# phaistos-networks/Trinity

Hardware: AMD Instinct MI355X
Metric: queries/sec (higher is better)
Workload: dtype u32

## Files before the change

### trinity_amd/csrc/dev_structs.hpp

```cpp
#pragma once
#include <cstdint>
#ifdef __HIPCC__
#define TRI_HD __host__ __device__
#else
#define TRI_HD
#endif

struct DevTerm {
        uint32_t documents;
        uint32_t first_block;
        uint32_t nblocks;
        uint32_t last_n;
        uint32_t win_off;
        uint32_t flags;
        uint32_t npfor;
        uint32_t pad;
};
constexpr uint32_t TERM_FULL_BLOCKS = 1u;
constexpr uint32_t TERM_SPARSE = 2u;

#define TRI_BLOCK_N(t, b, index, off) (((t).flags & TERM_FULL_BLOCKS) ? ((b) + 1 == (t).nblocks ? (t).last_n : 32u) : (uint32_t)(index)[(off)-1])
constexpr uint32_t WIN_MIN_BLOCKS = 128;

constexpr uint32_t QT_GROUP = 0x80000000u;
constexpr uint32_t QT_NOT = 0x40000000u;
constexpr uint32_t QT_TERM = 0x3fffffffu;
constexpr uint32_t MAX_QTERMS = 16;
struct DevQuery {
        uint32_t nterms;
        uint32_t term_base;
        uint64_t out_off;
        uint32_t out_cap;
        uint32_t qid;
        uint32_t first_task, ntasks;
        uint32_t score_base, nscore;
        uint32_t phrase_base, nphrases;
        uint32_t fused_idx, form;
};

constexpr uint32_t RESULT_DOCIDS = 0, RESULT_BITMAP = 1;
constexpr uint32_t MAX_PHRASE_TERMS = 16;
struct DevPhrase {
        uint32_t term_base;
        uint32_t nterms;
        double weight;
};

struct DevTask {
        uint32_t slot;
        uint32_t tile_begin;
        uint32_t tile_end;
        uint32_t kind;
        uint64_t out_off;
};
constexpr uint32_t CAND_QUEUES = 8;
constexpr uint32_t CAND_TICKET_STRIDE = 16;
constexpr uint32_t CAND_HEAVY_TILES = 3;
constexpr uint32_t TASK_CAND = 0;
constexpr uint32_t TASK_DENSE = 1;
constexpr uint32_t TASK_FUSED = 2;
constexpr uint32_t TASK_FUSED16 = 3;

constexpr uint32_t TASK_FUSED_GEN = 4;
constexpr uint32_t TASK_PLANES = 5;
constexpr uint32_t TASK_PLANES8 = 6;
constexpr uint32_t TASK_PSET = 7;
constexpr uint32_t TASK_PROBE = 8;
constexpr uint32_t TASK_TREE = 9;
constexpr uint32_t TASK_KINDS = 10;
constexpr uint32_t PSET_INLINE_TERMS = 4;
#ifndef TRI_PSET_TASK_WINDOWS
#define TRI_PSET_TASK_WINDOWS 4
#endif
constexpr uint32_t PSET_TASK_WINDOWS = TRI_PSET_TASK_WINDOWS;
struct DevPsetUnit {
        uint64_t out_off;
        uint32_t w_begin, w_end;
        uint32_t tix;
        uint32_t nterms;
        uint32_t term_base;
        uint32_t first;
        uint32_t tt[PSET_INLINE_TERMS];
        uint32_t row[PSET_INLINE_TERMS];
};
static_assert(sizeof(DevPsetUnit) == 64, "one cache-line half per unit");
constexpr uint32_t PSET_UNIT_FIRST = 1u, PSET_UNIT_BITMAP = 2u;
constexpr uint32_t PSET_UNIT_ROUND_SHIFT = 4, PSET_UNIT_ROUND_MASK = 15u;
constexpr uint32_t PSET_ROUND_DOCS = 16384, PSET_STAGE_DOCS = 1024;
constexpr uint32_t PSET_UNIT_SCATTER = 4u;
constexpr uint32_t TREE_MAX_NODES = 64;
constexpr uint32_t TREE_HDR_WORDS = 8;
constexpr uint32_t TREE_CHUNK_WORDS = 2048;
constexpr uint32_t TREE_ROW_PHRASE = 0x80000000u;
struct DevTreeNode {
        uint8_t op;
        uint8_t parent;
        uint8_t ord;
        uint8_t thr;
        uint32_t arg;
        uint32_t row;
        uint32_t score;
        uint32_t rmask;
        uint8_t kid0, kid1, pad0, pad1;
        uint64_t kids;
};
static_assert(sizeof(DevTreeNode) == 32, "eight words per node");
constexpr uint32_t TREE_WIDE_MAX_NODES = 1024;
constexpr uint32_t TREE_WIDE_STACK = 64;
constexpr uint32_t TREE_KIND_WIDE = 1;
constexpr uint32_t TREE_NO_PARENT = 0xffffu;
struct DevTreeNodeW {
        uint8_t op;
        uint8_t cbits;
        uint16_t parent;
        uint32_t arg, row, score, rmask;
        uint16_t ord;
        uint16_t nkids;
        uint16_t thr;
        uint8_t pop;
        uint8_t pcbits;
        uint32_t pad;
};
static_assert(sizeof(DevTreeNodeW) == sizeof(DevTreeNode), "a wide record's nodes are eight words each too");
constexpr uint32_t RICH_NARROW_TERMS = 16, RICH_WIDE_TERMS = 64;
struct DevRichWide {
        uint64_t cells;
        uint64_t slots;
        uint32_t stride, pad;
};
static_assert(sizeof(DevRichWide) == 24, "three 8-byte words per plan slot");
TRI_HD constexpr uint32_t tree_counter_planes(const uint32_t nkids) {
        uint32_t b = 0;
        while ((1u << b) <= nkids)
                ++b;
        return b;
}
TRI_HD constexpr bool task_onepass(const uint32_t kind) { return kind >= TASK_FUSED && kind <= TASK_PLANES8; }

constexpr uint32_t PL_W = 32768;
constexpr uint32_t PL_WORDS = PL_W / 32;
constexpr uint32_t PL_NONE = 0xffffffffu;
constexpr uint32_t PL_NESTED = 6;
constexpr uint32_t PL_LEVEL_WORDS = 3;
constexpr uint32_t PL_STORED = 4;
constexpr uint32_t PL_PLANES = PL_STORED + PL_LEVEL_WORDS;
constexpr uint32_t PL_HI = PL_PLANES - 1;
constexpr uint32_t PL_HI_LEVELS = PL_STORED - 1;
constexpr uint32_t PL_RANK_WORDS = 16;
constexpr uint32_t PL_RANK_DOCS = 256;
constexpr uint32_t BLK_HITS_PLAIN = 0x80000000u;
constexpr int TILE_BLOCKS = 256;
constexpr int TILE_CANDS = TILE_BLOCKS * 32;
constexpr uint32_t SPAN_BITS = 1u << 17;
constexpr uint32_t SPAN_WORDS = SPAN_BITS / 32;
constexpr uint32_t CELL_LOG2 = 10;
constexpr uint32_t CELL_DOCS = 1u << CELL_LOG2;
constexpr uint32_t CELLS_PER_SPAN = SPAN_BITS / CELL_DOCS;
#ifndef TRI_FUS_CELLS
#define TRI_FUS_CELLS 14
#endif
constexpr uint32_t FUS_CELLS = TRI_FUS_CELLS;
constexpr uint32_t FUS_W = FUS_CELLS * CELL_DOCS;
constexpr uint32_t PLK_MAX_SPARSE = 6;
constexpr uint32_t PLK_NS_SMALL = 5;
constexpr uint32_t TOPK_MAX = 256;
constexpr uint32_t FUS_MAX_SLOTS = 8;
constexpr uint32_t FUS_MAX_LEAVES = 16;
struct DevFused {
        uint32_t nslots;
        uint32_t fbits;
        uint32_t cap;
        uint32_t nreq;
        uint32_t term[FUS_MAX_SLOTS];
        uint32_t gmask[FUS_MAX_SLOTS];
        uint32_t gslots[FUS_MAX_SLOTS];
        uint32_t nmask;
        uint32_t hw;
        uint32_t mode;
        uint32_t nleaf;
        uint32_t tt[8];
        uint8_t leaf_slot[FUS_MAX_LEAVES];
        uint32_t ctt[FUS_MAX_LEAVES][8];
        uint32_t plane[FUS_MAX_SLOTS];
        uint32_t negslots;
};
constexpr uint32_t FUS_MODE_TT = 1;
constexpr uint32_t FUS_MODE_EMIT = 2;
```

### trinity_amd/csrc/host/plan_host.cpp

```cpp
#include "../planner.hpp"
#include "../lucene_enc_units.hpp"
#include "lucene_encoder.hpp"
#include "perc_lower.hpp"

#include <cstdlib>
#include <memory>
#include <mutex>

namespace {
        struct HostPlan {
                BatchPlan P;
                uint8_t *block = nullptr;
                ~HostPlan() { free(block); }
        };
        void put_err(char *err, size_t cap, const std::string &s) {
                if (err && cap) {
                        const size_t n = std::min(cap - 1, s.size());
                        memcpy(err, s.data(), n);
                        err[n] = 0;
                }
        }
}

extern "C" {
void *tri_host_index_build(const uint8_t *index, uint64_t len, const uint8_t *hits, uint64_t hits_len, int codec, const uint32_t *terms3, uint64_t nterms,
                           uint32_t docs_cnt, char *err, uint64_t errcap) {
        auto H = std::make_unique<HostIndex>();
        std::string e;
        static_assert(sizeof(tri_term) == 12, "tri_term is three u32");
        if (build_host_index(index, len, hits, hits_len, codec, reinterpret_cast<const tri_term *>(terms3), nterms, docs_cnt, *H, e) != TRI_OK) {
                put_err(err, errcap, e);
                return nullptr;
        }
        return H.release();
}
void tri_host_index_free(void *h) { delete static_cast<HostIndex *>(h); }

void *tri_host_plan(void *hindex, const uint32_t *prog, uint64_t prog_len, const uint32_t *queries2, uint64_t nq, uint32_t flags, uint32_t topk, int similarity,
                    unsigned threads, const char *const *opt_names, const uint64_t *opt_values, unsigned nopt, uint32_t cus, char *err, uint64_t errcap) {
        const HostIndex &H = *static_cast<HostIndex *>(hindex);
        PlanEnv env;
        env.cus = cus ? cus : 256;
        bool use_frag_cache = false;
        for (unsigned i = 0; i < nopt; ++i) {
                const std::string n = opt_names[i];
                if (n == "frag_cache") {
                        use_frag_cache = opt_values[i] != 0;
                        continue;
                }
                tri_options &o = env.opt;
                uint64_t *slot = n == "dense_min_postings" ? &o.dense_min_postings : n == "dense_task_cost" ? &o.dense_task_cost : n == "fused" ? &o.fused
                                 : n == "fused_task_cost" ? &o.fused_task_cost : n == "fused_freq_cap" ? &o.fused_freq_cap : n == "fused_halfwords" ? &o.fused_halfwords
                                 : n == "account_needed_bytes" ? &o.account_needed_bytes : n == "planes" ? &o.planes : n == "planes_split" ? &o.planes_split
                                 : n == "plane_div" ? &o.plane_div : n == "plane_max_bytes" ? &o.plane_max_bytes : n == "probe_max_blocks" ? &o.probe_max_blocks : n == "tree_max_bytes" ? &o.tree_max_bytes : n == "tree_max_nodes" ? &o.tree_max_nodes : n == "tree_wide_min_nodes" ? &o.tree_wide_min_nodes : n == "result_bitmaps" ? &o.result_bitmaps : n == "cand_task_cost" ? &o.cand_task_cost : n == "dense_window_cost" ? &o.dense_window_cost
                                 : n == "cand_xcd" ? &o.cand_xcd : n == "planes_order" ? &o.planes_order : n == "pset_order" ? &o.pset_order : n == "scatter_bitmap_slack" ? &o.scatter_bitmap_slack : n == "phrase_task_div" ? &o.phrase_task_div : n == "plane_amortize" ? &o.plane_amortize : n == "rich_max_terms" ? &o.rich_max_terms : nullptr;
                if (!slot) {
                        put_err(err, errcap, "unknown option " + n);
                        return nullptr;
                }
                *slot = opt_values[i];
        }
        PlanInput in;
        in.prog = prog;
        in.prog_len = prog_len;
        static_assert(sizeof(tri_query) == 8, "tri_query is two u32");
        in.queries = reinterpret_cast<const tri_query *>(queries2);
        in.nq = nq;
        in.flags = flags;
        in.topk = topk;
        in.similarity = similarity;
        auto hp = std::make_unique<HostPlan>();
        std::unique_ptr<HostPool> pool;
        if (threads > 1)
                pool = std::make_unique<HostPool>(threads);
        std::string e;
        static trip::FragCache g_frag_cache;
        static std::mutex g_frag_mu;
        std::unique_lock<std::mutex> frag_lock(g_frag_mu, std::defer_lock);
        if (use_frag_cache)
                frag_lock.lock();
        const int rc = plan_batch(
                H, env, in, pool.get(),
                [&](size_t bytes) {
                        hp->block = static_cast<uint8_t *>(aligned_alloc(64, (bytes + 63) & ~(size_t)63));
                        if (hp->block)
                                memset(hp->block, 0, bytes);
                        return hp->block;
                },
                hp->P, e, use_frag_cache ? &g_frag_cache : nullptr);
        if (rc != TRI_OK) {
                put_err(err, errcap, e);
                return nullptr;
        }
        return hp.release();
}
void tri_host_plan_free(void *p) { delete static_cast<HostPlan *>(p); }

void tri_host_plan_summary(void *p, uint64_t *out , double *ms ) {
        const BatchPlan &P = static_cast<HostPlan *>(p)->P;
        const uint64_t v[] = {P.block_bytes,       P.plan.size(),    P.qterms.size(),      P.tasks.size(),  P.fused.size(),       P.qplane.size(),    P.plane_terms.size(), P.sterms.size(),
                              P.sweights.size(),   P.phrases.size(), P.pterms.size(),      P.ptasks.size(), P.plan.off,           P.qterms.off,       P.tasks.off,          P.sched.off,
                              P.fused.off,         P.qplane.off,     P.plane_terms.off,    P.sterms.off,    P.sweights.off,       P.phrases.off,      P.pterms.off,         P.ptasks.off,
                              P.n_dense,           P.n_cand,         P.n_fused,            P.n_fused16,     P.n_fusedgen,         P.n_planes,         P.n_planes8,          P.plw,
                              P.sparse_cap,        P.out_capacity,   P.term_bytes,         P.term_bytes_dense, P.dense_queries,   P.cand_queries,     P.fused_queries,      P.planes_queries,
                              P.unsupported_queries, P.rich_R,       sizeof(DevQuery),     sizeof(DevTask), sizeof(DevFused),     sizeof(DevPhrase),  P.cand_needed_term_bytes, P.plane_decoded_bytes,
                              P.n_pset,            P.pset_queries,   P.n_probe,            P.probe_queries, P.units.size(),       P.units.off,        P.pset_sched.off,     sizeof(DevPsetUnit),
                              P.n_tree,            P.tree_queries,   P.tree.size(),        P.tree.off,      P.tree_terms.size(),  P.tree_terms.off,   P.tree_hidden.size(), P.tree_hidden.off,
                              P.cand_q.off};
        static_assert(sizeof v / sizeof v[0] == 65, "summary layout");
        memcpy(out, v, sizeof v);
        if (ms)
                memcpy(ms, P.plan_ms, sizeof P.plan_ms);
}
void tri_host_plan_rich_wide(void *p, uint64_t *out ) {
        const BatchPlan &P = static_cast<HostPlan *>(p)->P;
        const uint64_t v[] = {P.rich_wide.size(), P.rich_wide.off, P.rich_sched.off, P.n_rich_wide, P.rich_wide_cells, P.rich_wide_slots, sizeof(DevRichWide)};
        memcpy(out, v, sizeof v);
}
void tri_host_plan_last_unsupported(void *p, char *out, uint64_t cap) { put_err(out, cap, static_cast<HostPlan *>(p)->P.last_unsupported); }
const uint8_t *tri_host_plan_block(void *p) { return static_cast<HostPlan *>(p)->P.block; }
void tri_host_plan_query_maps(void *p, uint32_t *slot_of_query, int32_t *qstatus) {
        const BatchPlan &P = static_cast<HostPlan *>(p)->P;
        memcpy(slot_of_query, P.slot_of_query.data(), P.slot_of_query.size() * 4);
        memcpy(qstatus, P.qstatus.data(), P.qstatus.size() * 4);
}
}

extern "C" {
int tri_host_lucene_encode(const uint32_t *docs, const uint32_t *freqs, const uint16_t *pos, const uint64_t *term_first, uint64_t nterms, uint8_t *index_out, uint64_t icap,
                           uint64_t *ilen, uint8_t *hits_out, uint64_t hcap, uint64_t *hlen, uint32_t *terms3) {
        using namespace trinity_amd::Codecs;
        Lucene::IndexSession sess;
        Lucene::Encoder enc(&sess);
        uint64_t h = 0;
        for (uint64_t t = 0; t < nterms; ++t) {
                enc.begin_term();
                for (uint64_t p = term_first[t]; p < term_first[t + 1]; ++p) {
                        enc.begin_document(docs[p]);
                        for (uint32_t i = 0; i < freqs[p]; ++i)
                                enc.new_hit(pos[h++]);
                        enc.end_document();
                }
                trinity_amd::term_index_ctx tctx;
                enc.end_term(&tctx);
                terms3[3 * t] = tctx.documents, terms3[3 * t + 1] = tctx.offset, terms3[3 * t + 2] = tctx.size;
        }
        *ilen = sess.indexOut.size(), *hlen = sess.positionsOut.size();
        if (*ilen > icap || *hlen > hcap)
                return -1;
        if (*ilen)
                memcpy(index_out, sess.indexOut.data(), *ilen);
        if (*hlen)
                memcpy(hits_out, sess.positionsOut.data(), *hlen);
        return 0;
}
int tri_host_lucene_encode_units(const uint32_t *docs, const uint32_t *freqs, const uint16_t *pos, const uint64_t *term_first, uint64_t nterms, uint8_t *index_out, uint64_t icap,
                                 uint64_t *ilen, uint8_t *hits_out, uint64_t hcap, uint64_t *hlen, uint32_t *terms3) {
        const uint64_t np = term_first[nterms];
        std::vector<uint64_t> hit_off(np + 1, 0), dblk_first(nterms + 1, 0), hblk_first(nterms + 1, 0);
        for (uint64_t p = 0; p < np; ++p)
                hit_off[p + 1] = hit_off[p] + freqs[p];
        for (uint64_t t = 0; t < nterms; ++t) {
                dblk_first[t + 1] = dblk_first[t] + (term_first[t + 1] - term_first[t]) / LENC_BLOCK;
                hblk_first[t + 1] = hblk_first[t] + (hit_off[term_first[t + 1]] - hit_off[term_first[t]]) / LENC_BLOCK;
        }
        std::vector<uint32_t> hdelta(hit_off[np] + 1);
        LencArgs a{docs, freqs, pos, hit_off.data(), term_first, hdelta.data(), dblk_first.data(), hblk_first.data(), nterms};
        for (uint64_t p = 0; p < np; ++p)
                lenc_unit_hdelta(a, p, hdelta.data());
        const uint64_t nd = dblk_first[nterms], nh = hblk_first[nterms];
        std::vector<uint64_t> doff(nd + 1, 0), hoff(nh + 1, 0), term_off(nterms + 1, 0), hterm_off(nterms + 1, 0);
        std::vector<uint32_t> tail_d(nterms + 1), tail_h(nterms + 1);
        for (uint64_t g = 0; g < nd; ++g)
                doff[g + 1] = doff[g] + lenc_unit_dblk_size(a, g);
        for (uint64_t h = 0; h < nh; ++h)
                hoff[h + 1] = hoff[h] + lenc_unit_hblk_size(a, h);
        for (uint64_t t = 0; t < nterms; ++t)
                lenc_unit_tail_size(a, t, &tail_d[t], &tail_h[t]);
        LencPlace pl{doff.data(), hoff.data(), term_off.data(), hterm_off.data(), tail_d.data(), tail_h.data()};
        for (uint64_t t = 0; t < nterms; ++t) {
                term_off[t + 1] = term_off[t] + lenc_term_index_size(a, pl, t);
                hterm_off[t + 1] = hterm_off[t] + lenc_term_hits_size(a, pl, t);
        }
        *ilen = term_off[nterms], *hlen = hterm_off[nterms];
        if (*ilen > icap || *hlen > hcap)
                return -1;
        for (uint64_t g = 0; g < nd; ++g)
                lenc_unit_dblk_write(a, pl, g, index_out);
        for (uint64_t h = 0; h < nh; ++h)
                lenc_unit_hblk_write(a, pl, h, hits_out);
        for (uint64_t t = 0; t < nterms; ++t) {
                lenc_unit_term_write(a, pl, t, index_out, hits_out);
                terms3[3 * t] = (uint32_t)(term_first[t + 1] - term_first[t]), terms3[3 * t + 1] = (uint32_t)term_off[t], terms3[3 * t + 2] = lenc_term_index_size(a, pl, t);
        }
        return 0;
}
}

extern "C" {
void tri_host_pfor128_group(const uint32_t *v, uint8_t *a, uint32_t *alen, uint8_t *b, uint32_t *blen) {
        auto get = [&](uint32_t i) { return v[i]; };
        const Pfor128Plan p = pfor128_plan(get);
        uint8_t *e = pfor128_emit(get, p, a);
        *alen = (uint32_t)(e - a);
        if ((uint32_t)(e - a) != p.bytes)
                *alen = 0xffffffffu;
        std::vector<uint8_t> o;
        trinity_amd::Codecs::Lucene::ints_encode(v, o);
        memcpy(b, o.data(), o.size());
        *blen = (uint32_t)o.size();
}
uint32_t tri_host_fastpfor_encode(const uint32_t *v, uint32_t *out) {
        std::vector<uint32_t> w;
        trif::fastpfor_encode(v, w);
        memcpy(out, w.data(), w.size() * 4);
        return (uint32_t)w.size();
}
int tri_host_fastpfor_decode(const uint32_t *w, uint32_t L, uint32_t *v) { return trif::fastpfor_decode(w, L, v) ? 1 : 0; }
uint32_t tri_host_pool_cpus(uint32_t threads, int32_t *out, uint32_t cap) {
        HostPool pool(threads);
        const std::vector<int> &c = pool.pinned_cpus();
        for (size_t i = 0; i < c.size() && i < cap; ++i)
                out[i] = c[i];
        return (uint32_t)c.size();
}

uint32_t tri_host_cpu_budget() { return host_cpu_budget(); }

uint32_t tri_host_index_hits_dir(void *h, uint32_t term, uint32_t *out, uint32_t *nfull) {
        const HostIndex &H = *static_cast<HostIndex *>(h);
        const DevTerm &t = H.terms[term];
        const bool have = H.codec == TRI_CODEC_GOOGLE || H.has_hdir;
        for (uint32_t b = 0; out && have && b < t.nblocks; ++b)
                out[b] = H.blk_hits[t.first_block + b];
        *nfull = H.has_hdir && t.nblocks ? H.hdir[t.pad] : 0;
        return t.nblocks;
}

void tri_host_index_facts(void *h, uint64_t *info6, uint32_t *per_term3) {
        const HostIndex &H = *static_cast<HostIndex *>(h);
        info6[0] = H.info.postings, info6[1] = H.info.blocks, info6[2] = H.info.doc_bytes, info6[3] = H.info.hit_bytes, info6[4] = H.transcoded_groups, info6[5] = H.dev_index.size();
        for (size_t t = 0; t < H.terms.size(); ++t) {
                per_term3[3 * t] = H.terms[t].documents;
                per_term3[3 * t + 1] = H.terms[t].nblocks;
                per_term3[3 * t + 2] = H.terms[t].nblocks ? H.blk_last[H.terms[t].first_block + H.terms[t].nblocks - 1] : 0;
        }
}

int tri_host_perc_lower(const uint32_t *prog, uint64_t prog_len, const uint32_t *queries2, uint64_t nq, uint32_t nterms, int32_t *status, uint64_t *info6, char *err, uint64_t errcap) {
        perc::Lowered L;
        std::string e;
        const int rc = perc::lower(prog, prog_len, reinterpret_cast<const tri_query *>(queries2), nq, nterms, L, e);
        put_err(err, errcap, e);
        if (rc != TRI_OK)
                return rc;
        for (uint64_t q = 0; q < nq; ++q)
                status[q] = L.status[q];
        uint64_t absent = 0;
        for (const uint32_t f : L.qflags)
                absent += (f & perc::Q_ABSENT) != 0;
        info6[0] = L.unsupported, info6[1] = L.leaf_term.size(), info6[2] = L.phrase_first.size() - 1, info6[3] = L.recs.size(), info6[4] = L.stack_max, info6[5] = absent;
        return TRI_OK;
}
int tri_host_perc_check_docs(const tri_perc_docs *docs, uint32_t nterms, char *err, uint64_t errcap) {
        std::string e;
        const int rc = perc::check_docs(docs, nterms, e);
        put_err(err, errcap, e);
        return rc;
}
}
```

### trinity_amd/csrc/k_psets.hpp

```cpp
#pragma once

#ifndef TRI_PSET_WG
#define TRI_PSET_WG 512
#endif
constexpr int PSET_WG = TRI_PSET_WG;
constexpr uint32_t PSET_WAVES = PSET_WG / 64;
constexpr uint32_t PSET_WORDS = 512;
constexpr uint32_t PSET_PER = PSET_WORDS / 64;
constexpr uint32_t PSET_STEP_WORDS = PSET_WAVES * PSET_WORDS;
static_assert(SPAN_WORDS % PSET_STEP_WORDS == 0, "a docID window is a whole number of steps");
constexpr uint32_t PSET_STAGE = 1024;
static_assert(PSET_PER == 8, "two 16-byte loads per lane and term");
static_assert(PSET_WAVES == 8, "the waves' counts are prefix-summed over lanes 0 .. 7 (psets_task)");
static_assert(PSET_WORDS * 32 == PSET_ROUND_DOCS && PSET_STAGE == PSET_STAGE_DOCS, "the planner sizes a task's rounds by them (dev_structs.hpp)");
static_assert(SPAN_WORDS == PSET_WAVES * PSET_WORDS, "a wave's share of a task: one sub-window of PSET_WORDS words per docID window");
static_assert(PSET_STAGE >= PSET_WORDS, "the dense walk parks the wave's words in its staging buffer");

struct PsetShared {
        uint32_t stage[PSET_WAVES][PSET_STAGE];
        alignas(16) uint32_t cnt[2][PSET_WAVES];
        DevPsetUnit unit[2];
        uint32_t tick[2];
};

#ifndef TRI_PSET_PREFETCH
#define TRI_PSET_PREFETCH 0
#endif
struct PsetNoBuf {};
struct PsetPairBuf {
        uint4 a0, a1, b0, b1;
};
template <class BUF, class R, class F>
__device__ __forceinline__ uint32_t psets_round(PsetShared &sh, R &&request, F &&words, const uint32_t w_origin, const uint32_t w_begin, const uint32_t w_end, uint32_t *__restrict__ qout,
                                                const bool as_bitmap, const uint32_t lane, const uint32_t wave, const uint32_t par) {
        const uint32_t nsub = w_end - w_begin;
        const uint32_t wave0 = w_begin * SPAN_WORDS + wave * nsub * PSET_WORDS + lane * PSET_PER;
        uint32_t *const st = sh.stage[wave];
        if (as_bitmap) {
                uint32_t lane_cnt = 0;
                BUF nxt;
                if (TRI_PSET_PREFETCH)
                        request(wave0, nxt);
                for (uint32_t sb = 0; sb < nsub; ++sb) {
                        const uint32_t word0 = wave0 + sb * PSET_WORDS;
                        BUF cur;
                        if (TRI_PSET_PREFETCH) {
                                cur = nxt;
                                if (sb + 1 < nsub)
                                        request(word0 + PSET_WORDS, nxt);
                        } else
                                request(word0, cur);
                        uint32_t acc[PSET_PER];
                        words(cur, word0, acc);
                        uint4 *o = (uint4 *)(qout + (word0 - w_origin * SPAN_WORDS));
                        o[0] = make_uint4(acc[0], acc[1], acc[2], acc[3]);
                        o[1] = make_uint4(acc[4], acc[5], acc[6], acc[7]);
#pragma unroll
                        for (uint32_t j = 0; j < PSET_PER; ++j)
                                lane_cnt += (uint32_t)__popc(acc[j]);
                }
                return lane_cnt;
        }
        uint32_t fill = 0;
        BUF nxt;
        if (TRI_PSET_PREFETCH)
                request(wave0, nxt);
        for (uint32_t sb = 0; sb < nsub; ++sb) {
                const uint32_t word0 = wave0 + sb * PSET_WORDS;
                BUF cur;
                if (TRI_PSET_PREFETCH) {
                        cur = nxt;
                        if (sb + 1 < nsub)
                                request(word0 + PSET_WORDS, nxt);
                } else
                        request(word0, cur);
                uint32_t acc[PSET_PER];
                words(cur, word0, acc);
                uint32_t c = 0;
#pragma unroll
                for (uint32_t j = 0; j < PSET_PER; ++j)
                        c += (uint32_t)__popc(acc[j]);
                uint32_t T;
                const uint32_t ex = wave_excl_scan(c, T);
#if !defined(TRI_PSET_VARIANT) || TRI_PSET_VARIANT != 1
                if (T && fill + T <= PSET_STAGE) {
                        uint32_t o = fill + ex;
#pragma unroll
                        for (uint32_t j = 0; j < PSET_PER; ++j) {
                                uint32_t m = acc[j];
                                const uint32_t d0 = (word0 + j) << 5;
                                while (m) {
                                        st[o++] = d0 + (uint32_t)__builtin_ctz(m);
                                        m &= m - 1u;
                                }
                        }
                }
#endif
                fill += T;
        }
        if (lane == 0)
                sh.cnt[par][wave] = fill;
        __syncthreads();
        const uint32_t own = sh.cnt[par][lane & (PSET_WAVES - 1u)], pre = row8_incl_scan(own);
        const uint32_t base = (uint32_t)__builtin_amdgcn_readlane((int)(pre - own), (int)wave);
        const uint32_t total = (uint32_t)__builtin_amdgcn_readlane((int)pre, (int)PSET_WAVES - 1);
#if defined(TRI_PSET_VARIANT) && (TRI_PSET_VARIANT == 1 || TRI_PSET_VARIANT == 2)
        return total;
#endif
        if (fill <= PSET_STAGE) {
                __builtin_amdgcn_wave_barrier();
                for (uint32_t i = lane; i < fill; i += 64u)
                        qout[base + i] = st[i];
                __builtin_amdgcn_wave_barrier();
        } else {
                uint32_t o = base;
                for (uint32_t sb = 0; sb < nsub; ++sb) {
                        const uint32_t word0 = wave0 + sb * PSET_WORDS;
                        uint32_t acc[PSET_PER];
                        BUF cur;
                        request(word0, cur);
                        words(cur, word0, acc);
                        uint32_t c = 0;
#pragma unroll
                        for (uint32_t j = 0; j < PSET_PER; ++j)
                                c += (uint32_t)__popc(acc[j]);
                        uint32_t T;
                        const uint32_t ex = wave_excl_scan(c, T);
                        if (!T)
                                continue;
                        if (T <= PSET_STAGE) {
                                uint32_t at = ex;
#pragma unroll
                                for (uint32_t j = 0; j < PSET_PER; ++j) {
                                        uint32_t m = acc[j];
                                        const uint32_t d0 = (word0 + j) << 5;
                                        while (m) {
                                                st[at++] = d0 + (uint32_t)__builtin_ctz(m);
                                                m &= m - 1u;
                                        }
                                }
                                __builtin_amdgcn_wave_barrier();
                                for (uint32_t i = lane; i < T; i += 64u)
                                        qout[o + i] = st[i];
                                __builtin_amdgcn_wave_barrier();
                                o += T;
                                continue;
                        }
#pragma unroll
                        for (uint32_t j = 0; j < PSET_PER; ++j)
                                st[lane * PSET_PER + j] = acc[j];
                        __builtin_amdgcn_wave_barrier();
                        const uint32_t wbase = word0 - lane * PSET_PER;
                        for (uint32_t cidx = 0; cidx < PSET_WORDS / 2; ++cidx) {
                                const uint32_t wi = 2u * cidx + (lane >> 5);
                                const bool bit = (st[wi] >> (lane & 31u)) & 1u;
                                const uint64_t bm = __builtin_amdgcn_ballot_w64(bit);
                                if (bit)
                                        qout[o + __builtin_amdgcn_mbcnt_hi((uint32_t)(bm >> 32), __builtin_amdgcn_mbcnt_lo((uint32_t)bm, 0u))] = ((wbase + wi) << 5) + (lane & 31u);
                                o += (uint32_t)__popcll(bm);
                        }
                        __builtin_amdgcn_wave_barrier();
                }
        }
        return total;
}

#ifndef TRI_PSET_WAVES
#define TRI_PSET_WAVES 8
#endif
template <int CODEC>
__global__ __launch_bounds__(PSET_WG, TRI_PSET_WAVES) void k_psets(const DevPsetUnit *__restrict__ units, const uint32_t *__restrict__ order, const uint32_t ntasks,
                                                                   uint32_t *__restrict__ ticket, const uint32_t *__restrict__ qterms, const uint32_t *__restrict__ qplane,
                                                                   uint32_t *__restrict__ out, uint32_t *__restrict__ counts, const uint32_t *__restrict__ masked,
                                                                   const uint32_t *__restrict__ planes, const uint32_t plw, const uint32_t *__restrict__ scat_off,
                                                                   const uint32_t *__restrict__ scat_cnt, const uint32_t *__restrict__ scat_docs TRI_FILTER_ARG) {
        __shared__ PsetShared sh;
        const uint32_t tid = threadIdx.x, lane = tid & 63u;
        const uint32_t wave = uni(tid >> 6);
        uint32_t nt = 0xffffffffu;
        if (wave == 0) {
                const uint32_t t0 = uni(atomicAdd(ticket, 1u)) >> 6;
                uint32_t wd = 0;
                if (t0 < ntasks)
                        wd = ((const uint32_t *)(units + order[t0]))[lane & 15u];
                ((uint32_t *)&sh.unit[0])[lane & 15u] = wd;
                sh.tick[0] = t0;
                nt = uni(atomicAdd(ticket, 1u)) >> 6;
        }
        __syncthreads();
        uint32_t par = 0;
        for (uint32_t p = 0;; p ^= 1u) {
                if (uni(sh.tick[p]) >= ntasks)
                        break;
                const DevPsetUnit &U = sh.unit[p];
                const uint32_t nterms = uni(U.nterms), w_begin = uni(U.w_begin), w_end = uni(U.w_end), tix = uni(U.tix), term_base = uni(U.term_base);
                const bool as_bitmap = uni(U.first) & PSET_UNIT_BITMAP;
                TRI_FILTER_TASK_OF(tix);
                uint32_t *const qout = out + (((uint64_t)uni((uint32_t)(U.out_off >> 32)) << 32) | uni((uint32_t)U.out_off));
                uint32_t nwd = 0, nnt = 0xffffffffu;
                if (wave == 0) {
                        if (nt < ntasks)
                                nwd = ((const uint32_t *)(units + order[nt]))[lane & 15u];
                        nnt = atomicAdd(ticket, 1u);
                }
                uint32_t produced = 0;
                uint32_t scat_at = 0, scat_n = 0;
                if (uni(U.first) & PSET_UNIT_SCATTER)
                        scat_at = uni(scat_off[tix]), scat_n = uni(scat_cnt[tix]);
                const uint32_t round_win = std::max(1u, (uni(U.first) >> PSET_UNIT_ROUND_SHIFT) & PSET_UNIT_ROUND_MASK);
                const uint32_t pair_row0 = uni(U.row[0]), pair_row1 = uni(U.row[1]), pair_tt1 = uni(U.tt[1]);
                if (nterms == 2 && pair_row0 != PL_NONE && pair_row1 != PL_NONE) {
                        const uint32_t *const row_a = planes + (size_t)pair_row0 * plw, *const row_b = planes + (size_t)pair_row1 * plw;
                        const bool pair_or = !(pair_tt1 & QT_GROUP);
                        const uint32_t flip = (pair_tt1 & QT_NOT) ? ~0u : 0u;
                        for (uint32_t wb = w_begin; wb < w_end; wb += round_win, par ^= 1u)
                        produced += psets_round<PsetPairBuf>(
                            sh,
                            [&](const uint32_t word0, PsetPairBuf &buf) {
                                    const uint4 *pa = (const uint4 *)(row_a + word0);
                                    const uint4 *pb = (const uint4 *)(row_b + word0);
                                    buf.a0 = pa[0], buf.a1 = pa[1], buf.b0 = pb[0], buf.b1 = pb[1];
                            },
                            [&](const PsetPairBuf &buf, const uint32_t word0, uint32_t(&acc)[PSET_PER]) {
                                    const uint4 a0 = buf.a0, a1 = buf.a1, b0 = buf.b0, b1 = buf.b1;
                                    if (pair_or) {
                                            acc[0] = a0.x | b0.x, acc[1] = a0.y | b0.y, acc[2] = a0.z | b0.z, acc[3] = a0.w | b0.w;
                                            acc[4] = a1.x | b1.x, acc[5] = a1.y | b1.y, acc[6] = a1.z | b1.z, acc[7] = a1.w | b1.w;
                                    } else {
                                            acc[0] = a0.x & (b0.x ^ flip), acc[1] = a0.y & (b0.y ^ flip), acc[2] = a0.z & (b0.z ^ flip), acc[3] = a0.w & (b0.w ^ flip);
                                            acc[4] = a1.x & (b1.x ^ flip), acc[5] = a1.y & (b1.y ^ flip), acc[6] = a1.z & (b1.z ^ flip), acc[7] = a1.w & (b1.w ^ flip);
                                    }
                                    if (masked) {
                                            const uint4 *pm = (const uint4 *)(masked + word0);
                                            const uint4 m0 = pm[0], m1 = pm[1];
                                            acc[0] &= ~m0.x, acc[1] &= ~m0.y, acc[2] &= ~m0.z, acc[3] &= ~m0.w;
                                            acc[4] &= ~m1.x, acc[5] &= ~m1.y, acc[6] &= ~m1.z, acc[7] &= ~m1.w;
                                    }
                            },
                            w_begin, wb, min(w_end, wb + round_win), as_bitmap ? qout : qout + produced, as_bitmap, lane, wave, par);
                } else
                        for (uint32_t wb = w_begin; wb < w_end; wb += round_win, par ^= 1u)
                        produced += psets_round<PsetNoBuf>(
                            sh, [](const uint32_t, PsetNoBuf &) {},
                            [&](const PsetNoBuf &, const uint32_t word0, uint32_t(&acc)[PSET_PER]) {
                                    uint32_t grp[PSET_PER];
                                    bool have_acc = false, cur_neg = false;
#pragma unroll
                                    for (uint32_t j = 0; j < PSET_PER; ++j)
                                            acc[j] = grp[j] = 0;
                                    for (uint32_t k = 0; k <= nterms; ++k) {
                                            uint32_t tt = QT_GROUP, row = 0;
                                            if (k < nterms) {
                                                    if (nterms <= PSET_INLINE_TERMS) {
                                                            tt = uni(U.tt[k]);
                                                            row = uni(U.row[k]);
                                                    } else {
                                                            tt = uni(qterms[term_base + k]);
                                                            row = uni(qplane[term_base + k]);
                                                    }
                                            }
                                            if (k && (tt & QT_GROUP)) {
#pragma unroll
                                                    for (uint32_t j = 0; j < PSET_PER; ++j) {
                                                            acc[j] = !have_acc ? grp[j] : cur_neg ? acc[j] & ~grp[j] : acc[j] & grp[j];
                                                            grp[j] = 0;
                                                    }
                                                    have_acc = true;
                                            }
                                            if (k == nterms)
                                                    break;
                                            if (tt & QT_GROUP)
                                                    cur_neg = tt & QT_NOT;
                                            if (row == PL_NONE)
                                                    continue;
                                            const uint4 *pa = (const uint4 *)(planes + (size_t)row * plw + word0);
#if defined(TRI_PSET_VARIANT) && TRI_PSET_VARIANT == 3
                                            const uint32_t hsh = (word0 * 2654435761u) ^ (k * 40503u);
                                            const uint4 v0 = make_uint4(hsh & (hsh >> 3) & (hsh >> 7), 0, (hsh >> 5) & (hsh << 2) & (hsh >> 11), 0), v1 = make_uint4(0, hsh & 0x10001u, 0, hsh & 0x200u);
#else
                                            const uint4 v0 = pa[0], v1 = pa[1];
#endif
                                            grp[0] |= v0.x, grp[1] |= v0.y, grp[2] |= v0.z, grp[3] |= v0.w;
                                            grp[4] |= v1.x, grp[5] |= v1.y, grp[6] |= v1.z, grp[7] |= v1.w;
                                    }
                                    if (masked) {
                                            const uint4 *pm = (const uint4 *)(masked + word0);
                                            const uint4 m0 = pm[0], m1 = pm[1];
                                            acc[0] &= ~m0.x, acc[1] &= ~m0.y, acc[2] &= ~m0.z, acc[3] &= ~m0.w;
                                            acc[4] &= ~m1.x, acc[5] &= ~m1.y, acc[6] &= ~m1.z, acc[7] &= ~m1.w;
                                    }
                            },
                            w_begin, wb, min(w_end, wb + round_win), as_bitmap ? qout : qout + produced, as_bitmap, lane, wave, par);
                if (uni(U.first) & PSET_UNIT_SCATTER) {
                        __syncthreads();
                        const uint32_t off = scat_at, n = scat_n, doc0 = w_begin * SPAN_BITS;
                        for (uint32_t i = tid; i < n; i += PSET_WG) {
                                const uint32_t rel = scat_docs[off + i] - doc0, bit = 1u << (rel & 31u);
                                produced += (atomicOr(&qout[rel >> 5], bit) & bit) ? 0u : 1u;
                        }
                }
                if (as_bitmap) {
#pragma unroll
                        for (int d = 32; d >= 1; d >>= 1)
                                produced += __shfl_xor(produced, d, 64);
                        sh.cnt[par][wave] = produced;
                        __syncthreads();
                        produced = 0;
#pragma unroll
                        for (uint32_t wv = 0; wv < PSET_WAVES; ++wv)
                                produced += uni(sh.cnt[par][wv]);
                        par ^= 1u;
                }
                if (wave == 0) {
                        counts[tix] = produced;
                        ((uint32_t *)&sh.unit[p ^ 1u])[lane & 15u] = nwd;
                        sh.tick[p ^ 1u] = nt;
                        __builtin_amdgcn_s_waitcnt(0xc07f);
                        nt = uni(nnt) >> 6;
                }
                __syncthreads();
        }
}

constexpr int PSCAT_WG = 256;
constexpr uint32_t PSCAT_MAX_TASKS = 4096;
static_assert((1ull << 31) / ((uint64_t)PSET_TASK_WINDOWS * SPAN_BITS) <= PSCAT_MAX_TASKS, "a query's tasks fit the workgroup's LDS counters");
struct PscatShared {
        DevTerm term[MAX_QTERMS];
        uint32_t nrows[MAX_QTERMS];
        uint32_t cnt[PSCAT_MAX_TASKS];
        uint32_t red[PSCAT_WG / 64 + 1];
};
struct PscatPost {
        uint32_t *cnt;
        const uint32_t *masked;
        uint32_t *place;
        uint32_t nbits, task_docs, cap;
        __device__ __forceinline__ void doc(const uint32_t d) {
                if (d >= nbits || (masked && ((masked[d >> 5] >> (d & 31u)) & 1u)))
                        return;
                const uint32_t at = atomicAdd(&cnt[d / task_docs], 1u);
                if (place && at < cap)
                        place[at] = d;
        }
        __device__ __forceinline__ void operator()(const uint32_t d, const uint32_t) { doc(d); }
};
__global__ __launch_bounds__(256) void k_psets_prep_list(const DevPsetUnit *__restrict__ units, const uint32_t nunits, uint32_t *__restrict__ cursor, uint32_t *__restrict__ list,
                                                         const uint32_t cap) {
        const uint32_t u = blockIdx.x * 256u + threadIdx.x;
        if (u >= nunits || !(units[u].first & PSET_UNIT_SCATTER) || units[u].w_begin != 0)
                return;
        const uint32_t at = atomicAdd(cursor, 1u);
        if (at < cap)
                list[at] = u;
}
template <int CODEC>
__global__ __launch_bounds__(PSCAT_WG) void k_psets_prep(const DevPsetUnit *__restrict__ units, const uint32_t *__restrict__ list, const uint32_t *__restrict__ listed, const DevQuery *__restrict__ plan, const DevTask *__restrict__ tasks,
                                                         const uint32_t *__restrict__ qterms, const uint32_t *__restrict__ qplane, const uint32_t *__restrict__ masked_,
                                                         const uint8_t *__restrict__ index, const uint32_t *__restrict__ blk_last, const uint32_t *__restrict__ blk_off,
                                                         const uint4 *__restrict__ blk_rec, const uint32_t *__restrict__ blk_doff, const DevTerm *__restrict__ terms,
                                                         uint32_t *__restrict__ cursor, uint32_t *__restrict__ scat_off, uint32_t *__restrict__ scat_cnt,
                                                         uint32_t *__restrict__ scat_docs, const uint32_t scat_cap, const FilterSel fsel) {
        __shared__ PscatShared sh;
        const uint32_t tid = threadIdx.x;
        if (blockIdx.x >= uni(*listed))
                return;
        const DevPsetUnit &U = units[uni(list[blockIdx.x])];
        const uint32_t nterms = uni(U.nterms), term_base = uni(U.term_base), tix = uni(U.tix);
        if (tid < MAX_QTERMS) {
                uint32_t n = 0;
                if (tid < nterms && qplane[term_base + tid] == PL_NONE) {
                        const DevTerm t = terms[qterms[term_base + tid] & QT_TERM];
                        sh.term[tid] = t;
                        n = t.nblocks;
                }
                sh.nrows[tid] = n;
        }
        const uint32_t slot = uni(tasks[tix].slot);
        const DevQuery &q = plan[slot];
        const uint32_t *const masked = filter_pick_if(masked_, fsel, slot);
        const uint32_t ntasks = min(uni(q.ntasks), PSCAT_MAX_TASKS), nbits = uni(q.out_cap) * 32u, task_docs = (uni(U.w_end) - uni(U.w_begin)) * SPAN_BITS;
        for (uint32_t t = tid; t < ntasks; t += PSCAT_WG)
                sh.cnt[t] = 0;
        __syncthreads();
        uint32_t total = 0;
        for (uint32_t k = 0; k < nterms; ++k)
                total += uni(sh.nrows[k]);
        for (uint32_t pass = 0; pass < 2; ++pass) {
                PscatPost post{sh.cnt, masked, pass ? scat_docs : nullptr, nbits, task_docs, scat_cap};
                for (uint32_t v = tid; v < total; v += PSCAT_WG) {
                        uint32_t k = 0, b = v;
                        for (; b >= sh.nrows[k]; ++k)
                                b -= sh.nrows[k];
                        const DevTerm t = sh.term[k];
                        const uint32_t *bl = blk_last + t.first_block;
                        const uint32_t prev = b ? bl[b - 1] : 0, last = bl[b];
#ifdef TRI_PROF
                        ProfClock prof_;
#endif
                        decode_row<CODEC, false, PscatPost>(index, blk_off, blk_rec, blk_doff, t, b, prev, last, 0u, post PROF_PASS);
                }
                __syncthreads();
                if (pass)
                        break;
                const uint32_t per = (ntasks + PSCAT_WG - 1) / PSCAT_WG, t0 = tid * per, t1 = min(ntasks, t0 + per);
                uint32_t mine = 0;
                for (uint32_t t = t0; t < t1; ++t)
                        mine += sh.cnt[t];
                uint32_t wtot;
                uint32_t ex = wave_excl_scan(mine, wtot);
                if ((tid & 63u) == 0)
                        sh.red[tid >> 6] = wtot;
                __syncthreads();
                uint32_t before = 0, all = 0;
                for (uint32_t w = 0; w < PSCAT_WG / 64; ++w) {
                        before += w < (tid >> 6) ? sh.red[w] : 0u;
                        all += sh.red[w];
                }
                if (tid == 0)
                        sh.red[PSCAT_WG / 64] = atomicAdd(cursor, all);
                __syncthreads();
                const uint32_t base = uni(sh.red[PSCAT_WG / 64]);
                uint32_t at = base + before + ex;
                for (uint32_t t = t0; t < t1; ++t) {
                        const uint32_t c = sh.cnt[t];
                        const bool fits = at + c <= scat_cap;
                        scat_off[tix + t] = fits ? at : 0u;
                        scat_cnt[tix + t] = fits ? c : 0u;
                        sh.cnt[t] = fits ? at : scat_cap;
                        at += c;
                }
                __syncthreads();
        }
}
```

### trinity_amd/csrc/planner.hpp

```cpp
#pragma once
#include "planner_lower.hpp"
#include "planner_tasks.hpp"

namespace trip {
        struct RowQ {
                uint8_t n = 0, q[CAND_QUEUES] = {}, sub[CAND_QUEUES] = {};
        };
        struct LapTimer {
                const bool on;
                std::chrono::steady_clock::time_point t0 = std::chrono::steady_clock::now();
                std::string line;
                void lap(const char *what) {
                        if (!on)
                                return;
                        char buf[64];
                        snprintf(buf, sizeof buf, " %s %.3f", what, ms_since(t0));
                        line += buf;
                }
        };

        struct PlanState {
                const HostIndex &ix;
                const PlanEnv &env;
                const tri_options &opt;
                HostPool *pool;
                BatchPlan &P;
                std::string &err;
                Ctx C;
                LapTimer dbg;
                FragCache *cache = nullptr;
                std::vector<Frag> frags;
                SectionCounts n;
                uint64_t cand_queries_all = 0;
                std::vector<uint64_t> benefit, cand_row;
                std::vector<uint32_t> tree_terms;
                std::vector<uint32_t> chosen;
                std::vector<uint32_t> row_of_rank;
                bool cand_rows = false;
                std::vector<RowQ> rowq;
                uint32_t pset_ranges = 0;
                uint32_t cand_first = 0, cand_qat[CAND_QUEUES] = {};
                std::vector<uint32_t> unit_of_task;
                ~PlanState() {
                        if (!cache)
                                return;
                        if (cache->frags.size() < frags.size())
                                cache->frags.resize(frags.size());
                        for (size_t k = 0; k < frags.size(); ++k)
                                cache->frags[k] = std::move(frags[k]);
                }
                template <class Fn>
                void run(Fn &&fn) {
                        if (pool && frags.size() > 1)
                                pool->run((unsigned)frags.size(), fn);
                        else
                                for (unsigned k = 0; k < frags.size(); ++k)
                                        fn(k);
                }
                int first_error() {
                        for (Frag &f : frags)
                                if (f.rc != TRI_OK) {
                                        err = f.err;
                                        return f.rc;
                                }
                        return TRI_OK;
                }
                template <class Fn>
                int run_pass(const char *name, const char *doing, Fn &&fn) {
                        run([&](unsigned k) {
                                Frag &f = frags[k];
                                try {
                                        f.rc = fn(f);
                                } catch (const std::bad_alloc &) {
                                        f.rc = herr(f.err, TRI_ERR_NOMEM, "tri_batch_create: out of host memory while %s", doing);
                                } catch (...) {
                                        f.rc = herr(f.err, TRI_ERR_INVALID, "tri_batch_create: unexpected exception while %s", doing);
                                }
                        });
                        dbg.lap(name);
                        return first_error();
                }
        };

        inline void eligible_planes(PlanState &S) {
                const HostIndex &ix = S.ix;
                const tri_options &opt = S.opt;
                S.P.plw = ((ix.max_doc >> 17) + 2u) * (SPAN_BITS / 32u);
                S.C.plw = S.P.plw;
                if (opt.planes && opt.plane_div && !ix.df_sorted.empty()) {
                        const uint64_t min_df = std::max<uint64_t>(1, ix.info.docs_cnt / opt.plane_div);
                        const size_t n = (size_t)(std::partition_point(ix.df_sorted.begin(), ix.df_sorted.end(), [&](uint32_t d) { return d && d >= min_df; }) - ix.df_sorted.begin());
                        const uint64_t row_bytes = (uint64_t)PL_PLANES * S.P.plw * 4;
                        S.C.n_ok = (uint32_t)std::min<uint64_t>(n, std::max<uint64_t>(1, opt.plane_max_bytes / std::max<uint64_t>(1, row_bytes)));
                }
        }

        inline void take_fragments(PlanState &S, FragCache *cache) {
                const size_t nq = S.C.in.nq;
                const unsigned nthreads = S.pool ? std::min<unsigned>(S.pool->size(), (unsigned)std::max<size_t>(1, nq / 512)) : 1u;
                const size_t nfrag = nthreads <= 1 ? 1 : std::min<size_t>(2 * nthreads, std::max<size_t>(1, nq / 256));
                S.frags.resize(nfrag);
                S.cache = cache;
                for (size_t k = 0; k < nfrag; ++k) {
                        if (cache && k < cache->frags.size()) {
                                S.frags[k] = std::move(cache->frags[k]);
                                S.frags[k].recycle();
                        }
                        S.frags[k].q_lo = nq * k / nfrag;
                        S.frags[k].q_hi = nq * (k + 1) / nfrag;
                }
        }

        inline void settle_batch_knobs(PlanState &S) {
                const tri_options &opt = S.opt;
                const PlanEnv &env = S.env;
                Ctx &C = S.C;
                uint64_t onepass_queries = 0, fused_postings = 0, phrase_queries = 0;
                for (const Frag &f : S.frags) {
                        onepass_queries += f.onepass_queries;
                        fused_postings += f.fused_postings;
                        phrase_queries += f.phrase_queries;
                }
                C.phrase_task_div = opt.phrase_task_div ? opt.phrase_task_div : !phrase_queries ? 1 : phrase_queries <= 8ull * env.cus ? 4 : phrase_queries <= 16ull * env.cus ? 2 : 1;
                C.planes_split = opt.planes_split ? opt.planes_split : (2 * onepass_queries >= 4ull * (uint64_t)env.cus * env.plk_wgs_per_cu ? 2 : 3) ;
                C.fused_task_cost = opt.fused_task_cost;
                if (!C.fused_task_cost) {
                        const uint64_t want_tasks = 2ull * (uint64_t)env.cus * env.fus_wgs_per_cu;
                        C.fused_task_cost = std::min<uint64_t>(8u << 20, std::max<uint64_t>(256u << 10, fused_postings / std::max<uint64_t>(1, want_tasks)));
                }
        }

        inline int place_fragments(PlanState &S) {
                BatchPlan &P = S.P;
                SectionCounts &n = S.n;
                const uint32_t n_ok = S.C.n_ok;
                uint64_t off = 0;
                S.benefit.assign(n_ok, 0), S.cand_row.assign(n_ok, 0);
                for (Frag &f : S.frags) {
                        f.b_plan = n.plan, f.b_qterms = n.qterms, f.b_sterms = n.sterms, f.b_phrases = n.phrases, f.b_pterms = n.pterms, f.b_tasks = n.tasks, f.b_fused = n.fused,
                        f.b_ptasks = n.ptasks, f.b_off = off, f.b_units = n.units, f.b_tree = n.tree, f.b_hidden = n.tree_hidden;
                        n.plan += f.tmp.size(), n.qterms += f.qterms.size(), n.sterms += f.sterms.size(), n.phrases += f.phrases.size(), n.pterms += f.pterms.size(),
                                n.tasks += f.tasks.size(), n.fused += f.fused.size(), n.ptasks += f.ptasks.size(), n.units += f.units.size(), n.tree += f.treepool.size(),
                                n.tree_hidden += f.n_hidden, off += f.off;
                        S.tree_terms.insert(S.tree_terms.end(), f.tree_terms.begin(), f.tree_terms.end());
                        P.merge(f);
                        for (uint32_t r = 0; r < n_ok; ++r)
                                S.benefit[r] += f.benefit[r], S.cand_row[r] += f.cand_row[r];
                        for (const size_t qi : f.left_out) {
                                P.qstatus[qi] = TRI_ERR_UNSUPPORTED;
                                ++P.unsupported_queries;
                        }
                        if (!f.left_out.empty())
                                P.last_unsupported = f.err;
                }
                S.cand_queries_all = P.cand_queries + P.probe_queries;
                if (n.qterms > 0xfffffff0ull || n.sterms > 0xfffffff0ull || n.tasks > 0xfffffff0ull || n.pterms > 0xfffffff0ull)
                        return herr(S.err, TRI_ERR_UNSUPPORTED, "tri_batch_create: the batch exceeds 2^32 terms or tasks: split it");
                P.out_capacity = off;
                if (P.rich_wide_queries)
                        n.rich_wide = n.plan, n.rich_sched = n.tasks;
                std::sort(S.tree_terms.begin(), S.tree_terms.end());
                S.tree_terms.erase(std::unique(S.tree_terms.begin(), S.tree_terms.end()), S.tree_terms.end());
                n.tree_terms = S.tree_terms.size();
                P.tree_scratch_bytes = ((uint64_t)n.tree_terms * PL_PLANES + n.tree_hidden + P.tree_queries) * P.plw * 4;
                if (P.tree_scratch_bytes > S.opt.tree_max_bytes)
                        return herr(S.err, TRI_ERR_NOMEM, "tri_batch_create: the batch's %llu tree queries need %llu bytes of bitmap scratch (%zu distinct term leaves, %zu phrase leaves; option tree_max_bytes = %llu): split the batch",
                                    (unsigned long long)P.tree_queries, (unsigned long long)P.tree_scratch_bytes, n.tree_terms, n.tree_hidden, (unsigned long long)S.opt.tree_max_bytes);
                return TRI_OK;
        }

        inline void choose_planes(PlanState &S) {
                const HostIndex &ix = S.ix;
                const uint32_t n_ok = S.C.n_ok;
                std::vector<uint32_t> rank_term(n_ok, UINT32_MAX);
                std::vector<uint8_t> forced(n_ok, 0);
                for (const Frag &f : S.frags) {
                        for (const QUse &u : f.quses)
                                rank_term[ix.df_rank[u.term]] = u.term;
                        for (const QUse &u : f.suses)
                                rank_term[ix.df_rank[u.term]] = u.term;
                        for (const FUse &u : f.fuses)
                                rank_term[ix.df_rank[u.term]] = u.term, forced[ix.df_rank[u.term]] = 1;
                }
                for (uint32_t r = 0; r < n_ok; ++r)
                        if (rank_term[r] != UINT32_MAX && (forced[r] || S.benefit[r] * std::max<uint64_t>(1, S.opt.plane_amortize) >= ix.terms[rank_term[r]].documents))
                                S.chosen.push_back(rank_term[r]);
                std::sort(S.chosen.begin(), S.chosen.end());
                S.row_of_rank.assign(n_ok, PL_NONE);
                for (const uint32_t term : S.chosen) {
                        S.row_of_rank[ix.df_rank[term]] = ix.df_rank[term];
                        S.P.plane_decoded_bytes += ix.docbytes[term];
                }
                S.P.plane_rows = n_ok;
                S.n.plane_terms = S.chosen.size();
                S.n.qplane = S.chosen.empty() ? 0 : S.n.qterms;
                S.n.splane = (S.chosen.empty() || !S.C.scored) ? 0 : S.n.sterms;
                S.n.sweights = S.C.scored ? S.n.sterms : 0;
        }

        inline void assign_cand_rows(PlanState &S) {
                const BatchPlan &P = S.P;
                const uint32_t n_ok = S.C.n_ok;
                const std::vector<uint64_t> &cand_row = S.cand_row;
                S.pset_ranges = ((S.ix.max_doc >> 17) + 1u + PSET_TASK_WINDOWS - 1) / PSET_TASK_WINDOWS;
                S.cand_rows = S.opt.cand_xcd && !S.chosen.empty() && S.cand_queries_all && P.cand_lead_docs >= CAND_ROWS_MIN_LEAD * S.cand_queries_all && P.cand_terms <= 3 * S.cand_queries_all;
                S.rowq.assign(S.cand_rows ? n_ok : 0, RowQ{});
                if (S.cand_rows) {
                        uint64_t total = 0, load[CAND_QUEUES] = {};
                        uint32_t placed[CAND_QUEUES] = {};
                        std::vector<uint32_t> rows;
                        for (uint32_t r = 0; r < n_ok; ++r)
                                if (cand_row[r] && S.row_of_rank[r] != PL_NONE)
                                        rows.push_back(r), total += cand_row[r];
                        std::sort(rows.begin(), rows.end(), [&](uint32_t a, uint32_t b) { return cand_row[a] != cand_row[b] ? cand_row[a] > cand_row[b] : a < b; });
                        const uint64_t cap = std::max<uint64_t>(1, total / (2 * CAND_QUEUES));
                        for (const uint32_t r : rows) {
                                RowQ &z = S.rowq[r];
                                z.n = (uint8_t)std::min<uint64_t>(CAND_QUEUES, (cand_row[r] + cap - 1) / cap);
                                for (uint32_t k = 0; k < z.n; ++k) {
                                        const uint32_t x = (uint32_t)(std::min_element(load, load + CAND_QUEUES) - load);
                                        load[x] += cand_row[r] / z.n;
                                        z.q[k] = (uint8_t)x;
                                        z.sub[k] = (uint8_t)(CAND_COST_SUBS + placed[x]++ % (CAND_SUBS - CAND_COST_SUBS - 1));
                                }
                        }
                }
                if (S.dbg.on) {
                        char buf[96];
                        snprintf(buf, sizeof buf, " [cand queries %llu lead docs %llu terms %llu rows %d]", (unsigned long long)S.cand_queries_all, (unsigned long long)P.cand_lead_docs, (unsigned long long)P.cand_terms, (int)S.cand_rows);
                        S.dbg.line += buf;
                }
        }

        inline int layout_block(PlanState &S, const std::function<uint8_t *(size_t)> &alloc_block) {
                BatchPlan &P = S.P;
                P.block_bytes = layout_sections(P, S.n);
                S.dbg.lap("sums+planes+layout");
                P.block = alloc_block(P.block_bytes);
                S.dbg.lap("alloc_block");
                if (!P.block)
                        return herr(S.err, TRI_ERR_NOMEM, "tri_batch_create: no host memory for the plan (%zu bytes)", P.block_bytes);
                point_sections(P, S.n);
                std::copy(S.tree_terms.begin(), S.tree_terms.end(), P.tree_terms.p);
                S.unit_of_task.assign(S.n.units ? S.n.tasks : 0, 0u);
                std::copy(S.chosen.begin(), S.chosen.end(), P.plane_terms.p);
                S.dbg.lap("spans");
                return TRI_OK;
        }

        inline int fill_fragment(PlanState &S, Frag &f) {
                const HostIndex &ix = S.ix;
                BatchPlan &P = S.P;
                const std::vector<uint32_t> &row_of_rank = S.row_of_rank;
                for (size_t i = 0; i < f.tmp.size(); ++i) {
                        DevQuery q = f.tmp[i].q;
                        q.term_base += (uint32_t)f.b_qterms;
                        q.score_base += (uint32_t)f.b_sterms;
                        q.phrase_base += (uint32_t)f.b_phrases;
                        q.first_task += (uint32_t)f.b_tasks;
                        q.out_off += f.b_off;
                        if (f.tmp[i].fuse)
                                q.fused_idx += (uint32_t)f.b_fused;
                        if (f.tmp[i].tree)
                                q.fused_idx += (uint32_t)f.b_tree;
                        if (f.tmp[i].hidden) {
                                q.qid = 0xffffffffu;
                                P.tree_hidden[f.b_hidden + f.tmp[i].hidden_ord] = (uint32_t)(f.b_plan + i);
                        } else
                                P.slot_of_query[q.qid] = (uint32_t)(f.b_plan + i);
                        P.plan[f.b_plan + i] = q;
                }
                if (!f.treepool.empty()) {
                        memcpy(&P.tree[f.b_tree], f.treepool.data(), f.treepool.size() * 4);
                        for (size_t i = 0; i < f.tmp.size(); ++i) {
                                if (!f.tmp[i].tree)
                                        continue;
                                uint32_t *rec = &P.tree[f.b_tree + f.tmp[i].q.fused_idx];
                                DevTreeNode *tn = reinterpret_cast<DevTreeNode *>(rec + TREE_HDR_WORDS);
                                for (uint32_t k = 0; k < rec[0]; ++k)
                                        if (tn[k].op == TRI_OP_TERM)
                                                tn[k].row = (uint32_t)(std::lower_bound(P.tree_terms.begin(), P.tree_terms.end(), tn[k].arg) - P.tree_terms.begin());
                                        else if (tn[k].op == TRI_OP_PHRASE) {
                                                tn[k].arg += (uint32_t)f.b_plan;
                                                tn[k].row += (uint32_t)f.b_hidden;
                                        }
                        }
                }
                for (size_t i = 0; i < f.tasks.size(); ++i) {
                        DevTask t = f.tasks[i];
                        t.slot += (uint32_t)f.b_plan;
                        t.out_off += f.b_off;
                        P.tasks[f.b_tasks + i] = t;
                }
                if (!f.qterms.empty())
                        memcpy(&P.qterms[f.b_qterms], f.qterms.data(), f.qterms.size() * 4);
                if (!f.sterms.empty())
                        memcpy(&P.sterms[f.b_sterms], f.sterms.data(), f.sterms.size() * 4);
                if (S.C.scored && !f.sweights.empty())
                        memcpy(&P.sweights[f.b_sterms], f.sweights.data(), f.sweights.size() * 8);
                for (size_t i = 0; i < f.phrases.size(); ++i) {
                        DevPhrase ph = f.phrases[i];
                        ph.term_base += (uint32_t)f.b_pterms;
                        P.phrases[f.b_phrases + i] = ph;
                }
                if (!f.pterms.empty())
                        memcpy(&P.pterms[f.b_pterms], f.pterms.data(), f.pterms.size() * 4);
                for (size_t i = 0; i < f.ptasks.size(); ++i)
                        P.ptasks[f.b_ptasks + i] = f.ptasks[i] + (uint32_t)f.b_tasks;
                for (size_t i = 0; i < f.fused.size(); ++i)
                        P.fused[f.b_fused + i] = f.fused[i];
                for (const FUse &u : f.fuses)
                        P.fused[f.b_fused + u.fidx].plane[u.slot] = row_of_rank[ix.df_rank[u.term]];
                for (size_t i = 0; i < f.units.size(); ++i) {
                        DevPsetUnit u = f.units[i];
                        u.out_off += f.b_off;
                        u.tix += (uint32_t)f.b_tasks;
                        u.term_base += (uint32_t)f.b_qterms;
                        const bool is_probe = f.tasks[f.units[i].tix].kind == TASK_PROBE;
                        bool rows = true;
                        for (uint32_t k = is_probe ? 1u : 0u; k < u.nterms; ++k) {
                                const uint32_t term = (k < PSET_INLINE_TERMS ? u.tt[k] : f.qterms[f.units[i].term_base + k]) & QT_TERM;
                                const uint32_t rank = ix.df_rank[term];
                                const uint32_t row = rank < row_of_rank.size() ? row_of_rank[rank] : PL_NONE;
                                rows &= row != PL_NONE;
                                if (k < PSET_INLINE_TERMS)
                                        u.row[k] = row;
                                if (row == PL_NONE && (u.first & PSET_UNIT_SCATTER) && u.w_begin == 0)
                                        f.pscatter_docs += ix.terms[term].documents;
                        }
                        if (is_probe && !rows) {
                                P.tasks[u.tix].kind = TASK_CAND;
                                if (u.first & PSET_UNIT_FIRST) {
                                        ++f.probe_demoted;
                                        f.probe_demoted_bytes += distinct_docbytes(ix, &f.qterms[f.units[i].term_base], u.nterms, f.S.seen);
                                }
                        }
                        P.units[f.b_units + i] = u;
                        S.unit_of_task[u.tix] = (uint32_t)(f.b_units + i);
                }
                if (S.n.splane) {
                        std::fill(&P.splane.p[f.b_sterms], &P.splane.p[f.b_sterms] + f.sterms.size(), PL_NONE);
                        for (const QUse &u : f.suses)
                                P.splane[f.b_sterms + u.qpos] = row_of_rank[ix.df_rank[u.term]];
                }
                if (S.n.qplane) {
                        std::fill(&P.qplane.p[f.b_qterms], &P.qplane.p[f.b_qterms] + f.qterms.size(), PL_NONE);
                        for (const QUse &u : f.quses)
                                P.qplane[f.b_qterms + u.qpos] = row_of_rank[ix.df_rank[u.term]];
                }
                return TRI_OK;
        }

        inline uint32_t key_planes_order(const PlanState &S, const Frag &f, const size_t i, const DevTask &tk) {
                const DevQuery &q = S.P.plan[tk.slot];
                const DevFused &z = S.P.fused[q.fused_idx];
                uint32_t minrow = PL_NONE;
                for (uint32_t sidx = 0; sidx < z.nslots; ++sidx)
                        minrow = std::min(minrow, z.plane[sidx]);
                const uint32_t ord = (uint32_t)(f.b_tasks + i) - q.first_task, per = SCHED_NB / 4;
                return SCHED_RANK[tk.kind] * SCHED_NB + (S.opt.planes_order == 2 ? std::min(minrow, per - 1) * 4 + std::min(ord, 3u) : std::min(ord, 3u) * per + std::min(minrow, per - 1));
        }
        inline uint32_t key_pset_order(const PlanState &S, const Frag &f, const size_t i) {
                const uint32_t range = (uint32_t)(f.tcost[i] & 0xffffffffull) / PSET_TASK_WINDOWS;
                const uint32_t rb = S.pset_ranges <= PSET_RANGE_BKS ? std::min(range, PSET_RANGE_BKS - 1) : (uint32_t)std::min<uint64_t>((uint64_t)range * PSET_RANGE_BKS / S.pset_ranges, PSET_RANGE_BKS - 1);
                return PSET_KEY0 + rb * PSET_SUBS + pset_sub((uint32_t)(f.tcost[i] >> 32));
        }
        inline uint32_t key_cand_rows(const PlanState &S, const Frag &f, const size_t i, const DevTask &tk) {
                const DevQuery &q = S.P.plan[tk.slot];
                uint32_t row = PL_NONE;
                for (uint32_t k = 1; k < q.nterms && row == PL_NONE; ++k)
                        row = S.P.qplane[q.term_base + k];
                uint32_t queue, sub;
                if (tk.tile_end - tk.tile_begin > CAND_HEAVY_TILES || row == PL_NONE)
                        queue = (uint32_t)(f.b_tasks + i) % CAND_QUEUES, sub = (sched_key(TASK_CAND, f.tcost[i]) % SCHED_NB) / (SCHED_NB / CAND_COST_SUBS);
                else if (row < S.rowq.size() && S.rowq[row].n) {
                        const RowQ &z = S.rowq[row];
                        const uint32_t piece = (uint32_t)(f.b_tasks + i) % z.n;
                        queue = z.q[piece], sub = z.sub[piece];
                } else
                        queue = row % CAND_QUEUES, sub = CAND_SUBS - 1;
                return CAND_KEY0 + queue * CAND_SUBS + sub;
        }
        inline uint32_t schedule_key(const PlanState &S, const Frag &f, const size_t i) {
                const DevTask &tk = S.P.tasks[f.b_tasks + i];
                switch (tk.kind) {
                        case TASK_PLANES:
                        case TASK_PLANES8:
                                if (S.opt.planes_order)
                                        return key_planes_order(S, f, i, tk);
                                break;
                        case TASK_PSET:
                                if (S.opt.pset_order)
                                        return key_pset_order(S, f, i);
                                break;
                        case TASK_CAND:
                                if (S.cand_rows)
                                        return key_cand_rows(S, f, i, tk);
                                break;
                }
                return sched_key(tk.kind, f.tcost[i]);
        }
        inline int key_fragment(const PlanState &S, Frag &f) {
                f.keys.resize(f.tasks.size());
                f.hist.assign(SCHED_KEYS, 0u);
                for (size_t i = 0; i < f.tasks.size(); ++i)
                        ++f.hist[f.keys[i] = schedule_key(S, f, i)];
                return TRI_OK;
        }

        inline void place_schedule(PlanState &S) {
                BatchPlan &P = S.P;
                uint32_t at = 0;
                for (uint32_t r = 0; r < TASK_KINDS; ++r) {
                        const uint32_t before = at;
                        if (r == SCHED_RANK[TASK_CAND])
                                S.cand_first = at;
                        auto place = [&](const uint32_t bk) {
                                for (Frag &f : S.frags) {
                                        const uint32_t c = f.hist[bk];
                                        f.hist[bk] = at;
                                        at += c;
                                }
                        };
                        for (uint32_t bk = r * SCHED_NB; bk < (r + 1) * SCHED_NB; ++bk)
                                place(bk);
                        if (r == SCHED_RANK[TASK_PSET] && S.opt.pset_order)
                                for (uint32_t bk = PSET_KEY0; bk < PSET_KEY0 + std::min(S.pset_ranges, PSET_RANGE_BKS) * PSET_SUBS; ++bk)
                                        place(bk);
                        if (r == SCHED_RANK[TASK_CAND])
                                for (uint32_t bk = CAND_KEY0; bk < PSET_KEY0; ++bk) {
                                        if ((bk - CAND_KEY0) % CAND_SUBS == 0)
                                                S.cand_qat[(bk - CAND_KEY0) / CAND_SUBS] = at;
                                        place(bk);
                                }
                        for (uint32_t k = 0; k < TASK_KINDS; ++k)
                                if (SCHED_RANK[k] == r)
                                        P.*SCHED_COUNT[k] = at - before;
                }
                const uint32_t units_first = sched_first(P, TASK_PSET), n_units_run = P.n_pset + P.n_probe;
                S.run([&](unsigned k) {
                        Frag &f = S.frags[k];
                        for (size_t i = 0; i < f.tasks.size(); ++i) {
                                const uint32_t pos = f.hist[f.keys[i]]++, ti = (uint32_t)(f.b_tasks + i);
                                P.sched[pos] = ti;
                                if (pos >= units_first && pos - units_first < n_units_run)
                                        P.pset_sched[pos - units_first] = S.unit_of_task[ti];
                        }
                });
        }

        inline void split_tree_section(BatchPlan &P) {
                if (!P.n_tree)
                        return;
                uint32_t *const ts = P.sched.p + sched_first(P, TASK_TREE);
                auto narrow = [&](const uint32_t ti) { return P.tree[P.plan[P.tasks[ti].slot].fused_idx + 1] != TREE_KIND_WIDE; };
                P.n_tree_wide = P.n_tree - (uint32_t)std::count_if(ts, ts + P.n_tree, narrow);
                if (P.n_tree_wide && P.n_tree_wide < P.n_tree)
                        std::stable_partition(ts, ts + P.n_tree, narrow);
        }

        inline void place_rich_wide(BatchPlan &P) {
                if (P.rich_wide.empty())
                        return;
                uint64_t cells = 0, slots = 0;
                for (size_t i = 0; i < P.plan.size(); ++i) {
                        const DevQuery &q = P.plan[i];
                        DevRichWide w{};
                        if (q.nscore > RICH_NARROW_TERMS) {
                                w.cells = cells, w.slots = slots, w.stride = (q.nscore + 7u) & ~7u;
                                cells += (uint64_t)q.out_cap * w.stride, slots += q.out_cap;
                                P.n_rich_wide += q.ntasks;
                        }
                        P.rich_wide[i] = w;
                }
                P.rich_wide_cells = cells, P.rich_wide_slots = slots;
                std::copy(P.sched.begin(), P.sched.end(), P.rich_sched.begin());
                std::stable_partition(P.rich_sched.begin(), P.rich_sched.end(), [&](const uint32_t ti) { return P.rich_wide[P.tasks[ti].slot].stride == 0; });
        }

        inline void deal_cand_queues(PlanState &S) {
                BatchPlan &P = S.P;
                const uint32_t nc = P.n_cand;
                uint32_t *const sc = P.sched.p + S.cand_first;
                if (S.cand_rows) {
                        for (uint32_t x = 0; x <= CAND_QUEUES; ++x)
                                P.cand_q[x] = x < CAND_QUEUES ? S.cand_qat[x] - S.cand_first : nc;
                } else {
                        const std::vector<uint32_t> was(sc, sc + nc);
                        uint32_t pos = 0;
                        for (uint32_t x = 0; x < CAND_QUEUES; ++x) {
                                P.cand_q[x] = pos;
                                for (uint32_t i = x; i < nc; i += CAND_QUEUES)
                                        sc[pos++] = was[i];
                        }
                        P.cand_q[CAND_QUEUES] = pos;
                }
        }

        inline void order_phrase_tasks(BatchPlan &P) {
                if (P.ptasks.size() <= 1)
                        return;
                const size_t np = P.ptasks.size();
                std::vector<uint32_t> key(np), sorted(np);
                uint32_t hist[SCHED_NB + 1] = {};
                for (size_t i = 0; i < np; ++i) {
                        const uint32_t ti = P.ptasks[i];
                        const DevTask &tk = P.tasks[ti];
                        const DevQuery &q = P.plan[tk.slot];
                        const uint64_t end = ti + 1 < q.first_task + q.ntasks ? P.tasks[ti + 1].out_off : q.out_off + q.out_cap;
                        key[i] = SCHED_NB - 1 - cost_bucket(end - tk.out_off);
                        ++hist[key[i] + 1];
                }
                for (uint32_t bk = 0; bk < SCHED_NB; ++bk)
                        hist[bk + 1] += hist[bk];
                for (size_t i = 0; i < np; ++i)
                        sorted[hist[key[i]]++] = P.ptasks[i];
                std::copy(sorted.begin(), sorted.end(), P.ptasks.p);
        }

        inline void account_distinct_bytes(const HostIndex &ix, const Ctx &C, BatchPlan &P) {
                std::vector<uint8_t> seen(ix.terms.size(), 0);
                std::vector<uint8_t> seen_hits(ix.terms.size(), 0);
                for (size_t sidx = 0; sidx < P.plan.size(); ++sidx) {
                        const DevQuery &q = P.plan[sidx];
                        const uint32_t kind = P.tasks[q.first_task].kind;
                        auto touch = [&](uint32_t term) {
                                if (!(seen[term] & 0x80u))
                                        P.distinct_bytes += ix.docbytes[term];
                                if (!(seen[term] & (1u << kind)))
                                        P.distinct_bytes_kind[kind] += ix.docbytes[term];
                                seen[term] |= (uint8_t)(0x80u | (1u << kind));
                        };
                        if (kind == TASK_TREE) {
                                const uint32_t *rec = &P.tree[q.fused_idx];
                                const DevTreeNode *tn = reinterpret_cast<const DevTreeNode *>(rec + TREE_HDR_WORDS);
                                for (uint32_t k = 0; k < rec[0]; ++k)
                                        if (tn[k].op == TRI_OP_TERM)
                                                touch(tn[k].arg);
                        } else if (task_onepass(kind)) {
                                const DevFused &z = P.fused[q.fused_idx];
                                for (uint32_t k = 0; k < z.nslots; ++k)
                                        touch(z.term[k]);
                        } else {
                                for (uint32_t k = 0; k < q.nterms; ++k)
                                        touch(P.qterms[q.term_base + k] & QT_TERM);
                                if (C.mode != TRI_FLAG_DOCUMENTS_ONLY)
                                        for (uint32_t k = 0; k < q.nscore; ++k)
                                                touch(P.sterms[q.score_base + k]);
                        }
                        auto touch_hits = [&](uint32_t term, bool phrase) {
                                if (!(seen_hits[term] & 1u))
                                        P.distinct_bytes += ix.hitbytes[term];
                                if (phrase && !(seen_hits[term] & 2u))
                                        P.distinct_bytes_kind[TASK_KINDS] += ix.hitbytes[term];
                                seen_hits[term] |= (uint8_t)(1u | (phrase ? 2u : 0u));
                        };
                        for (uint32_t ph = 0; ph < q.nphrases; ++ph)
                                for (uint32_t k = 0; k < P.phrases[q.phrase_base + ph].nterms; ++k)
                                        touch_hits(P.pterms[P.phrases[q.phrase_base + ph].term_base + k], true);
                        if (C.rich)
                                for (uint32_t k = 0; k < q.nscore; ++k)
                                        touch_hits(P.sterms[q.score_base + k], false);
                }
        }
}

inline int plan_batch(const HostIndex &ix, const PlanEnv &env, const PlanInput &in, HostPool *pool, const std::function<uint8_t *(size_t)> &alloc_block,
                      BatchPlan &P, std::string &err, trip::FragCache *frag_cache = nullptr) {
        using namespace trip;
        auto t0 = std::chrono::steady_clock::now();
        static const bool dbg_plan = getenv("TRINITY_DEBUG_PLAN") != nullptr;
        const uint32_t mode = in.flags & (TRI_FLAG_DOCUMENTS_ONLY | TRI_FLAG_ACCUMULATED_SCORE | TRI_FLAG_MATCHED_TERMS);
        PlanState S{ix, env, env.opt, pool, P, err, Ctx{ix, env, in, mode == TRI_FLAG_ACCUMULATED_SCORE, mode == TRI_FLAG_MATCHED_TERMS, mode}, LapTimer{dbg_plan}};
        if (env.opt.tree_max_nodes < TREE_MAX_NODES || env.opt.tree_max_nodes > TREE_WIDE_MAX_NODES)
                return herr(err, TRI_ERR_INVALID, "tri_batch_create: option tree_max_nodes = %llu (%u .. %u)", (unsigned long long)env.opt.tree_max_nodes, TREE_MAX_NODES, TREE_WIDE_MAX_NODES);
        if (env.opt.rich_max_terms < RICH_NARROW_TERMS || env.opt.rich_max_terms > RICH_WIDE_TERMS)
                return herr(err, TRI_ERR_INVALID, "tri_batch_create: option rich_max_terms = %llu (%u .. %u)", (unsigned long long)env.opt.rich_max_terms, RICH_NARROW_TERMS, RICH_WIDE_TERMS);
        P.slot_of_query.assign(in.nq, UINT32_MAX);
        P.qstatus.assign(in.nq, TRI_OK);
        eligible_planes(S);
        take_fragments(S, frag_cache);
        S.dbg.lap("setup");
        if (const int rc = S.run_pass("LOWER", "lowering the batch", [&](Frag &f) { return lower_range(S.C, f); }))
                return rc;
        settle_batch_knobs(S);
        S.dbg.lap("glue0");
        P.plan_ms[0] = ms_since(t0);
        if (const int rc = S.run_pass("TASKS", "cutting the batch into tasks", [&](Frag &f) { return task_range(S.C, f); }))
                return rc;
        P.plan_ms[1] = ms_since(t0);
        if (const int rc = place_fragments(S))
                return rc;
        choose_planes(S);
        assign_cand_rows(S);
        if (const int rc = layout_block(S, alloc_block))
                return rc;
        if (const int rc = S.run_pass("FILL", "filling the plan", [&](Frag &f) {
                    fill_fragment(S, f);
                    return key_fragment(S, f);
            }))
                return rc;
        for (const Frag &f : S.frags) {
                P.pscatter_docs += f.pscatter_docs;
                P.probe_queries -= f.probe_demoted, P.cand_queries += f.probe_demoted;
                P.term_bytes_probe -= f.probe_demoted_bytes;
        }
        P.plan_ms[2] = ms_since(t0);
        place_schedule(S);
        deal_cand_queues(S);
        split_tree_section(P);
        place_rich_wide(P);
        order_phrase_tasks(P);
        P.sparse_cap = (P.sparse_cap + 63u) & ~63u;
        S.dbg.lap("sched+rest");
        if (dbg_plan)
                fprintf(stderr, "[tri plan] nq %zu frags %zu:%s\n", in.nq, S.frags.size(), S.dbg.line.c_str());
        P.plan_ms[3] = ms_since(t0);
        if (env.opt.account_needed_bytes && !ix.terms.empty())
                account_distinct_bytes(ix, S.C, P);
        return TRI_OK;
}
```

### trinity_amd/csrc/planner_tasks.hpp

```cpp
#pragma once
#include "planner_types.hpp"

namespace trip {
        inline void tasks_tree(const Ctx &C, Frag &f, Tmp &t, const uint32_t slot, uint64_t &off) {
                t.q.out_off = off;
                t.q.out_cap = (uint32_t)t.tree_ub;
                t.q.first_task = (uint32_t)f.tasks.size();
                t.q.ntasks = 1;
                f.tcost.push_back(std::max<uint64_t>(1, t.tree_ub));
                f.tasks.push_back({slot, 0, (C.plw + TREE_CHUNK_WORDS - 1) / TREE_CHUNK_WORDS, TASK_TREE, off});
                off += t.q.out_cap;
                ++f.tree_queries;
        }

        inline int tasks_onepass(const Ctx &C, Frag &f, Tmp &t, const uint32_t slot, uint64_t &off) {
                const HostIndex &ix = C.ix;
                DevFused z = f.fz[t.fz];
                uint32_t nsparse = 0;
                for (uint32_t sidx = 0; sidx < z.nslots; ++sidx) {
                        z.plane[sidx] = PL_NONE;
                        nsparse += C.plane_ok(z.term[sidx]) ? 0u : 1u;
                }
                const bool pk = !t.truth && (C.env.opt.planes & 4u) && nsparse <= PLK_MAX_SPARSE && ix.max_doc < 0x7fff0000u;
                {
// ... 30 lines not shown
                        if (emit)
                                for (uint32_t sidx = 0; sidx < z.nslots; ++sidx)
                                        b1 += C.first_block_ge(ix.terms[z.term[sidx]], (uint64_t)wb * fw);
                        uint64_t entries = 0;
                        if (pk) {
                                for (uint32_t sidx = 0; sidx < z.nslots; ++sidx) {
                                        if (C.plane_ok(z.term[sidx]))
                                                continue;
                                        const DevTerm &tk = ix.terms[z.term[sidx]];
                                        const uint32_t r0 = C.first_block_ge(tk, (uint64_t)wb * fw);
                                        const uint32_t r1 = C.first_block_ge(tk, (uint64_t)we * fw);
                                        if (r0 < tk.nblocks)
                                                entries += 32ull * (std::min(r1, tk.nblocks - 1) - r0 + 1);
                                }
                                if (entries > 0x7fffffffull)
                                        return herr(f.err, TRI_ERR_UNSUPPORTED, "query %u: a task's decoded lists exceed 2^31 entries", t.q.qid);
                                f.sparse_cap = std::max(f.sparse_cap, (uint32_t)entries);
                        }
                        f.tcost.push_back(per_win * (we - wb));
                        f.tasks.push_back({slot, wb, we, pk ? (z.nslots <= PLK_NS_SMALL ? TASK_PLANES : TASK_PLANES8) : z.mode ? TASK_FUSED_GEN : z.hw ? TASK_FUSED16 : TASK_FUSED,
                                           off + (emit ? b1 * 32 + 32ull * ord * z.nslots : 0)});
                }
                if (emit) {
                        uint64_t blocks = 0;
                        for (uint32_t sidx = 0; sidx < z.nslots; ++sidx)
                                blocks += ix.terms[z.term[sidx]].nblocks;
                        t.q.out_cap = (uint32_t)std::min<uint64_t>(0xffffffffull, blocks * 32 + 32ull * (ord + 1) * z.nslots);
                        off += t.q.out_cap;
                }
                t.q.ntasks = (uint32_t)f.tasks.size() - t.q.first_task;
                f.fused.push_back(z);
                return TRI_OK;
        }

        struct Route {
                bool pset = false;
                bool pscatter = false;
                bool probe = false;
        };
        inline Route route_cnf(const Ctx &C, Frag &f, Tmp &t, const uint32_t *qt) {
                const HostIndex &ix = C.ix;
                const tri_options &opt = C.env.opt;
                const uint64_t planes_opt = opt.planes;
                const DevTerm &lead = ix.terms[qt[0] & QT_TERM];
                Route r;
                r.pset = t.dense && (planes_opt & 2u);
                for (uint32_t k = 0; r.pset && k < t.q.nterms; ++k)
                        r.pset = C.plane_ok(qt[k] & QT_TERM);
                if (t.dense && !r.pset && (planes_opt & 2u) && C.mode == TRI_FLAG_DOCUMENTS_ONLY && opt.result_bitmaps && !t.q.nphrases && t.q.nterms >= 2) {
                        uint64_t plane_df = 0;
                        bool one_group = true;
                        for (uint32_t k = 0; k < t.q.nterms; ++k) {
                                one_group = one_group && !(qt[k] & QT_NOT) && (k == 0) == ((qt[k] & QT_GROUP) != 0);
                                if (C.plane_ok(qt[k] & QT_TERM))
                                        plane_df += ix.terms[qt[k] & QT_TERM].documents;
                        }
                        const uint32_t nwin = t.last_doc / SPAN_BITS + 1;
                        const double N = std::max<double>(1.0, (double)ix.info.docs_cnt);
                        r.pscatter = one_group && plane_df && std::min<double>(N, (double)plane_df) * (double)std::max<uint64_t>(1, opt.scatter_bitmap_slack) >= (double)nwin * SPAN_WORDS;
                        r.pset = r.pscatter;
                }
                if (t.dense && !r.pset && t.nlead == 1 && (planes_opt & 1u) && !C.plane_ok(qt[0] & QT_TERM) && t.q.nterms >= 2) {
                        bool probes = true;
                        for (uint32_t k = 1; probes && k < t.q.nterms; ++k)
                                probes = C.plane_ok(qt[k] & QT_TERM);
                        if (probes)
                                t.dense = false;
                }
                if (t.dense) {
                        (r.pset ? f.term_bytes_pset : f.term_bytes_dense) += distinct_docbytes(ix, qt, t.q.nterms, f.S.seen);
                        for (uint32_t k = 0; k < t.q.nterms; ++k) {
                                const uint32_t term = qt[k] & QT_TERM;
                                if ((planes_opt & 2u) && C.plane_ok(term)) {
                                        f.benefit[ix.df_rank[term]] += ix.terms[term].documents;
                                        f.quses.push_back({t.q.term_base + k, term});
                                }
                        }
                        ++(r.pset ? f.pset_queries : f.dense_queries);
                } else {
                        r.probe = t.nlead == 1 && t.q.nterms >= 2 && t.q.nphrases == 0 && (planes_opt & 1u) && lead.nblocks <= opt.probe_max_blocks;
                        for (uint32_t k = 1; r.probe && k < t.q.nterms; ++k)
                                r.probe = C.plane_ok(qt[k] & QT_TERM);
                        ++(r.probe ? f.probe_queries : f.cand_queries);
                        f.cand_lead_docs += lead.documents, f.cand_terms += t.q.nterms;
                        if (r.probe)
                                f.term_bytes_probe += distinct_docbytes(ix, qt, t.q.nterms, f.S.seen);
                        bool first_row = !r.probe;
                        for (uint32_t k = 1; k < t.q.nterms; ++k) {
                                const uint32_t term = qt[k] & QT_TERM;
                                if ((planes_opt & 1u) && C.plane_ok(term)) {
                                        f.benefit[ix.df_rank[term]] += std::min<uint64_t>(ix.terms[term].documents, 32ull * lead.documents);
                                        f.quses.push_back({t.q.term_base + k, term});
                                        if (first_row) {
                                                const uint32_t ntiles = (lead.nblocks + TILE_BLOCKS - 1) / TILE_BLOCKS;
                                                f.cand_row[ix.df_rank[term]] += ntiles + (ntiles + CAND_HEAVY_TILES - 1) / CAND_HEAVY_TILES;
                                                first_row = false;
                                        }
                                }
                        }
                }
                if (C.scored && (planes_opt & 1u))
                        for (uint32_t k = 0; k < t.q.nscore; ++k) {
                                const uint32_t term = f.sterms[t.q.score_base + k];
                                if (C.plane_ok(term)) {
                                        f.benefit[ix.df_rank[term]] += std::min<uint64_t>(ix.terms[term].documents, 32ull * t.lead_docs);
                                        f.suses.push_back({t.q.score_base + k, term});
                                }
                        }
                return r;
        }

        inline int tasks_windows(const Ctx &C, Frag &f, Tmp &t, const uint32_t slot, const uint32_t *qt, const Route r, const uint64_t off) {
                const HostIndex &ix = C.ix;
                const tri_options &opt = C.env.opt;
                const uint32_t nlead = t.nlead;
                const bool pset = r.pset, pscatter = r.pscatter;
                const uint32_t nwin = t.last_doc / SPAN_BITS + 1;
                bool bitmap = false;
                double est = 1.0;
                if (pset || (C.mode == TRI_FLAG_DOCUMENTS_ONLY && opt.result_bitmaps && !t.q.nphrases)) {
                        const double N = std::max<double>(1.0, (double)ix.info.docs_cnt);
                        double g = 0.0;
                        bool negg = false;
                        for (uint32_t k = 0; k <= t.q.nterms; ++k) {
                                if (k == t.q.nterms || (k && (qt[k] & QT_GROUP))) {
                                        if (!negg)
                                                est *= std::min(1.0, g / N);
                                        g = 0.0;
                                }
                                if (k == t.q.nterms)
                                        break;
                                if (qt[k] & QT_GROUP)
                                        negg = qt[k] & QT_NOT;
                                g += ix.terms[qt[k] & QT_TERM].documents;
                        }
                        bitmap = C.mode == TRI_FLAG_DOCUMENTS_ONLY && opt.result_bitmaps && !t.q.nphrases && (pscatter || est * N >= (double)nwin * SPAN_WORDS);
                }
                uint32_t round_win = 1;
                while (round_win < PSET_TASK_WINDOWS && est * (double)PSET_ROUND_DOCS * (double)(round_win * 2u) <= 0.75 * (double)PSET_STAGE_DOCS)
                        round_win *= 2u;
                if (pscatter && !bitmap)
                        return herr(f.err, TRI_ERR_INTERNAL, "query %u: a scatter union whose result is not a bitmap", t.q.qid);
                t.q.form = bitmap ? RESULT_BITMAP : RESULT_DOCIDS;
                const uint64_t per_win = std::max<uint64_t>(1, t.sumdf / (ix.info.docs_cnt / SPAN_BITS + 1)) + (pset ? 0 : opt.dense_window_cost);
                const uint32_t pdiv = t.q.nphrases ? (uint32_t)std::max<uint64_t>(1, C.phrase_task_div) : 1u;
                const uint32_t win_per_task = pset ? std::max(1u, PSET_TASK_WINDOWS / pdiv) : (uint32_t)std::max<uint64_t>(1, std::max<uint64_t>(1, opt.dense_task_cost) / pdiv / per_win);
                uint32_t ord = 0;
                uint64_t lead_blocks = 0;
                for (uint32_t k = 0; k < nlead; ++k)
                        lead_blocks += ix.terms[qt[k] & QT_TERM].nblocks;
                uint64_t heaviest = 0xffffffffull;
                for (uint32_t k = 0; pset && k < t.q.nterms; ++k)
                        heaviest = std::min<uint64_t>(heaviest, ix.df_rank[qt[k] & QT_TERM]);
                for (uint32_t wb = 0; wb < nwin; wb += win_per_task, ++ord) {
                        const uint32_t we = std::min(nwin, wb + win_per_task);
                        uint64_t b1 = 0;
                        for (uint32_t k = 0; k < nlead; ++k)
                                b1 += C.first_block_ge(ix.terms[qt[k] & QT_TERM], (uint64_t)wb * SPAN_BITS);
                        f.tcost.push_back(pset ? wb | heaviest << 32 : per_win * (we - wb));
                        const uint64_t task_off = bitmap ? off + (uint64_t)wb * SPAN_WORDS : off + b1 * 32 + 32ull * ord * nlead;
                        if (pset)
                                f.units.push_back(make_unit(t.q, qt, (uint32_t)f.tasks.size(), wb, we, task_off,
                                                            (bitmap ? PSET_UNIT_BITMAP : 0u) | (pscatter ? PSET_UNIT_SCATTER : 0u) | round_win << PSET_UNIT_ROUND_SHIFT));
                        f.tasks.push_back({slot, wb, we, pset ? TASK_PSET : TASK_DENSE, task_off});
                }
                t.q.out_cap = bitmap ? nwin * SPAN_WORDS : (uint32_t)std::min<uint64_t>(0xffffffffull, lead_blocks * 32 + 32ull * (ord + 1) * nlead);
                f.bitmap_queries += bitmap;
                f.pscatter_queries += pscatter;
                return TRI_OK;
        }

        inline uint64_t cand_needed_bytes(const HostIndex &ix, const uint32_t *qt, const uint32_t nterms) {
                const DevTerm &lead = ix.terms[qt[0] & QT_TERM];
                uint64_t need = ix.docbytes[qt[0] & QT_TERM];
                const uint32_t *ll = &ix.blk_last[lead.first_block];
                for (uint32_t k = 1; k < nterms; ++k) {
                        const DevTerm &tk = ix.terms[qt[k] & QT_TERM];
                        const uint32_t *ol = &ix.blk_last[tk.first_block];
                        uint64_t blocks = 0;
                        uint32_t at = 0;
                        for (uint32_t lb = 0; lb < lead.nblocks && at < tk.nblocks; ++lb) {
                                const uint32_t lo_doc = lb ? ll[lb - 1] + 1 : 1u, hi_doc = ll[lb];
                                at = (uint32_t)(std::lower_bound(ol + at, ol + tk.nblocks, lo_doc) - ol);
                                if (at >= tk.nblocks)
                                        break;
                                const uint32_t last = (uint32_t)(std::lower_bound(ol + at, ol + tk.nblocks, hi_doc) - ol);
                                const uint32_t span = std::min(last, tk.nblocks - 1) - at + 1;
                                const uint32_t ndocs = lb + 1 == lead.nblocks ? lead.last_n : 32u;
                                blocks += std::min(span, ndocs);
                        }
                        need += (uint64_t)((double)ix.docbytes[qt[k] & QT_TERM] * std::min(1.0, (double)blocks / std::max(1u, tk.nblocks)));
                }
                return need;
        }

        inline void tasks_tiles(const Ctx &C, Frag &f, Tmp &t, const uint32_t slot, const uint32_t *qt, const Route r, const uint64_t off) {
                const tri_options &opt = C.env.opt;
                const DevTerm &lead = C.ix.terms[qt[0] & QT_TERM];
                const uint32_t ntiles = (lead.nblocks + TILE_BLOCKS - 1) / TILE_BLOCKS;
                const uint64_t per_tile = std::max<uint64_t>(1, t.cost / ntiles);
                const uint32_t tiles_per_task = (uint32_t)std::max<uint64_t>(1, std::max<uint64_t>(1, opt.cand_task_cost / (t.q.nphrases ? std::max<uint64_t>(1, C.phrase_task_div) : 1)) / per_tile);
                for (uint32_t tb = 0; tb < ntiles; tb += tiles_per_task) {
                        const uint32_t te = std::min(ntiles, tb + tiles_per_task);
                        f.tcost.push_back(per_tile * (te - tb));
                        if (r.probe)
                                f.units.push_back(make_unit(t.q, qt, (uint32_t)f.tasks.size(), tb, te, off + (uint64_t)tb * TILE_CANDS, tb == 0 ? PSET_UNIT_FIRST : 0u));
                        f.tasks.push_back({slot, tb, te, r.probe ? TASK_PROBE : TASK_CAND, off + (uint64_t)tb * TILE_CANDS});
                }
                t.q.out_cap = lead.documents;
                if (opt.account_needed_bytes)
                        f.cand_needed_term_bytes += cand_needed_bytes(C.ix, qt, t.q.nterms);
        }

        inline int task_range(const Ctx &C, Frag &f) {
                const HostIndex &ix = C.ix;
                f.benefit.assign(C.n_ok, 0);
                f.cand_row.assign(C.n_ok, 0);
                uint64_t off = 0;
                for (size_t ti = 0; ti < f.tmp.size(); ++ti) {
                        if (ti + 6 < f.tmp.size()) {
                                const Tmp &a = f.tmp[ti + 6];
                                for (uint32_t k = 0; k < a.q.nterms && k < 8 && !a.tree; ++k)
                                        prefetch_term(ix, f.qterms[a.q.term_base + k] & QT_TERM);
                        }
                        Tmp &t = f.tmp[ti];
                        const uint32_t slot = (uint32_t)ti;
                        if (t.tree) {
                                tasks_tree(C, f, t, slot, off);
                                continue;
                        }
                        if (t.fuse) {
                                if (const int rc = tasks_onepass(C, f, t, slot, off))
                                        return rc;
                                continue;
                        }
                        const uint32_t *qt = &f.qterms[t.q.term_base];
                        const Route r = route_cnf(C, f, t, qt);
                        t.q.out_off = off;
                        t.q.first_task = (uint32_t)f.tasks.size();
                        if (t.dense) {
                                if (const int rc = tasks_windows(C, f, t, slot, qt, r, off))
                                        return rc;
                        } else
                                tasks_tiles(C, f, t, slot, qt, r, off);
                        off += t.q.out_cap;
                        t.q.ntasks = (uint32_t)f.tasks.size() - t.q.first_task;
                        if (t.q.nphrases)
                                for (uint32_t k = t.q.first_task; k < t.q.first_task + t.q.ntasks; ++k)
                                        f.ptasks.push_back(k);
                }
                f.off = off;
                return TRI_OK;
        }
}
```

### trinity_amd/csrc/planner_types.hpp

```cpp
#pragma once
#include "host_pool.hpp"
#include "index_host.hpp"

#include <array>
#include <chrono>
#include <cmath>
#include <memory>
#include <numeric>

struct tri_options {
        uint64_t dense_min_postings = 512 * 1024;
        uint64_t dense_task_cost = 192 * 1024;
        uint64_t dense_window_cost = 16 * 1024;
        uint64_t cand_task_cost = 32 * 1024;
        uint64_t fused = 1;
        uint64_t fused_task_cost = 0;
        uint64_t fused_freq_cap = 0;
        uint64_t account_needed_bytes = 0;
        uint64_t fused_halfwords = 1;
        uint64_t overlap_dense_wgs = 0, overlap_cand_wgs = 0;
        uint64_t overlap = 0;
        uint64_t planes = 7;
        uint64_t planes_split = 0;
        uint64_t plane_div = 1024;
        uint64_t plane_amortize = 1;
        uint64_t plane_max_bytes = 8ull << 30;
        uint64_t planes_rebuild = 0;
        uint64_t phrase_task_div = 0;
        uint64_t planes_order = 1;
        uint64_t scatter_bitmap_slack = 4;
        uint64_t pset_order = 1;
        uint64_t cand_xcd = 1;
        uint64_t plan_threads = 0;
        uint64_t plan_hot_us = 300;
        uint64_t plan_pin = 2;
        uint64_t result_bitmaps = 1;
        uint64_t tree_max_bytes = 16ull << 30;
        uint64_t tree_max_nodes = 64;
        uint64_t tree_wide_min_nodes = 65;
        uint64_t rich_max_terms = 16;
        uint64_t isect_max_bytes = 2ull << 30;
        uint64_t isect_max_masks = 262144;
        uint64_t isect_max_runs = 524288;
        uint64_t perc_max_bytes = 4ull << 30;
        uint64_t perc_prune = 1;
        uint64_t probe_max_blocks = 0;
};

struct PlanEnv {
        tri_options opt;
        uint32_t cus = 256;
        uint32_t fus_wgs_per_cu = 2;
        uint32_t plk_wgs_per_cu = 2;
};

template <class T>
struct Span {
        T *p = nullptr;
        size_t n = 0;
        size_t off = 0;
        size_t size() const { return n; }
        bool empty() const { return !n; }
        T *data() { return p; }
        const T *data() const { return p; }
        T &operator[](size_t i) { return p[i]; }
        const T &operator[](size_t i) const { return p[i]; }
        T *begin() { return p; }
        T *end() { return p + n; }
        const T *begin() const { return p; }
        const T *end() const { return p + n; }
};

struct PlanInput {
        const uint32_t *prog = nullptr;
        size_t prog_len = 0;
        const tri_query *queries = nullptr;
        size_t nq = 0;
        const double *weights = nullptr;
        uint32_t flags = 0, topk = 0;
        int similarity = TRI_SIM_BM25;
};

namespace trip {
        struct PlanCounters {
                uint64_t term_bytes = 0, term_bytes_dense = 0, term_bytes_fused = 0, term_bytes_planes = 0, term_bytes_phrase_hits = 0, term_bytes_pset = 0, term_bytes_probe = 0,
                         cand_needed_term_bytes = 0;
                uint64_t dense_queries = 0, pset_queries = 0, probe_queries = 0, cand_queries = 0, fused_queries = 0, planes_queries = 0, tree_queries = 0;
                uint64_t bitmap_queries = 0;
                uint64_t pscatter_queries = 0, pscatter_docs = 0;
                uint64_t cand_lead_docs = 0, cand_terms = 0;
                uint64_t probe_demoted = 0, probe_demoted_bytes = 0;
                uint32_t sparse_cap = 0;
                uint32_t rich_R = 0;
                uint64_t rich_wide_queries = 0;
                bool rich_allow = false;
                void merge(const PlanCounters &o) {
                        term_bytes += o.term_bytes, term_bytes_dense += o.term_bytes_dense, term_bytes_fused += o.term_bytes_fused, term_bytes_planes += o.term_bytes_planes;
                        term_bytes_phrase_hits += o.term_bytes_phrase_hits, term_bytes_pset += o.term_bytes_pset, term_bytes_probe += o.term_bytes_probe;
                        cand_needed_term_bytes += o.cand_needed_term_bytes;
                        dense_queries += o.dense_queries, pset_queries += o.pset_queries, probe_queries += o.probe_queries, cand_queries += o.cand_queries;
                        fused_queries += o.fused_queries, planes_queries += o.planes_queries, tree_queries += o.tree_queries;
                        bitmap_queries += o.bitmap_queries, pscatter_queries += o.pscatter_queries, pscatter_docs += o.pscatter_docs;
                        cand_lead_docs += o.cand_lead_docs, cand_terms += o.cand_terms;
                        probe_demoted += o.probe_demoted, probe_demoted_bytes += o.probe_demoted_bytes;
                        sparse_cap = std::max(sparse_cap, o.sparse_cap);
                        rich_R = std::max(rich_R, o.rich_R);
                        rich_wide_queries += o.rich_wide_queries;
                        rich_allow |= o.rich_allow;
                }
        };
}

struct BatchPlan : trip::PlanCounters {
        uint8_t *block = nullptr;
        size_t block_bytes = 0;
        Span<DevQuery> plan;
        Span<uint32_t> qterms;
        Span<DevTask> tasks;
        Span<uint32_t> sched;
        Span<DevFused> fused;
        Span<uint32_t> qplane;
        Span<uint32_t> plane_terms;
        Span<uint32_t> splane;
        Span<uint32_t> sterms;
        Span<double> sweights;
        Span<DevPhrase> phrases;
        Span<uint32_t> pterms, ptasks;
        Span<DevPsetUnit> units;
        Span<uint32_t> pset_sched;
        Span<uint32_t> cand_q;
        Span<uint32_t> tree;
        Span<uint32_t> tree_terms;
        Span<uint32_t> tree_hidden;
        Span<DevRichWide> rich_wide;
        Span<uint32_t> rich_sched;
        uint32_t n_rich_wide = 0;
        uint64_t rich_wide_cells = 0, rich_wide_slots = 0;
        uint32_t n_tree = 0;
        uint32_t n_tree_wide = 0;
        uint64_t tree_scratch_bytes = 0;
        std::vector<uint32_t> slot_of_query;
        std::vector<int32_t> qstatus;
        uint32_t n_dense = 0, n_pset = 0, n_probe = 0, n_cand = 0, n_fused = 0, n_fused16 = 0, n_fusedgen = 0, n_planes = 0, n_planes8 = 0;
        uint32_t plw = 0;
        uint32_t plane_rows = 0;
        uint64_t out_capacity = 0;
        uint64_t plane_decoded_bytes = 0, unsupported_queries = 0;
        uint64_t distinct_bytes = 0, distinct_bytes_kind[TASK_KINDS + 1] = {};
        std::string last_unsupported;
        double plan_ms[4] = {0, 0, 0, 0};
};

namespace trip {
        constexpr size_t SECTION_ALIGN = 64;
        struct SectionCounts {
                size_t plan = 0, qterms = 0, tasks = 0, fused = 0, qplane = 0, plane_terms = 0, splane = 0, sterms = 0, sweights = 0, phrases = 0, pterms = 0, ptasks = 0, units = 0,
                       tree = 0, tree_terms = 0, tree_hidden = 0, rich_wide = 0, rich_sched = 0;
        };
        template <class Plan, class Fn>
        inline void for_each_section(Plan &P, const SectionCounts &n, Fn &&fn) {
                fn(P.plan, n.plan);
                fn(P.qterms, n.qterms);
                fn(P.tasks, n.tasks);
                fn(P.sched, n.tasks);
                fn(P.fused, n.fused);
                fn(P.qplane, n.qplane);
                fn(P.plane_terms, n.plane_terms);
                fn(P.splane, n.splane);
                fn(P.sterms, n.sterms);
                fn(P.sweights, n.sweights);
                fn(P.phrases, n.phrases);
                fn(P.pterms, n.pterms);
                fn(P.ptasks, n.ptasks);
                fn(P.units, n.units);
                fn(P.pset_sched, n.units);
                fn(P.cand_q, (size_t)CAND_QUEUES + 1);
                fn(P.tree, n.tree);
                fn(P.tree_terms, n.tree_terms);
                fn(P.tree_hidden, n.tree_hidden);
                if (n.rich_wide) {
                        fn(P.rich_wide, n.rich_wide);
                        fn(P.rich_sched, n.rich_sched);
                }
        }
        inline size_t layout_sections(BatchPlan &P, const SectionCounts &n) {
                size_t bytes = 0;
                for_each_section(P, n, [&](auto &s, const size_t count) {
                        s.off = bytes;
                        s.n = count;
                        bytes += (count * sizeof(*s.p) + SECTION_ALIGN + SECTION_ALIGN - 1) & ~(SECTION_ALIGN - 1);
                });
                return bytes;
        }
        inline void point_sections(BatchPlan &P, const SectionCounts &n) {
                for_each_section(P, n, [&](auto &s, size_t) { s.p = reinterpret_cast<std::remove_reference_t<decltype(*s.p)> *>(P.block + s.off); });
        }

        constexpr uint32_t SCHED_NB = 64 * 4;
        constexpr uint32_t CAND_SUBS = 128, CAND_COST_SUBS = 16;
        constexpr uint32_t PSET_RANGE_BKS = 64, PSET_SUBS = 64;
        constexpr uint32_t CAND_KEY0 = TASK_KINDS * SCHED_NB, PSET_KEY0 = CAND_KEY0 + CAND_QUEUES * CAND_SUBS, SCHED_KEYS = PSET_KEY0 + PSET_RANGE_BKS * PSET_SUBS;
        inline uint32_t pset_sub(const uint32_t rank) { return rank < PSET_SUBS / 2 ? rank : std::min(PSET_SUBS / 2 + (rank - PSET_SUBS / 2) / 8, PSET_SUBS - 1); }
        constexpr uint64_t CAND_ROWS_MIN_LEAD = 1024;
        constexpr uint32_t SCHED_RANK[TASK_KINDS] = {3, 0, 4, 5, 6, 7, 8, 1, 2, 9};
        constexpr uint32_t BatchPlan::*const SCHED_COUNT[TASK_KINDS] = {&BatchPlan::n_cand, &BatchPlan::n_dense, &BatchPlan::n_fused, &BatchPlan::n_fused16, &BatchPlan::n_fusedgen,
                                                                        &BatchPlan::n_planes, &BatchPlan::n_planes8, &BatchPlan::n_pset, &BatchPlan::n_probe, &BatchPlan::n_tree};
        inline uint32_t sched_first(const BatchPlan &P, const uint32_t kind) {
                uint32_t at = 0;
                for (uint32_t k = 0; k < TASK_KINDS; ++k)
                        if (SCHED_RANK[k] < SCHED_RANK[kind])
                                at += P.*SCHED_COUNT[k];
                return at;
        }
        inline uint32_t cost_bucket(const uint64_t cost) {
                const uint64_t c = std::max<uint64_t>(1, cost);
                const uint32_t lg = 63u - (uint32_t)__builtin_clzll(c);
                const uint32_t frac = lg >= 2 ? (uint32_t)((c >> (lg - 2)) & 3u) : (uint32_t)((c << (2 - lg)) & 3u);
                return lg * 4 + frac;
        }
        inline uint32_t sched_key(const uint32_t kind, const uint64_t cost) {
                if (kind == TASK_PSET)
                        return SCHED_RANK[TASK_PSET] * SCHED_NB + (uint32_t)std::min<uint64_t>((cost & 0xffffffffull) / PSET_TASK_WINDOWS, SCHED_NB - 1);
                return SCHED_RANK[kind] * SCHED_NB + (SCHED_NB - 1 - cost_bucket(cost));
        }

        struct PNode {
                uint32_t op = 0, term = 0;
                uint32_t tok = 0;
                uint32_t kid_off = 0, kid_n = 0;
                uint64_t cost = 0;
                bool empty = false;
        };

        struct Scratch {
                std::vector<PNode> nodes;
                std::vector<int> kidpool, st, tmpk;
                std::vector<uint64_t> cs;
                std::vector<uint32_t> gt, gs;
                std::vector<uint32_t> gorder, leaves, leaf_tok, negs, opts, opt_tok, ts, ts_tok, u, uniq, rt, seen, phterms, slots;
                struct PhraseTmp {
                        uint32_t t0, n;
                        double weight;
                };
                std::vector<PhraseTmp> qphrases;
                std::vector<std::pair<uint32_t, double>> sc;
                const int *kids(const PNode &x) const { return kidpool.data() + x.kid_off; }
        };

        struct Tmp {
                DevQuery q;
                uint64_t cost;
                uint32_t nlead;
                int32_t fz;
                bool truth;
                bool tree;
                bool hidden;
                uint64_t tree_ub;
                bool tree_wide;
                uint32_t hidden_ord;
                uint64_t sumdf, lead_docs;
                uint32_t last_doc;
                bool dense, fuse;
        };

        struct QUse {
                uint32_t qpos, term;
        };
        struct FUse {
                uint32_t fidx, slot, term;
        };

        struct Frag : PlanCounters {
                size_t q_lo = 0, q_hi = 0;
                Scratch S;
                std::vector<Tmp> tmp;
                std::vector<uint32_t> qterms, pterms, sterms;
                std::vector<double> sweights;
                std::vector<DevPhrase> phrases;
                std::vector<DevFused> fz;
                std::vector<size_t> left_out;
                uint64_t onepass_queries = 0, fused_postings = 0, phrase_queries = 0;
                std::vector<DevTask> tasks;
                std::vector<uint64_t> tcost;
                std::vector<DevFused> fused;
                std::vector<uint32_t> ptasks;
                std::vector<DevPsetUnit> units;
                std::vector<QUse> quses, suses;
                std::vector<FUse> fuses;
                std::vector<uint64_t> benefit;
                std::vector<uint64_t> cand_row;
                std::vector<uint32_t> keys, hist;
                std::vector<uint32_t> treepool;
                std::vector<uint32_t> tree_terms;
                uint32_t n_hidden = 0;
                uint64_t off = 0;
                size_t b_plan = 0, b_qterms = 0, b_sterms = 0, b_phrases = 0, b_pterms = 0, b_tasks = 0, b_fused = 0, b_ptasks = 0, b_units = 0, b_tree = 0, b_hidden = 0;
                uint64_t b_off = 0;
                int rc = TRI_OK;
                std::string err;
                void recycle() {
                        Frag fresh;
                        auto keep = [](auto &dst, auto &src) {
                                src.clear();
                                dst = std::move(src);
                        };
                        keep(fresh.S.nodes, S.nodes), keep(fresh.S.kidpool, S.kidpool), keep(fresh.S.st, S.st), keep(fresh.S.tmpk, S.tmpk), keep(fresh.S.cs, S.cs);
                        keep(fresh.S.gt, S.gt), keep(fresh.S.gs, S.gs), keep(fresh.S.gorder, S.gorder), keep(fresh.S.leaves, S.leaves), keep(fresh.S.leaf_tok, S.leaf_tok);
                        keep(fresh.S.negs, S.negs), keep(fresh.S.opts, S.opts), keep(fresh.S.opt_tok, S.opt_tok), keep(fresh.S.ts, S.ts), keep(fresh.S.ts_tok, S.ts_tok);
                        keep(fresh.S.u, S.u), keep(fresh.S.uniq, S.uniq), keep(fresh.S.rt, S.rt), keep(fresh.S.seen, S.seen), keep(fresh.S.phterms, S.phterms);
                        keep(fresh.S.slots, S.slots), keep(fresh.S.qphrases, S.qphrases), keep(fresh.S.sc, S.sc);
                        keep(fresh.tmp, tmp), keep(fresh.qterms, qterms), keep(fresh.pterms, pterms), keep(fresh.sterms, sterms), keep(fresh.sweights, sweights);
                        keep(fresh.phrases, phrases), keep(fresh.fz, fz), keep(fresh.left_out, left_out), keep(fresh.tasks, tasks), keep(fresh.tcost, tcost);
                        keep(fresh.fused, fused), keep(fresh.ptasks, ptasks), keep(fresh.units, units), keep(fresh.quses, quses), keep(fresh.suses, suses);
                        keep(fresh.fuses, fuses), keep(fresh.benefit, benefit), keep(fresh.cand_row, cand_row), keep(fresh.keys, keys), keep(fresh.hist, hist), keep(fresh.treepool, treepool);
                        keep(fresh.tree_terms, tree_terms);
                        *this = std::move(fresh);
                }
        };
        struct FragCache {
                std::vector<Frag> frags;
        };

        struct Ctx {
                const HostIndex &ix;
                const PlanEnv &env;
                const PlanInput &in;
                bool scored, rich;
                uint32_t mode;
                uint32_t n_ok = 0;
                bool plane_ok(uint32_t term) const { return ix.df_rank[term] < n_ok; }
                uint64_t planes_split = 2, fused_task_cost = 0, phrase_task_div = 1;
                uint32_t plw = 0;
                double term_weight(const uint32_t df) const {
                        if (in.similarity == TRI_SIM_TFIDF)
                                return std::log((double)((uint64_t)ix.info.docs_cnt + 1) / (double)(df + 1)) + 1.0;
                        if (in.similarity == TRI_SIM_TRIVIAL)
                                return 0.0;
                        const float num = (float)((uint64_t)ix.info.docs_cnt - (uint64_t)df) + 0.5f;
                        const float den = (float)df + 0.5f;
                        return (double)std::log(1 + num / den);
                }
                uint32_t first_block_ge(const DevTerm &t, const uint64_t key) const {
                        if (t.win_off != 0xffffffffu && !ix.win.empty() && !(key & (CELL_DOCS - 1)) && (key >> CELL_LOG2) < ix.nwin)
                                return ix.win[t.win_off + (key >> CELL_LOG2)];
                        const uint32_t *lb = &ix.blk_last[t.first_block];
                        return (uint32_t)(std::lower_bound(lb, lb + t.nblocks, (uint32_t)std::min<uint64_t>(key, 0xffffffffull)) - lb);
                }
        };

        inline uint64_t distinct_docbytes(const HostIndex &ix, const uint32_t *terms, const size_t n, std::vector<uint32_t> &seen) {
                uint64_t bytes = 0;
                seen.clear();
                for (size_t k = 0; k < n; ++k) {
                        const uint32_t term = terms[k] & QT_TERM;
                        if (std::find(seen.begin(), seen.end(), term) == seen.end()) {
                                seen.push_back(term);
                                bytes += ix.docbytes[term];
                        }
                }
                return bytes;
        }
        inline DevPsetUnit make_unit(const DevQuery &q, const uint32_t *qt, const uint32_t tix, const uint32_t begin, const uint32_t end, const uint64_t out_off, const uint32_t first) {
                DevPsetUnit u{};
                u.out_off = out_off;
                u.first = first;
                u.w_begin = begin, u.w_end = end;
                u.tix = tix;
                u.nterms = q.nterms;
                u.term_base = q.term_base;
                for (uint32_t k = 0; k < q.nterms && k < PSET_INLINE_TERMS; ++k)
                        u.tt[k] = qt[k];
                return u;
        }
        template <class Fn>
        inline void for_each_term_token(const HostIndex &ix, const PlanInput &in, const size_t q, Fn &&fn) {
                const tri_query &t = in.queries[q];
                if ((uint64_t)t.prog_off + t.prog_len > in.prog_len)
                        return;
                for (uint32_t i = 0; i < t.prog_len && i < 16; ++i) {
                        const uint32_t tok = in.prog[t.prog_off + i];
                        const uint32_t x = tok & 0x0fffffffu;
                        if ((tok >> 28) == TRI_OP_TERM && x < ix.terms.size())
                                fn(x);
                }
        }
        inline void prefetch_term(const HostIndex &ix, const uint32_t x) {
                __builtin_prefetch(&ix.terms[x]);
                __builtin_prefetch(&ix.docbytes[x]);
                __builtin_prefetch(&ix.df_rank[x]);
        }

        inline double ms_since(std::chrono::steady_clock::time_point &t0) {
                const auto now = std::chrono::steady_clock::now();
                const double ms = std::chrono::duration<double, std::milli>(now - t0).count();
                t0 = now;
                return ms;
        }
}
```

### trinity_amd/csrc/trinity_hip.hip

```cpp
#include "../../include/trinity_hip.h"
#include <chrono>
#include <hip/hip_runtime.h>

#include <algorithm>
#include <array>
#include <cmath>
#include <cstdarg>
#include <cstdio>
#include <cstring>
#include <ctime>
#include <unistd.h>
#include <dlfcn.h>
#include <memory>
#include <mutex>
#include <numeric>
#include <string>
#include <thread>
#include <unordered_map>
#include <functional>
#include <vector>

static thread_local char g_err[512] = "";
static int fail(int code, const char *fmt, ...) {
        va_list ap;
// ... 278 lines not shown
        DevMem<uint64_t> d_hashes;
        Pooled<uint32_t> d_part_docs;
        Pooled<double> d_part_scores, d_all_scores;
        Pooled<uint32_t> d_rich_present;
        Pooled<uint16_t> d_rich_freq;
        Pooled<uint16_t> d_rich_freq_wide;
        Pooled<uint32_t> d_rich_present_hi, d_rich_allow_hi;
        DevMem<uint16_t> d_rich_pool;
        DevMem<uint8_t> d_rich_plen;
        DevMem<uint64_t> d_rich_payload;
        Pooled<double> d_pscore;
        Pooled<uint32_t> d_tree_scratch;
        Pooled<double> d_tree_scores;
        Pooled<uint32_t> d_scat_docs;
        Pooled<uint8_t> d_filter_tab;
        Pooled<uint32_t> d_filter_rows;
        Pooled<uint8_t> d_rank_block;
        template <class T>
        T *dev_at(const Span<T> &s) const {
                return reinterpret_cast<T *>(d_arena + s.off);
        }
        template <class T>
        T *dev_opt(const Span<T> &s) const {
                return s.empty() ? nullptr : dev_at(s);
        }
        uint32_t *d_counts = nullptr;
        uint32_t *d_ticket = nullptr;
        uint32_t *d_build = nullptr;
        unsigned long long *d_qthr = nullptr;
        uint32_t *d_part_counts = nullptr;
        uint32_t *d_score_order = nullptr;
        uint32_t *d_task_hits = nullptr;
        uint64_t *d_task_pos_base = nullptr;
        uint32_t *d_scat_off = nullptr, *d_scat_cnt = nullptr;
        uint32_t *d_scat_list = nullptr;
        uint64_t *d_qcounts = nullptr;
        uint32_t *d_top_counts = nullptr, *d_top_docs = nullptr;
        float *d_top_scores = nullptr;
        uint32_t *d_tree_rows = nullptr, *d_tree_prows = nullptr, *d_tree_qbits = nullptr, *d_tree_cc = nullptr, *d_tree_build = nullptr;
        double *d_rank_w = nullptr, *d_rank_part_scores = nullptr, *d_rank_scores = nullptr;
        uint32_t *d_rank_part_docs = nullptr, *d_rank_part_counts = nullptr, *d_rank_docs = nullptr, *d_rank_counts = nullptr;
        uint32_t scat_cap = 0;
        bool ran = false;
        bool planes_hi = false;
        std::vector<uint64_t> h_task_pos_base;
        size_t rich_pool_cap = 0;
        std::vector<uint32_t> h_counts;
        std::vector<uint64_t> h_query_counts;
        bool synced = false;
        std::vector<const tri_filter *> filter_rows;
        size_t filter_rows_cap = 0;
        bool rank_on = false, rank_done = false;
        tri_ranker rank{};
        std::vector<uint32_t> h_prog;
        std::vector<tri_query> h_queries;
        tri_batch_info info{};
        ~tri_batch() {
                if (!dev)
                        return;
                hipSetDevice(dev->device);
                if (ran && !synced)
                        hipStreamSynchronize(dev->stream);
                if (ev[EV_UP])
                        hipEventSynchronize(ev[EV_UP]);
        }
};


#include "dev_stream.hpp"
#include "k_decode.hpp"
#include "k_match.hpp"
#include "k_score.hpp"
#include "k_fused.hpp"
#include "k_planes.hpp"
#include "k_psets.hpp"
#include "k_probe.hpp"
#include "k_encode.hpp"
#include "k_phrase.hpp"
#include "k_rich.hpp"
#include "k_rich_rank.hpp"
#include "k_decode_hits.hpp"
#include "k_isect.hpp"
#include "k_tree.hpp"
#include "k_tree_wide.hpp"
#include "k_perc.hpp"
#include "k_commit.hpp"
#include "k_lencode.hpp"
#include "filtered_kernels.hpp"

template <class Pick, class... Args>
static void tri_launch(const int codec, Pick pick, const dim3 grid, const dim3 block, const hipStream_t stream, Args &&...args) {
        if (codec == TRI_CODEC_LUCENE)
                hipLaunchKernelGGL(pick(std::integral_constant<int, CODEC_LUCENE>()), grid, block, 0, stream, std::forward<Args>(args)...);
        else
                hipLaunchKernelGGL(pick(std::integral_constant<int, CODEC_GOOGLE>()), grid, block, 0, stream, std::forward<Args>(args)...);
}
#define TRI_LAUNCH(K, codec, grid, block, stream, ...) tri_launch(codec, [](auto c_) { return K<c_.value>; }, grid, block, stream, __VA_ARGS__)

extern "C" int tri_dev_open(int device, tri_dev **out) {
        if (!out)
                return fail(TRI_ERR_INVALID, "tri_dev_open: null out");
        int n = 0;
        HIP_TRY(hipGetDeviceCount(&n));
        if (device < 0 || device >= n)
                return fail(TRI_ERR_INVALID, "tri_dev_open: device %d out of range (%d devices)", device, n);
        HIP_TRY(hipSetDevice(device));
        auto d = std::make_unique<tri_dev>();
        d->device = device;
        HIP_TRY(hipStreamCreateWithFlags(&d->stream, hipStreamNonBlocking));
        HIP_TRY(hipStreamCreateWithFlags(&d->stream2, hipStreamNonBlocking));
        HIP_TRY(hipStreamCreateWithFlags(&d->stream_up, hipStreamNonBlocking));
        HIP_TRY(hipStreamCreateWithFlags(&d->stream_rb, hipStreamNonBlocking));
        HIP_TRY(hipEventCreateWithFlags(&d->ev_fork, hipEventDisableTiming));
        HIP_TRY(hipEventCreateWithFlags(&d->ev_join, hipEventDisableTiming));
        hipDeviceProp_t prop;
        HIP_TRY(hipGetDeviceProperties(&prop, device));
        d->cus = prop.multiProcessorCount;
        *out = d.release();
        return TRI_OK;
}

extern "C" void tri_dev_close(tri_dev *d) {
        if (!d)
                return;
        if (d->refs > 0) {
                d->closing = true;
                return;
        }
        dev_destroy(d);
}

namespace {
        uint64_t *option_slot(tri_options &o, const char *name) {
                static const struct {
                        const char *name;
                        uint64_t tri_options::*field;
                } table[] = {{"dense_min_postings", &tri_options::dense_min_postings}, {"dense_task_cost", &tri_options::dense_task_cost},
                             {"fused", &tri_options::fused},
                             {"fused_task_cost", &tri_options::fused_task_cost},
                             {"fused_freq_cap", &tri_options::fused_freq_cap},
                             {"fused_halfwords", &tri_options::fused_halfwords},
                             {"account_needed_bytes", &tri_options::account_needed_bytes},
                             {"overlap_dense_wgs", &tri_options::overlap_dense_wgs},
                             {"overlap_cand_wgs", &tri_options::overlap_cand_wgs},
                             {"overlap", &tri_options::overlap},
                             {"planes", &tri_options::planes},
                             {"plane_div", &tri_options::plane_div},
                             {"planes_split", &tri_options::planes_split},
                             {"plane_max_bytes", &tri_options::plane_max_bytes},
                             {"plane_amortize", &tri_options::plane_amortize},
                             {"planes_rebuild", &tri_options::planes_rebuild},
                             {"cand_xcd", &tri_options::cand_xcd},
                             {"plan_threads", &tri_options::plan_threads},
                             {"probe_max_blocks", &tri_options::probe_max_blocks}, {"phrase_task_div", &tri_options::phrase_task_div}, {"plan_hot_us", &tri_options::plan_hot_us}, {"plan_pin", &tri_options::plan_pin}, {"planes_order", &tri_options::planes_order}, {"pset_order", &tri_options::pset_order}, {"scatter_bitmap_slack", &tri_options::scatter_bitmap_slack}, {"tree_max_bytes", &tri_options::tree_max_bytes}, {"tree_max_nodes", &tri_options::tree_max_nodes}, {"tree_wide_min_nodes", &tri_options::tree_wide_min_nodes}, {"rich_max_terms", &tri_options::rich_max_terms}, {"result_bitmaps", &tri_options::result_bitmaps}, {"cand_task_cost", &tri_options::cand_task_cost}, {"dense_window_cost", &tri_options::dense_window_cost},
                             {"isect_max_bytes", &tri_options::isect_max_bytes}, {"isect_max_masks", &tri_options::isect_max_masks}, {"isect_max_runs", &tri_options::isect_max_runs},
                             {"perc_max_bytes", &tri_options::perc_max_bytes}, {"perc_prune", &tri_options::perc_prune}};
                for (const auto &e : table)
                        if (!strcmp(e.name, name))
                                return &(o.*(e.field));
                return nullptr;
        }
}

extern "C" int tri_dev_set_option(tri_dev *d, const char *name, uint64_t value) {
        if (!d || !name)
                return fail(TRI_ERR_INVALID, "tri_dev_set_option: null argument");
        uint64_t *slot = option_slot(d->opt, name);
        if (!slot)
                return fail(TRI_ERR_INVALID, "tri_dev_set_option: unknown option '%s'", name);
        *slot = value;
        return TRI_OK;
}

extern "C" int tri_dev_get_option(tri_dev *d, const char *name, uint64_t *value) {
        if (!d || !name || !value)
                return fail(TRI_ERR_INVALID, "tri_dev_get_option: null argument");
        if (!strcmp(name, "rich_write_last_us") || !strcmp(name, "rank_last_us")) {
                *value = !strcmp(name, "rich_write_last_us") ? d->rich_write_last_us : d->rank_last_us;
                return TRI_OK;
        }
        if (!strcmp(name, "crank_merge_last_us")) {
                *value = d->crank_merge_last_us;
                return TRI_OK;
        }
        const uint64_t *slot = option_slot(d->opt, name);
        if (!slot)
                return fail(TRI_ERR_INVALID, "tri_dev_get_option: unknown option '%s'", name);
        *value = *slot;
        return TRI_OK;
}

extern "C" int tri_dev_memory(tri_dev *d, tri_dev_memory_info *out) {
        if (!d || !out)
                return fail(TRI_ERR_INVALID, "tri_dev_memory: null argument");
        HIP_TRY(hipSetDevice(d->device));
        size_t fr = 0, total = 0;
        HIP_TRY(hipMemGetInfo(&fr, &total));
        DevLock g(d->mu);
        uint64_t all = 0, pinned = 0;
        for (const auto &kv : d->pool.size_of)
                all += kv.second;
        for (const auto &pb : d->pinned_idle)
                pinned += pb.first;
        out->pool_idle_bytes = d->pool.idle_bytes;
        out->pool_in_use_bytes = all - d->pool.idle_bytes;
        out->pinned_idle_bytes = pinned;
        out->device_free_bytes = fr;
        out->device_total_bytes = total;
        return TRI_OK;
}

extern "C" int tri_dev_sync(tri_dev *d) {
        if (!d)
                return fail(TRI_ERR_INVALID, "null dev");
        HIP_TRY(hipStreamSynchronize(d->stream));
        return TRI_OK;
}

extern "C" void *tri_dev_stream(tri_dev *d) { return d ? (void *)d->stream : nullptr; }

namespace {
        template <class T>
        int dev_upload(DevMem<T> &dst, const std::vector<T> &src, size_t extra = 0) {
                HIP_TRY(dst.alloc((src.size() + extra) * sizeof(T) + 16));
                if (!src.empty())
                        HIP_TRY(hipMemcpy(dst, src.data(), src.size() * sizeof(T), hipMemcpyHostToDevice));
                return TRI_OK;
        }
}

extern "C" int tri_index_upload(tri_dev *dev, const uint8_t *index, size_t len, const uint8_t *hits, size_t hits_len, int codec,
                                const tri_term *terms, size_t nterms, uint32_t docs_cnt, tri_index **out) {
        if (!dev || !out || (!index && len) || (!terms && nterms) || (!hits && hits_len))
                return fail(TRI_ERR_INVALID, "tri_index_upload: null argument");
        HIP_TRY(hipSetDevice(dev->device));
        auto ix = std::make_unique<tri_index>();
        {
                std::string err;
                if (const int rc = build_host_index(index, len, hits, hits_len, codec, terms, nterms, docs_cnt, *ix, err))
                        return fail(rc, "%s", err.c_str());
        }
        ix->dev.retain(dev);
        if (!ix->dev_index.empty()) {
                index = ix->dev_index.data();
                len = ix->dev_index.size();
                hits = ix->dev_hits.empty() ? nullptr : ix->dev_hits.data();
                hits_len = ix->dev_hits.size();
        }
        int rc;
        if ((rc = dev_upload(ix->d_win, ix->win, 3 * CELLS_PER_SPAN + 8)))
                return rc;
        HIP_TRY(hipMemset(ix->d_win + ix->win.size(), 0, (3 * CELLS_PER_SPAN + 8) * sizeof(uint32_t)));
        HIP_TRY(ix->d_index.alloc(len + 256));
        HIP_TRY(hipMemset(ix->d_index, 0, len + 256));
        if (len)
                HIP_TRY(hipMemcpy(ix->d_index, index, len, hipMemcpyHostToDevice));
        if ((rc = dev_upload(ix->d_blk_last, ix->blk_last)) || (rc = dev_upload(ix->d_blk_off, ix->blk_off)) || (rc = dev_upload(ix->d_terms, ix->terms)))
                return rc;
        if (codec == TRI_CODEC_GOOGLE) {
                ix->blk_doff.push_back((uint32_t)ix->dstream.size() + 1);
                ix->dstream.resize(ix->dstream.size() + 256, 0);
                if ((rc = dev_upload(ix->d_dstream, ix->dstream)) || (rc = dev_upload(ix->d_blk_doff, ix->blk_doff)))
                        return rc;
        }
        if (hits_len) {
                HIP_TRY(ix->d_hits.alloc(hits_len + 256));
                HIP_TRY(hipMemset(ix->d_hits, 0, hits_len + 256));
                HIP_TRY(hipMemcpy(ix->d_hits, hits, hits_len, hipMemcpyHostToDevice));
                if (ix->has_hdir && ((rc = dev_upload(ix->d_blk_hits, ix->blk_hits)) || (rc = dev_upload(ix->d_hdir, ix->hdir))))
                        return rc;
        }
        if (codec == TRI_CODEC_GOOGLE && (rc = dev_upload(ix->d_blk_hits, ix->blk_hits)))
                return rc;
        if (codec == TRI_CODEC_LUCENE) {
                static_assert(sizeof(RowRec) == sizeof(uint4), "row records are read as uint4");
                HIP_TRY(ix->d_blk_rec.alloc(ix->blk_rec.size() * sizeof(uint4) + 16));
                if (!ix->blk_rec.empty())
                        HIP_TRY(hipMemcpy(ix->d_blk_rec, ix->blk_rec.data(), ix->blk_rec.size() * sizeof(uint4), hipMemcpyHostToDevice));
        }
        ix->release_device_columns();
        *out = ix.release();
        return TRI_OK;
}


extern "C" int tri_index_set_masked(tri_index *ix, const uint32_t *docids, size_t n) {
        if (!ix || (!docids && n))
                return fail(TRI_ERR_INVALID, "tri_index_set_masked: null argument");
        HIP_TRY(hipSetDevice(ix->dev->device));
        HIP_TRY(hipStreamSynchronize(ix->dev->stream));
        if (!n) {
                ix->d_masked.reset();
                return TRI_OK;
        }
        const size_t words = ((size_t)ix->max_doc / SPAN_BITS + 2) * (SPAN_BITS / 32);
        std::vector<uint32_t> bm(words, 0);
        for (size_t i = 0; i < n; ++i)
                if (docids[i] <= ix->max_doc)
                        bm[docids[i] >> 5] |= 1u << (docids[i] & 31);
        if (!ix->d_masked)
                HIP_TRY(ix->d_masked.alloc(words * 4));
        HIP_TRY(hipMemcpy(ix->d_masked, bm.data(), words * 4, hipMemcpyHostToDevice));
        return TRI_OK;
}

extern "C" void tri_index_destroy(tri_index *ix) {
        delete ix;
// ... 545 lines not shown
        b->dev.retain(dev);
        b->flags = flags;
        b->topk = topk;
        b->similarity = similarity;
        b->nq = nq;
        const PlanInput in{prog, prog_len, queries, nq, weights, flags, topk, similarity};
        if (const int rc = create_plan(b.get(), in))
                return rc;
        dbg_lap(0);
        DevLock dev_lock(dev->mu);
        if (const int rc = create_arena(b.get()))
                return rc;
        dbg_lap(1);
        if (const int rc = create_buffers(b.get(), in, dbg_lap))
                return rc;
        HIP_TRY(hipEventRecord(b->ev[EV_UP], dev->stream_up));
        create_info(b.get());
        b->info.create_ms = (float)std::chrono::duration<double, std::milli>(std::chrono::steady_clock::now() - t_create).count();
        if (dbg_create)
                fprintf(stderr, "[tri create] nq %zu: plan %.3f  arena+copy %.3f  planes/sparse %.3f  out(%.1f MB) %.3f  rest %.3f  total %.3f ms\n", nq, dbg_t[0], dbg_t[1] - dbg_t[0],
                        dbg_t[2] - dbg_t[1], (double)b->out_capacity * 4 / 1e6, dbg_t[3] - dbg_t[2], b->info.create_ms - dbg_t[3], b->info.create_ms);
        *out = b.release();
        return TRI_OK;
}

extern "C" void tri_batch_destroy(tri_batch *b) {
        delete b;
}


static FilterSel filter_sel(const tri_batch *b) {
        if (b->filter_rows.empty())
                return FilterSel{nullptr, nullptr, nullptr, 0u};
        return FilterSel{b->d_filter_rows, (const uint32_t *)b->d_filter_tab.get(), b->dev_at(b->tasks), (uint32_t)filter_words(b->ix)};
}
template <class F>
struct FilteredKernel;
template <class... A>
struct FilteredKernel<void (*)(A...)> {
        using type = void (*)(A..., FilterSel);
};
template <class Pick, class... Args>
static void tri_launch_matching(const tri_batch *b, const int kernel, const int variant, Pick pick, const dim3 grid, const dim3 block, const hipStream_t stream, Args &&...args) {
        const FilterSel fsel = filter_sel(b);
        if (!fsel.rows)
                return tri_launch(b->ix->codec, pick, grid, block, stream, std::forward<Args>(args)...);
        using Plain = decltype(+pick(std::integral_constant<int, CODEC_GOOGLE>()));
        const auto twin = reinterpret_cast<typename FilteredKernel<Plain>::type>(const_cast<void *>(filtered_kernel(kernel, b->ix->codec == TRI_CODEC_LUCENE ? CODEC_LUCENE : CODEC_GOOGLE, variant)));
        hipLaunchKernelGGL(twin, grid, block, 0, stream, std::forward<Args>(args)..., fsel);
}
static size_t filter_tab_ptrs_off(const tri_batch *b) { return (b->plan.size() * 4 + 15) & ~(size_t)15; }

static int run_filter_rows(tri_batch *b) {
        if (b->filter_rows.empty())
                return TRI_OK;
        tri_dev *dev = b->dev;
        const size_t n4 = filter_words(b->ix) / 4;
        const uint32_t nrows = (uint32_t)b->filter_rows.size();
        for (uint32_t y0 = 0; y0 < nrows; y0 += 65535u) {
                hipLaunchKernelGGL(k_filter_rows, dim3((unsigned)std::min<size_t>((n4 + FILTER_WG - 1) / FILTER_WG, 1024), std::min(65535u, nrows - y0)), dim3(FILTER_WG), 0, dev->stream,
                                   (const uint4 *const *)(b->d_filter_tab + filter_tab_ptrs_off(b)) + y0, (const uint4 *)b->ix->d_masked.get(), (uint4 *)b->d_filter_rows.get() + (size_t)y0 * n4, n4);
                HIP_TRY(hipGetLastError());
        }
        return TRI_OK;
}

static int run_plane_rows(tri_batch *b) {
        tri_dev *dev = b->dev;
        tri_index *ix = b->ix;
        b->info.term_planes_decoded_bytes = 0;
        if (!b->plane_terms.empty()) {
                std::vector<uint32_t> build;
                const uint8_t needs = b->planes_hi ? 3u : 1u;
                for (const uint32_t term : b->plane_terms) {
                        const uint32_t row = ix->df_rank[term];
                        if (row < ix->pc_cap && ((ix->pc_built[row] & needs) != needs || dev->opt.planes_rebuild)) {
                                build.push_back(term);
                                build.push_back(row);
                                b->info.term_planes_decoded_bytes += ix->docbytes[term];
                        }
                }
                if (!build.empty()) {
                        HIP_TRY(hipMemcpyAsync(b->d_build, build.data(), build.size() * 4, hipMemcpyHostToDevice, dev->stream));
                        const uint32_t nrows = (uint32_t)(build.size() / 2), nwin = b->plw / PL_WORDS;
                        for (uint32_t y0 = 0; y0 < nrows; y0 += 65535u) {
                                const uint32_t ny = std::min(65535u, nrows - y0);
                                if (b->planes_hi)
                                        TRI_LAUNCH(k_term_planes, ix->codec, dim3(nwin, ny), dim3(AND_WG), dev->stream, ix->d_index, ix->d_blk_last, ix->d_blk_off, ix->d_blk_rec,
                                                   ix->d_blk_doff, ix->d_win, ix->d_terms, (const uint32_t *)b->d_build + 2 * (size_t)y0, ix->d_pcache, (size_t)b->plw, ix->d_pcache_hi,
                                                   (size_t)PL_HI * b->plw, b->plw, (uint32_t *)nullptr);
                                else
                                        TRI_LAUNCH(k_term_plane0, ix->codec, dim3((nwin + P0_GROUP - 1) / P0_GROUP, ny), dim3(AND_WG), dev->stream, ix->d_index, ix->d_blk_last, ix->d_blk_off,
                                                   ix->d_blk_rec, ix->d_blk_doff, ix->d_win, ix->d_terms, (const uint32_t *)b->d_build + 2 * (size_t)y0, ix->d_pcache, b->plw, (uint32_t *)nullptr);
                                HIP_TRY(hipGetLastError());
                        }
                        for (size_t i = 1; i < build.size(); i += 2)
                                ix->pc_built[build[i]] |= needs;
                }
        }
        HIP_TRY(hipEventRecord(b->ev[EV_PLANE_ROWS], dev->stream));
        return TRI_OK;
}

static int run_matching(tri_batch *b) {
        tri_dev *dev = b->dev;
        tri_index *ix = b->ix;
        const uint8_t *match_bytes = ix->codec == TRI_CODEC_GOOGLE ? ix->d_dstream : ix->d_index;
        const uint32_t *match_off = ix->codec == TRI_CODEC_GOOGLE ? ix->d_blk_doff : ix->d_blk_off;
        uint32_t dense_wgs = TRI_DENSE_WAVES * 256 / DENSE_WG, cand_wgs = 4;
        bool overlap = false;
        if (dev->opt.overlap_dense_wgs && dev->opt.overlap_cand_wgs && (b->n_dense || b->n_pset) && b->n_cand) {
                overlap = true;
                dense_wgs = (uint32_t)dev->opt.overlap_dense_wgs;
                cand_wgs = (uint32_t)dev->opt.overlap_cand_wgs;
        } else if (dev->opt.overlap && b->n_cand && trip::sched_first(*b, TASK_CAND))
                overlap = true;
        hipStream_t cand_stream = dev->stream;
        if (overlap) {
                HIP_TRY(hipEventRecord(dev->ev_fork, dev->stream));
                HIP_TRY(hipStreamWaitEvent(dev->stream2, dev->ev_fork, 0));
                cand_stream = dev->stream2;
        }
        const DevPsetUnit *units = b->dev_at(b->units);
        const uint32_t *pset_sched = b->dev_at(b->pset_sched);
        const FilterSel fsel = filter_sel(b);
        const bool prep = b->n_pset && b->pscatter_queries, prep_forked = prep && !overlap && b->n_dense;
        if (prep) {
                if (prep_forked) {
                        HIP_TRY(hipEventRecord(dev->ev_fork, dev->stream));
                        HIP_TRY(hipStreamWaitEvent(dev->stream2, dev->ev_fork, 0));
                }
                hipStream_t prep_stream = prep_forked ? dev->stream2 : dev->stream;
                const uint32_t nunits = b->n_pset + b->n_probe, nscat = (uint32_t)b->pscatter_queries;
                hipLaunchKernelGGL(k_psets_prep_list, dim3((nunits + 255) / 256), dim3(256), 0, prep_stream, units, nunits, b->d_ticket + TICKET_SCAT_WORD + 1, b->d_scat_list, nscat);
                HIP_TRY(hipGetLastError());
                TRI_LAUNCH(k_psets_prep, ix->codec, dim3(nscat), dim3(PSCAT_WG), prep_stream, units, (const uint32_t *)b->d_scat_list, (const uint32_t *)(b->d_ticket + TICKET_SCAT_WORD + 1),
                           b->dev_at(b->plan), b->dev_at(b->tasks), (const uint32_t *)b->dev_at(b->qterms), (const uint32_t *)b->dev_opt(b->qplane), ix->d_masked, ix->d_index, ix->d_blk_last, ix->d_blk_off, ix->d_blk_rec,
                           ix->d_blk_doff, ix->d_terms, b->d_ticket + TICKET_SCAT_WORD, b->d_scat_off, b->d_scat_cnt, b->d_scat_docs, b->scat_cap, fsel);
                HIP_TRY(hipGetLastError());
                if (prep_forked)
                        HIP_TRY(hipEventRecord(dev->ev_join, dev->stream2));
        }
        if (b->n_dense) {
                tri_launch_matching(b, FK_AND_DENSE, 0, [](auto c) { return k_and_dense<c.value>; }, dim3(std::min<uint32_t>(b->n_dense, (uint32_t)dev->cus * dense_wgs)), dim3(DENSE_WG), dev->stream, match_bytes, ix->d_blk_last,
                           match_off, ix->d_win, ix->d_terms, b->dev_at(b->plan), b->dev_at(b->tasks), b->dev_at(b->sched) + trip::sched_first(*b, TASK_DENSE), b->dev_at(b->qterms), b->n_dense,
                           b->d_ticket + TICKET_DENSE_WORD, b->d_out, b->d_counts, ix->d_masked, (const uint32_t *)b->dev_opt(b->qplane), (const uint32_t *)ix->d_pcache, b->plw);
                HIP_TRY(hipGetLastError());
        }
        HIP_TRY(hipEventRecord(b->ev[EV_DENSE], dev->stream));
        if (prep_forked)
                HIP_TRY(hipStreamWaitEvent(dev->stream, dev->ev_join, 0));
        if (b->n_pset) {
                const uint32_t pset_wgs = TRI_PSET_WAVES * 256 / PSET_WG;
                tri_launch_matching(b, FK_PSETS, 0, [](auto c) { return k_psets<c.value>; }, dim3(std::min<uint32_t>(b->n_pset, (uint32_t)dev->cus * (overlap && dev->opt.overlap_dense_wgs ? std::min<uint32_t>(dense_wgs, pset_wgs) : pset_wgs))),
                           dim3(PSET_WG), dev->stream, units, pset_sched, b->n_pset, b->d_ticket + TICKET_PSET_WORD, (const uint32_t *)b->dev_at(b->qterms), (const uint32_t *)b->dev_opt(b->qplane), b->d_out,
                           b->d_counts, ix->d_masked, (const uint32_t *)ix->d_pcache, b->plw, (const uint32_t *)b->d_scat_off, (const uint32_t *)b->d_scat_cnt,
                           (const uint32_t *)b->d_scat_docs);
                HIP_TRY(hipGetLastError());
        }
        HIP_TRY(hipEventRecord(b->ev[EV_PSET], dev->stream));
        if (b->n_probe) {
                tri_launch_matching(b, FK_PROBE, 0, [](auto c) { return k_probe<c.value>; }, dim3(std::min<uint32_t>((b->n_probe + PROBE_WG / 64 - 1) / (PROBE_WG / 64), (uint32_t)dev->cus * (TRI_PROBE_WAVES * 256 / PROBE_WG))),
                           dim3(PROBE_WG), dev->stream, match_bytes, ix->d_blk_last, match_off, ix->d_terms, units, pset_sched + b->n_pset, b->n_probe, b->d_ticket + TICKET_PROBE_WORD,
                           (const uint32_t *)b->dev_at(b->qterms), (const uint32_t *)b->dev_opt(b->qplane), b->d_out, b->d_counts, ix->d_masked, (const uint32_t *)ix->d_pcache, b->plw);
                HIP_TRY(hipGetLastError());
        }
        HIP_TRY(hipEventRecord(b->ev[EV_PROBE], dev->stream));
        if (b->n_cand)
                tri_launch_matching(b, FK_AND, 0, [](auto c) { return k_and<c.value>; }, dim3(std::min<uint32_t>(b->n_cand, (uint32_t)dev->cus * cand_wgs)), dim3(AND_WG), cand_stream, match_bytes, ix->d_blk_last, match_off,
                           ix->d_win, ix->d_terms, b->dev_at(b->plan), b->dev_at(b->tasks), b->dev_at(b->sched) + trip::sched_first(*b, TASK_CAND), b->dev_at(b->qterms), b->dev_at(b->cand_q),
                           b->d_ticket + TICKET_CAND_WORD, b->d_out, b->d_counts, ix->d_masked, (const uint32_t *)b->dev_opt(b->qplane), (const uint32_t *)ix->d_pcache, b->plw);
        HIP_TRY(hipGetLastError());
        if (overlap) {
                HIP_TRY(hipEventRecord(dev->ev_join, dev->stream2));
                HIP_TRY(hipStreamWaitEvent(dev->stream, dev->ev_join, 0));
        }
        HIP_TRY(hipEventRecord(b->ev[EV_CAND], dev->stream));
        return TRI_OK;
}

static int run_fused(tri_batch *b) {
        tri_dev *dev = b->dev;
        tri_index *ix = b->ix;
        for (uint32_t kind = TASK_FUSED; kind <= TASK_FUSED_GEN; ++kind) {
                const uint32_t nf = b->*trip::SCHED_COUNT[kind], variant = kind - TASK_FUSED;
                if (!nf)
                        continue;
                tri_launch_matching(b, FK_FUSED, (int)variant, [&](auto c) { return std::array{k_fused<c.value, 0, 0>, k_fused<c.value, 1, 0>, k_fused<c.value, 0, 1>}[variant]; },
                           dim3(std::min<uint32_t>(nf, (uint32_t)dev->cus * FUS_WGS_PER_CU)), dim3(FUS_WG), dev->stream, ix->d_index, ix->d_blk_last, ix->d_blk_off, ix->d_blk_rec,
                           ix->d_blk_doff, ix->d_win, ix->d_terms, b->dev_at(b->plan), b->dev_at(b->fused), b->dev_at(b->tasks), (const uint32_t *)b->dev_at(b->sched) + trip::sched_first(*b, kind), b->dev_at(b->sterms),
                           b->dev_at(b->sweights), nf, b->d_ticket + TICKET_FUSED_WORD + 2 * variant, b->d_counts, b->topk, b->d_part_docs, b->d_part_scores, b->d_part_counts, ix->d_masked,
                           b->similarity, b->d_out, b->d_all_scores, b->d_rich_allow);
                HIP_TRY(hipGetLastError());
        }
        HIP_TRY(hipEventRecord(b->ev[EV_FUSED], dev->stream));
        return TRI_OK;
}

static int run_planes(tri_batch *b) {
        tri_dev *dev = b->dev;
        tri_index *ix = b->ix;
        if (b->d_qthr)
                HIP_TRY(hipMemsetAsync(b->d_qthr, 0, (b->plan.size() + 1) * 8, dev->stream));
        for (uint32_t kind = TASK_PLANES; kind <= TASK_PLANES8; ++kind) {
                const uint32_t np = b->*trip::SCHED_COUNT[kind], wide = kind - TASK_PLANES;
                if (!np)
                        continue;
                tri_launch_matching(b, FK_PLANES, (int)wide, [&](auto c) { return wide ? k_planes<c.value, FUS_MAX_SLOTS> : k_planes<c.value, PLK_NS_SMALL>; },
                           dim3(std::min<uint32_t>(np, (uint32_t)dev->cus * PLK_WGS_PER_CU)), dim3(PLK_WG), dev->stream, ix->d_index, ix->d_blk_last, ix->d_blk_off, ix->d_blk_rec,
                           ix->d_blk_doff, ix->d_win, ix->d_terms, b->dev_at(b->plan), b->dev_at(b->fused), b->dev_at(b->tasks), (const uint32_t *)b->dev_at(b->sched) + trip::sched_first(*b, kind), b->dev_at(b->sterms),
                           b->dev_at(b->sweights), np, b->d_ticket + TICKET_PLANES_WORD + 2 * wide, b->d_counts, b->topk, b->d_part_docs, b->d_part_scores, b->d_part_counts, ix->d_masked,
                           b->similarity, (const uint32_t *)ix->d_pcache, (const uint32_t *)ix->d_pcache_hi, b->plw, ix->pc_cap, b->d_sparse, b->sparse_cap, b->d_qthr);
                HIP_TRY(hipGetLastError());
        }
        HIP_TRY(hipEventRecord(b->ev[EV_PLANES], dev->stream));
        return TRI_OK;
}

static int run_phrases(tri_batch *b) {
        tri_dev *dev = b->dev;
        tri_index *ix = b->ix;
        if (!b->ptasks.empty() && ix->codec == TRI_CODEC_GOOGLE && ix->d_prank && ix->pc_cap) {
                std::vector<uint32_t> hits_build, hits_only;
                uint32_t max_blocks = 0;
                for (size_t i = 0; i < b->pterms.size(); ++i) {
                        const uint32_t term = b->pterms[i], r = ix->df_rank[term];
                        if (r >= ix->pc_cap || ix->ph_built[r])
                                continue;
                        const DevTerm &t = ix->terms[term];
                        if (!(t.flags & TERM_FULL_BLOCKS) || !t.documents)
                                continue;
                        ix->ph_built[r] = 1;
                        max_blocks = std::max(max_blocks, t.nblocks);
                        std::vector<uint32_t> &dst = (ix->pc_built[r] & 4u) ? hits_only : hits_build;
                        ix->pc_built[r] |= 5u;
                        dst.push_back(term);
                        dst.push_back(r);
                }
                const uint32_t nrows_build = (uint32_t)(hits_build.size() / 2);
                hits_build.insert(hits_build.end(), hits_only.begin(), hits_only.end());
                if (!hits_build.empty()) {
                        uint32_t *d_pairs = ix->d_ph_pairs + 2 * ix->ph_pairs_n;
                        HIP_TRY(hipMemcpyAsync(d_pairs, hits_build.data(), hits_build.size() * 4, hipMemcpyHostToDevice, dev->stream));
                        ix->ph_pairs_n += hits_build.size() / 2;
                        for (uint32_t y0 = 0; y0 < nrows_build; y0 += 65535u) {
                                const dim3 grid((b->plw / PL_WORDS + P0_GROUP - 1) / P0_GROUP, std::min(65535u, nrows_build - y0));
                                TRI_LAUNCH(k_term_plane0, ix->codec, grid, dim3(AND_WG), dev->stream, ix->d_index, ix->d_blk_last, ix->d_blk_off, ix->d_blk_rec, ix->d_blk_doff, ix->d_win,
                                           ix->d_terms, (const uint32_t *)d_pairs + 2 * (size_t)y0, ix->d_pcache, b->plw, ix->d_prank);
                                HIP_TRY(hipGetLastError());
                        }
                        const uint32_t npairs = (uint32_t)(hits_build.size() / 2);
                        for (uint32_t y0 = 0; y0 < npairs; y0 += 65535u) {
                                hipLaunchKernelGGL(k_term_hits, dim3((max_blocks + 255) / 256, std::min(65535u, npairs - y0)), dim3(256), 0, dev->stream, ix->d_index, ix->d_blk_off,
                                                   ix->d_blk_hits, ix->d_terms, (const uint32_t *)d_pairs + 2 * (size_t)y0, (const uint64_t *)ix->d_hs_off, ix->d_phs, ix->d_term_row);
                                HIP_TRY(hipGetLastError());
                        }
                }
        }
        if (!b->ptasks.empty()) {
                const uint32_t np = (uint32_t)b->ptasks.size();
                TRI_LAUNCH(k_phrase, ix->codec, dim3(std::min<uint32_t>(np, (uint32_t)dev->cus * PHRASE_WGS_PER_CU)), dim3(AND_WG), dev->stream, ix->d_index, ix->d_hits,
                           ix->d_blk_hits, ix->d_hdir, ix->d_blk_last, ix->d_blk_off, ix->d_win, ix->d_terms, b->dev_at(b->plan), b->dev_at(b->tasks), b->dev_at(b->ptasks), np, b->dev_at(b->phrases), b->dev_at(b->pterms),
                           b->d_ticket + TICKET_PHRASE_WORD, b->d_out, b->d_counts, b->d_pscore,
                           (b->flags & TRI_FLAG_ACCUMULATED_SCORE) ? 65535u : 1u,
                           b->similarity, (const uint32_t *)ix->d_pcache, ix->pc_plw, (const uint32_t *)ix->d_prank, (const unsigned long long *)ix->d_phs,
                           (const uint64_t *)ix->d_hs_off, ix->codec == TRI_CODEC_GOOGLE ? (const uint32_t *)ix->d_term_row : nullptr);
                HIP_TRY(hipGetLastError());
        }
        HIP_TRY(hipEventRecord(b->ev[EV_PHRASE], dev->stream));
        return TRI_OK;
}

static int run_trees(tri_batch *b) {
        tri_dev *dev = b->dev;
        tri_index *ix = b->ix;
        if (b->n_tree) {
                const uint32_t plw = b->plw, nterms = (uint32_t)b->tree_terms.size(), nhid = (uint32_t)b->tree_hidden.size();
                const uint32_t nchunks = (plw + TREE_CHUNK_WORDS - 1) / TREE_CHUNK_WORDS;
                const uint32_t *tsched = b->dev_at(b->sched) + trip::sched_first(*b, TASK_TREE);
                const uint32_t *d_tree = b->dev_at(b->tree);
                for (uint32_t y0 = 0; y0 < nterms; y0 += 65535u) {
                        const dim3 grid(plw / PL_WORDS, std::min(65535u, nterms - y0));
                        TRI_LAUNCH(k_term_planes, ix->codec, grid, dim3(AND_WG), dev->stream, ix->d_index, ix->d_blk_last, ix->d_blk_off, ix->d_blk_rec, ix->d_blk_doff, ix->d_win,
                                   ix->d_terms, (const uint32_t *)b->d_tree_build + 2 * (size_t)y0, b->d_tree_rows, (size_t)PL_PLANES * plw, b->d_tree_rows + plw,
                                   (size_t)PL_PLANES * plw, plw, (uint32_t *)nullptr);
                        HIP_TRY(hipGetLastError());
                }
                if (nhid) {
                        HIP_TRY(hipMemsetAsync(b->d_tree_prows, 0, (size_t)nhid * plw * 4, dev->stream));
                        hipLaunchKernelGGL(k_tree_gather, dim3(nhid), dim3(TREE_WG), 0, dev->stream, b->dev_at(b->plan), b->dev_at(b->tasks), b->dev_at(b->tree_hidden), b->d_out,
                                           b->d_counts, b->d_pscore, b->d_tree_prows, plw);
                        HIP_TRY(hipGetLastError());
                }
                const bool scored_run = b->flags & TRI_FLAG_ACCUMULATED_SCORE, rich_run = b->flags & TRI_FLAG_MATCHED_TERMS;
                double *tscores = !scored_run ? nullptr : b->topk ? (double *)b->d_tree_scores : (double *)b->d_all_scores;
                const uint32_t n_narrow = b->n_tree - b->n_tree_wide;
                for (uint32_t y0 = 0; y0 < b->n_tree;) {
                        const bool wide = y0 >= n_narrow;
                        const uint32_t ny = std::min(65535u, (wide ? b->n_tree : n_narrow) - y0);
                        const dim3 grid(nchunks, ny);
                        uint32_t *qbits = b->d_tree_qbits + (size_t)y0 * plw, *cc = b->d_tree_cc + (size_t)y0 * nchunks;
#define TREE_EVAL_ARGS b->dev_at(b->plan), b->dev_at(b->tasks), tsched + y0, d_tree, (const uint32_t *)b->d_tree_rows, (const uint32_t *)b->d_tree_prows, (const uint32_t *)ix->d_masked, qbits, cc, plw, filter_sel(b)
                        if (wide)
                                hipLaunchKernelGGL(k_tree_eval_wide, grid, dim3(TREE_WG), 0, dev->stream, TREE_EVAL_ARGS);
                        else
                                hipLaunchKernelGGL(k_tree_eval, grid, dim3(TREE_WG), 0, dev->stream, TREE_EVAL_ARGS);
#undef TREE_EVAL_ARGS
                        hipLaunchKernelGGL(k_tree_expand, grid, dim3(TREE_WG), 0, dev->stream, b->dev_at(b->plan), b->dev_at(b->tasks), tsched + y0, (const uint32_t *)qbits, (const uint32_t *)cc,
// ... 1109 lines not shown
```

### trinity_amd/hostplan.py

```python
import ctypes as C

import numpy as np

from .engine import TrinityError, flatten, host_lib

_SUMMARY = ["block_bytes", "n_plan", "n_qterms", "n_tasks", "n_fused_maps", "n_qplane", "n_plane_terms", "n_sterms", "n_sweights", "n_phrases", "n_pterms", "n_ptasks",
            "off_plan", "off_qterms", "off_tasks", "off_sched", "off_fused", "off_qplane", "off_plane_terms", "off_sterms", "off_sweights", "off_phrases", "off_pterms", "off_ptasks",
            "n_dense", "n_cand", "n_fused", "n_fused16", "n_fusedgen", "n_planes", "n_planes8", "plw", "sparse_cap", "out_capacity", "term_bytes", "term_bytes_dense",
            "dense_queries", "cand_queries", "fused_queries", "planes_queries", "unsupported_queries", "rich_R", "sizeof_query", "sizeof_task", "sizeof_fused", "sizeof_phrase",
            "cand_needed_term_bytes", "plane_decoded_bytes", "n_pset", "pset_queries", "n_probe", "probe_queries", "n_units", "off_units", "off_unit_sched", "sizeof_unit",
            "n_tree", "tree_queries", "n_tree_words", "off_tree", "n_tree_terms", "off_tree_terms", "n_tree_hidden", "off_tree_hidden", "off_cand_q"]

DEV_QUERY = np.dtype([("nterms", "<u4"), ("term_base", "<u4"), ("out_off", "<u8"), ("out_cap", "<u4"), ("qid", "<u4"), ("first_task", "<u4"), ("ntasks", "<u4"),
                      ("score_base", "<u4"), ("nscore", "<u4"), ("phrase_base", "<u4"), ("nphrases", "<u4"), ("fused_idx", "<u4"), ("form", "<u4")])
DEV_TASK = np.dtype([("slot", "<u4"), ("begin", "<u4"), ("end", "<u4"), ("kind", "<u4"), ("out_off", "<u8")])
TASK_CAND, TASK_DENSE, TASK_FUSED, TASK_FUSED16, TASK_FUSED_GEN, TASK_PLANES, TASK_PLANES8, TASK_PSET, TASK_PROBE, TASK_TREE = range(10)
DEV_TREE_NODE = np.dtype([("op", "u1"), ("parent", "u1"), ("ord", "u1"), ("thr", "u1"), ("arg", "<u4"), ("row", "<u4"), ("score", "<u4"), ("rmask", "<u4"),
                          ("kid0", "u1"), ("kid1", "u1"), ("pad", "u1", 2), ("kids", "<u8")])
TREE_HDR_WORDS = 8
DEV_TREE_NODE_WIDE = np.dtype([("op", "u1"), ("cbits", "u1"), ("parent", "<u2"), ("arg", "<u4"), ("row", "<u4"), ("score", "<u4"), ("rmask", "<u4"),
                               ("ord", "<u2"), ("nkids", "<u2"), ("thr", "<u2"), ("pop", "u1"), ("pcbits", "u1"), ("pad", "<u4")])
TREE_KIND_NARROW, TREE_KIND_WIDE = 0, 1
DEV_RICH_WIDE = np.dtype([("cells", "<u8"), ("slots", "<u8"), ("stride", "<u4"), ("pad", "<u4")])
_RICH_WIDE = ["n_rich_wide_tab", "off_rich_wide", "off_rich_sched", "n_rich_wide", "rich_wide_cells", "rich_wide_slots", "sizeof_rich_wide"]
TREE_NO_PARENT = 0xFFFF
DEV_UNIT = np.dtype([("out_off", "<u8"), ("begin", "<u4"), ("end", "<u4"), ("tix", "<u4"), ("nterms", "<u4"), ("term_base", "<u4"), ("first", "<u4"), ("tt", "<u4", 4), ("row", "<u4", 4)])
SCHED_ORDER = [TASK_DENSE, TASK_PSET, TASK_PROBE, TASK_CAND, TASK_FUSED, TASK_FUSED16, TASK_FUSED_GEN, TASK_PLANES, TASK_PLANES8, TASK_TREE]


def _lib():
    L = host_lib()
    if not hasattr(L, "_plan_ready"):
        vp = C.c_void_p
        L.tri_host_index_build.restype = vp
        L.tri_host_index_build.argtypes = [vp, C.c_uint64, vp, C.c_uint64, C.c_int, vp, C.c_uint64, C.c_uint32, C.c_char_p, C.c_uint64]
        L.tri_host_index_free.argtypes = [vp]
        L.tri_host_plan.restype = vp
        L.tri_host_plan.argtypes = [vp, vp, C.c_uint64, vp, C.c_uint64, C.c_uint32, C.c_uint32, C.c_int, C.c_uint, vp, vp, C.c_uint, C.c_uint32, C.c_char_p, C.c_uint64]
        L.tri_host_plan_free.argtypes = [vp]
        L.tri_host_plan_summary.argtypes = [vp, vp, vp]
        L.tri_host_plan_block.restype = C.POINTER(C.c_uint8)
        L.tri_host_plan_block.argtypes = [vp]
        L.tri_host_plan_query_maps.argtypes = [vp, vp, vp]
        L.tri_host_plan_last_unsupported.argtypes = [vp, C.c_char_p, C.c_uint64]
        L.tri_host_plan_last_unsupported.restype = None
        L.tri_host_plan_rich_wide.argtypes = [vp, vp]
        L.tri_host_plan_rich_wide.restype = None
        L.tri_host_pfor128_group.argtypes = [vp, vp, C.POINTER(C.c_uint32), vp, C.POINTER(C.c_uint32)]
        L.tri_host_pfor128_group.restype = None
        for f in (L.tri_host_lucene_encode, L.tri_host_lucene_encode_units):
            f.argtypes = [vp, vp, vp, vp, C.c_uint64, vp, C.c_uint64, C.POINTER(C.c_uint64), vp, C.c_uint64, C.POINTER(C.c_uint64), vp]
        L._plan_ready = True
    return L


class HostIndex:
    def __init__(self, index_bytes, terms, docs_cnt, codec=1, hits=None):
        b = np.ascontiguousarray(index_bytes, dtype=np.uint8)
        t = np.ascontiguousarray(terms, dtype=np.uint32).reshape(-1, 3)
        h = np.ascontiguousarray(hits, dtype=np.uint8) if hits is not None and len(hits) else None
        err = C.create_string_buffer(600)
        self.h = _lib().tri_host_index_build(b.ctypes.data, b.size, h.ctypes.data if h is not None else None, h.size if h is not None else 0, codec, t.ctypes.data, t.shape[0],
                                             docs_cnt, err, 600)
        if not self.h:
            raise TrinityError(err.value.decode())

    @classmethod
    def from_segment(cls, seg):
        return cls(seg.index, seg.terms, seg.docs_cnt, codec=seg.codec, hits=seg.hits)

    def hits_dir(self, term):
        L = _lib()
        L.tri_host_index_hits_dir.restype = C.c_uint32
        L.tri_host_index_hits_dir.argtypes = [C.c_void_p, C.c_uint32, C.c_void_p, C.POINTER(C.c_uint32)]
        nfull = C.c_uint32()
        n = L.tri_host_index_hits_dir(self.h, term, None, C.byref(nfull))
        out = np.zeros(max(1, n), dtype=np.uint32)
        L.tri_host_index_hits_dir(self.h, term, out.ctypes.data, C.byref(nfull))
        return out[:n], nfull.value

    def close(self):
        if self.h:
            _lib().tri_host_index_free(self.h)
            self.h = None

    def __del__(self):
        self.close()


class HostPlan:

    def __init__(self, hindex, programs, flags, topk=0, similarity=0, threads=1, options=None, cus=256, flat=None):
        self.nq = len(programs) if flat is None else flat[1].shape[0]
        prog, q = flatten(programs) if flat is None else flat
        options = options or {}
        names = (C.c_char_p * max(1, len(options)))(*[k.encode() for k in options])
        values = np.array(list(options.values()) or [0], dtype=np.uint64)
        err = C.create_string_buffer(600)
        self.h = _lib().tri_host_plan(hindex.h, prog.ctypes.data, prog.size, q.ctypes.data, self.nq, flags, topk, similarity, threads, names, values.ctypes.data, len(options), cus,
                                      err, 600)
        if not self.h:
            raise TrinityError(err.value.decode())
        out = np.zeros(len(_SUMMARY), dtype=np.uint64)
        ms = np.zeros(4, dtype=np.float64)
        _lib().tri_host_plan_summary(self.h, out.ctypes.data, ms.ctypes.data)
        self.s = {k: int(v) for k, v in zip(_SUMMARY, out)}
        self.ms = ms
        wide = np.zeros(len(_RICH_WIDE), dtype=np.uint64)
        _lib().tri_host_plan_rich_wide(self.h, wide.ctypes.data)
        self.s.update({k: int(v) for k, v in zip(_RICH_WIDE, wide)})
        assert self.s["sizeof_rich_wide"] == DEV_RICH_WIDE.itemsize
        assert self.s["sizeof_query"] == DEV_QUERY.itemsize and self.s["sizeof_task"] == DEV_TASK.itemsize
        p = _lib().tri_host_plan_block(self.h)
        self.block = np.ctypeslib.as_array(p, shape=(max(1, self.s["block_bytes"]),)).copy()
        self.slot_of_query = np.zeros(max(1, self.nq), dtype=np.uint32)
        self.qstatus = np.zeros(max(1, self.nq), dtype=np.int32)
        _lib().tri_host_plan_query_maps(self.h, self.slot_of_query.ctypes.data, self.qstatus.ctypes.data)
        why = C.create_string_buffer(600)
        _lib().tri_host_plan_last_unsupported(self.h, why, 600)
        self.last_unsupported = why.value.decode()

    def _view(self, off, n, dtype):
        dt = np.dtype(dtype)
        return self.block[self.s[off] : self.s[off] + n * dt.itemsize].view(dt)

    @property
    def plan(self):
        return self._view("off_plan", self.s["n_plan"], DEV_QUERY)

    @property
    def tasks(self):
        return self._view("off_tasks", self.s["n_tasks"], DEV_TASK)

    @property
    def sched(self):
        return self._view("off_sched", self.s["n_tasks"], "<u4")

    @property
    def units(self):
        return self._view("off_units", self.s["n_units"], DEV_UNIT)

    @property
    def unit_sched(self):
        return self._view("off_unit_sched", self.s["n_pset"] + self.s["n_probe"], "<u4")

    @property
    def cand_q(self):
        return self._view("off_cand_q", 9, "<u4")

    @property
    def qterms(self):
        return self._view("off_qterms", self.s["n_qterms"], "<u4")

    @property
    def qplane(self):
        return self._view("off_qplane", self.s["n_qplane"], "<u4")

    @property
    def plane_terms(self):
        return self._view("off_plane_terms", self.s["n_plane_terms"], "<u4")

    @property
    def tree_terms(self):
        return self._view("off_tree_terms", self.s["n_tree_terms"], "<u4")

    @property
    def tree_hidden(self):
        return self._view("off_tree_hidden", self.s["n_tree_hidden"], "<u4")

    @property
    def rich_wide(self):
        return self._view("off_rich_wide", self.s["n_rich_wide_tab"], DEV_RICH_WIDE)

    @property
    def rich_sched(self):
        return self._view("off_rich_sched", self.s["n_tasks"] if self.s["n_rich_wide_tab"] else 0, "<u4")

    def leaf_report_mask(self, slot, node):
        if self.tree_kind(slot)[0] == TREE_KIND_WIDE:
            nd = self.tree_nodes_wide(slot)[node]
            return int(nd["rmask"]) | (int(nd["pad"]) << 32)
        nd = self.tree_nodes(slot)[node]
        return int(nd["rmask"]) | ((int(nd["kids"]) & 0xFFFFFFFF) << 32)

    def tree_nodes(self, slot):
        words = self._view("off_tree", self.s["n_tree_words"], "<u4")
        at = int(self.plan[slot]["fused_idx"])
        n = int(words[at])
        return words[at + TREE_HDR_WORDS : at + TREE_HDR_WORDS + 8 * n].view(DEV_TREE_NODE)

    def tree_kind(self, slot):
        words = self._view("off_tree", self.s["n_tree_words"], "<u4")
        at = int(self.plan[slot]["fused_idx"])
        return int(words[at + 1]), int(words[at])

    def tree_header(self, slot):
        words = self._view("off_tree", self.s["n_tree_words"], "<u4")
        at = int(self.plan[slot]["fused_idx"])
        return words[at : at + TREE_HDR_WORDS]

    def tree_nodes_wide(self, slot):
        assert self.tree_kind(slot)[0] == TREE_KIND_WIDE
        return self.tree_nodes(slot).view(DEV_TREE_NODE_WIDE)

    def close(self):
        if self.h:
            self.block = None
            _lib().tri_host_plan_free(self.h)
            self.h = None

    def __del__(self):
        self.close()


def pfor128_group_pair(v):
    v = np.ascontiguousarray(v, dtype=np.uint32)
    assert v.size == 128
    a, b = np.zeros(700, dtype=np.uint8), np.zeros(700, dtype=np.uint8)
    al, bl = C.c_uint32(), C.c_uint32()
    _lib().tri_host_pfor128_group(v.ctypes.data, a.ctypes.data, C.byref(al), b.ctypes.data, C.byref(bl))
    return a[: al.value] if al.value != 0xFFFFFFFF else None, b[: bl.value]


def lucene_encode(docs, freqs, positions, term_first, units=False):
    d = np.ascontiguousarray(docs, dtype=np.uint32)
    f = np.ascontiguousarray(freqs, dtype=np.uint32)
    p = np.ascontiguousarray(positions, dtype=np.uint16)
    tf = np.ascontiguousarray(term_first, dtype=np.uint64)
    n = tf.size - 1
    icap, hcap = 128 + 16 * n + 12 * d.size, 128 + 6 * p.size + 8 * n
    io, ho, t3 = np.zeros(icap, dtype=np.uint8), np.zeros(hcap, dtype=np.uint8), np.zeros((max(n, 1), 3), dtype=np.uint32)
    il, hl = C.c_uint64(), C.c_uint64()
    fn = _lib().tri_host_lucene_encode_units if units else _lib().tri_host_lucene_encode
    if fn(d.ctypes.data, f.ctypes.data, p.ctypes.data, tf.ctypes.data, n, io.ctypes.data, icap, C.byref(il), ho.ctypes.data, hcap, C.byref(hl), t3.ctypes.data):
        raise TrinityError("lucene_encode: buffer too small")
    return io[: il.value], ho[: hl.value], t3[:n]


def cpu_budget():
    L = host_lib()
    L.tri_host_cpu_budget.restype = C.c_uint32
    return int(L.tri_host_cpu_budget())


def pool_cpus(threads=16):
    L = host_lib()
    L.tri_host_pool_cpus.restype = C.c_uint32
    L.tri_host_pool_cpus.argtypes = [C.c_uint32, C.c_void_p, C.c_uint32]
    out = np.zeros(256, dtype=np.int32)
    n = L.tri_host_pool_cpus(threads, out.ctypes.data, out.size)
    return out[:n].tolist()
```

Before: 14.64 million.

## Share identical pset tasks across queries, copying leader output to followers

The planner hashes pset query units and groups queries with identical term sets, windows and flags. Only leader tasks are launched. The kernel writes each result word, docid and count to the follower output slots as well, and follower tasks are scheduled past the lead range. This removes redundant intersection work for duplicate queries, at the cost of extra stores, planner hashing and more complex scheduling.

```diff
diff --git a/trinity_amd/csrc/dev_structs.hpp b/trinity_amd/csrc/dev_structs.hpp
--- a/trinity_amd/csrc/dev_structs.hpp
+++ b/trinity_amd/csrc/dev_structs.hpp
@@ -86,6 +86,9 @@
 static_assert(sizeof(DevPsetUnit) == 64, "one cache-line half per unit");
 constexpr uint32_t PSET_UNIT_FIRST = 1u, PSET_UNIT_BITMAP = 2u;
 constexpr uint32_t PSET_UNIT_ROUND_SHIFT = 4, PSET_UNIT_ROUND_MASK = 15u;
+constexpr uint32_t PSET_UNIT_FOL_SHIFT = 8, PSET_UNIT_FOL_MASK = 15u, PSET_UNIT_FOL_AT_SHIFT = 12;
+constexpr uint32_t PSET_GROUP_MAX = PSET_UNIT_FOL_MASK + 1u;
+constexpr uint32_t PSET_FOL_AT_END = 1u << (32 - PSET_UNIT_FOL_AT_SHIFT);
 constexpr uint32_t PSET_ROUND_DOCS = 16384, PSET_STAGE_DOCS = 1024;
 constexpr uint32_t PSET_UNIT_SCATTER = 4u;
 constexpr uint32_t TREE_MAX_NODES = 64;
diff --git a/trinity_amd/csrc/host/plan_host.cpp b/trinity_amd/csrc/host/plan_host.cpp
--- a/trinity_amd/csrc/host/plan_host.cpp
+++ b/trinity_amd/csrc/host/plan_host.cpp
@@ -53,7 +53,7 @@
                                  : n == "fused_task_cost" ? &o.fused_task_cost : n == "fused_freq_cap" ? &o.fused_freq_cap : n == "fused_halfwords" ? &o.fused_halfwords
                                  : n == "account_needed_bytes" ? &o.account_needed_bytes : n == "planes" ? &o.planes : n == "planes_split" ? &o.planes_split
                                  : n == "plane_div" ? &o.plane_div : n == "plane_max_bytes" ? &o.plane_max_bytes : n == "probe_max_blocks" ? &o.probe_max_blocks : n == "tree_max_bytes" ? &o.tree_max_bytes : n == "tree_max_nodes" ? &o.tree_max_nodes : n == "tree_wide_min_nodes" ? &o.tree_wide_min_nodes : n == "result_bitmaps" ? &o.result_bitmaps : n == "cand_task_cost" ? &o.cand_task_cost : n == "dense_window_cost" ? &o.dense_window_cost
-                                 : n == "cand_xcd" ? &o.cand_xcd : n == "planes_order" ? &o.planes_order : n == "pset_order" ? &o.pset_order : n == "scatter_bitmap_slack" ? &o.scatter_bitmap_slack : n == "phrase_task_div" ? &o.phrase_task_div : n == "plane_amortize" ? &o.plane_amortize : n == "rich_max_terms" ? &o.rich_max_terms : nullptr;
+                                 : n == "cand_xcd" ? &o.cand_xcd : n == "planes_order" ? &o.planes_order : n == "pset_order" ? &o.pset_order : n == "share_tasks" ? &o.share_tasks : n == "scatter_bitmap_slack" ? &o.scatter_bitmap_slack : n == "phrase_task_div" ? &o.phrase_task_div : n == "plane_amortize" ? &o.plane_amortize : n == "rich_max_terms" ? &o.rich_max_terms : nullptr;
                 if (!slot) {
                         put_err(err, errcap, "unknown option " + n);
                         return nullptr;
@@ -117,6 +117,11 @@
         const uint64_t v[] = {P.rich_wide.size(), P.rich_wide.off, P.rich_sched.off, P.n_rich_wide, P.rich_wide_cells, P.rich_wide_slots, sizeof(DevRichWide)};
         memcpy(out, v, sizeof v);
 }
+void tri_host_plan_share(void *p, uint64_t *out ) {
+        const BatchPlan &P = static_cast<HostPlan *>(p)->P;
+        const uint64_t v[] = {P.n_pset_lead, (uint64_t)P.n_pset - P.n_pset_lead, 0};
+        memcpy(out, v, sizeof v);
+}
 void tri_host_plan_last_unsupported(void *p, char *out, uint64_t cap) { put_err(out, cap, static_cast<HostPlan *>(p)->P.last_unsupported); }
 const uint8_t *tri_host_plan_block(void *p) { return static_cast<HostPlan *>(p)->P.block; }
 void tri_host_plan_query_maps(void *p, uint32_t *slot_of_query, int32_t *qstatus) {
diff --git a/trinity_amd/csrc/k_psets.hpp b/trinity_amd/csrc/k_psets.hpp
--- a/trinity_amd/csrc/k_psets.hpp
+++ b/trinity_amd/csrc/k_psets.hpp
@@ -21,7 +21,17 @@
         alignas(16) uint32_t cnt[2][PSET_WAVES];
         DevPsetUnit unit[2];
         uint32_t tick[2];
+        uint32_t fol_lo[PSET_GROUP_MAX - 1], fol_hi[PSET_GROUP_MAX - 1];
+        uint32_t fol_tix[PSET_GROUP_MAX - 1];
 };
+#ifdef TRI_FILTERED_KERNELS
+constexpr bool PSET_SHARE = false;
+#else
+constexpr bool PSET_SHARE = true;
+#endif
+__device__ __forceinline__ uint32_t *psets_follower(const PsetShared &sh, uint32_t *const p, const uint32_t m) {
+        return p + (ptrdiff_t)(((uint64_t)uni(sh.fol_hi[m]) << 32) | uni(sh.fol_lo[m]));
+}
 
 #ifndef TRI_PSET_PREFETCH
 #define TRI_PSET_PREFETCH 0
@@ -32,7 +42,8 @@
 };
 template <class BUF, class R, class F>
 __device__ __forceinline__ uint32_t psets_round(PsetShared &sh, R &&request, F &&words, const uint32_t w_origin, const uint32_t w_begin, const uint32_t w_end, uint32_t *__restrict__ qout,
-                                                const bool as_bitmap, const uint32_t lane, const uint32_t wave, const uint32_t par) {
+                                                const bool as_bitmap, const uint32_t lane, const uint32_t wave, const uint32_t par, const uint32_t nfol_) {
+        const uint32_t nfol = PSET_SHARE ? nfol_ : 0u;
         const uint32_t nsub = w_end - w_begin;
         const uint32_t wave0 = w_begin * SPAN_WORDS + wave * nsub * PSET_WORDS + lane * PSET_PER;
         uint32_t *const st = sh.stage[wave];
@@ -55,6 +66,11 @@
                         uint4 *o = (uint4 *)(qout + (word0 - w_origin * SPAN_WORDS));
                         o[0] = make_uint4(acc[0], acc[1], acc[2], acc[3]);
                         o[1] = make_uint4(acc[4], acc[5], acc[6], acc[7]);
+                        for (uint32_t m = 0; m < nfol; ++m) {
+                                uint4 *om = (uint4 *)psets_follower(sh, (uint32_t *)o, m);
+                                om[0] = make_uint4(acc[0], acc[1], acc[2], acc[3]);
+                                om[1] = make_uint4(acc[4], acc[5], acc[6], acc[7]);
+                        }
 #pragma unroll
                         for (uint32_t j = 0; j < PSET_PER; ++j)
                                 lane_cnt += (uint32_t)__popc(acc[j]);
@@ -111,6 +127,11 @@
                 __builtin_amdgcn_wave_barrier();
                 for (uint32_t i = lane; i < fill; i += 64u)
                         qout[base + i] = st[i];
+                for (uint32_t m = 0; m < nfol; ++m) {
+                        uint32_t *const qm = psets_follower(sh, qout, m);
+                        for (uint32_t i = lane; i < fill; i += 64u)
+                                qm[base + i] = st[i];
+                }
                 __builtin_amdgcn_wave_barrier();
         } else {
                 uint32_t o = base;
@@ -142,6 +163,11 @@
                                 __builtin_amdgcn_wave_barrier();
                                 for (uint32_t i = lane; i < T; i += 64u)
                                         qout[o + i] = st[i];
+                                for (uint32_t m = 0; m < nfol; ++m) {
+                                        uint32_t *const qm = psets_follower(sh, qout, m);
+                                        for (uint32_t i = lane; i < T; i += 64u)
+                                                qm[o + i] = st[i];
+                                }
                                 __builtin_amdgcn_wave_barrier();
                                 o += T;
                                 continue;
@@ -155,8 +181,14 @@
                                 const uint32_t wi = 2u * cidx + (lane >> 5);
                                 const bool bit = (st[wi] >> (lane & 31u)) & 1u;
                                 const uint64_t bm = __builtin_amdgcn_ballot_w64(bit);
+                                const uint32_t at = o + __builtin_amdgcn_mbcnt_hi((uint32_t)(bm >> 32), __builtin_amdgcn_mbcnt_lo((uint32_t)bm, 0u)), doc = ((wbase + wi) << 5) + (lane & 31u);
                                 if (bit)
-                                        qout[o + __builtin_amdgcn_mbcnt_hi((uint32_t)(bm >> 32), __builtin_amdgcn_mbcnt_lo((uint32_t)bm, 0u))] = ((wbase + wi) << 5) + (lane & 31u);
+                                        qout[at] = doc;
+                                for (uint32_t m = 0; m < nfol; ++m) {
+                                        uint32_t *const qm = psets_follower(sh, qout, m);
+                                        if (bit)
+                                                qm[at] = doc;
+                                }
                                 o += (uint32_t)__popcll(bm);
                         }
                         __builtin_amdgcn_wave_barrier();
@@ -170,7 +202,7 @@
 #endif
 template <int CODEC>
 __global__ __launch_bounds__(PSET_WG, TRI_PSET_WAVES) void k_psets(const DevPsetUnit *__restrict__ units, const uint32_t *__restrict__ order, const uint32_t ntasks,
-                                                                   uint32_t *__restrict__ ticket, const uint32_t *__restrict__ qterms, const uint32_t *__restrict__ qplane,
+                                                                   const uint32_t *__restrict__ fol, uint32_t *__restrict__ ticket, const uint32_t *__restrict__ qterms, const uint32_t *__restrict__ qplane,
                                                                    uint32_t *__restrict__ out, uint32_t *__restrict__ counts, const uint32_t *__restrict__ masked,
                                                                    const uint32_t *__restrict__ planes, const uint32_t plw, const uint32_t *__restrict__ scat_off,
                                                                    const uint32_t *__restrict__ scat_cnt, const uint32_t *__restrict__ scat_docs TRI_FILTER_ARG) {
@@ -197,6 +229,15 @@
                 const bool as_bitmap = uni(U.first) & PSET_UNIT_BITMAP;
                 TRI_FILTER_TASK_OF(tix);
                 uint32_t *const qout = out + (((uint64_t)uni((uint32_t)(U.out_off >> 32)) << 32) | uni((uint32_t)U.out_off));
+                const uint32_t nfol = PSET_SHARE ? (uni(U.first) >> PSET_UNIT_FOL_SHIFT) & PSET_UNIT_FOL_MASK : 0u;
+                if (nfol) {
+                        if (tid < nfol) {
+                                const DevPsetUnit &F = units[fol[(uni(U.first) >> PSET_UNIT_FOL_AT_SHIFT) + tid]];
+                                const uint64_t d = F.out_off - U.out_off;
+                                sh.fol_lo[tid] = (uint32_t)d, sh.fol_hi[tid] = (uint32_t)(d >> 32), sh.fol_tix[tid] = F.tix;
+                        }
+                        __syncthreads();
+                }
                 uint32_t nwd = 0, nnt = 0xffffffffu;
                 if (wave == 0) {
                         if (nt < ntasks)
@@ -237,7 +278,7 @@
                                             acc[4] &= ~m1.x, acc[5] &= ~m1.y, acc[6] &= ~m1.z, acc[7] &= ~m1.w;
                                     }
                             },
-                            w_begin, wb, min(w_end, wb + round_win), as_bitmap ? qout : qout + produced, as_bitmap, lane, wave, par);
+                            w_begin, wb, min(w_end, wb + round_win), as_bitmap ? qout : qout + produced, as_bitmap, lane, wave, par, nfol);
                 } else
                         for (uint32_t wb = w_begin; wb < w_end; wb += round_win, par ^= 1u)
                         produced += psets_round<PsetNoBuf>(
@@ -290,7 +331,7 @@
                                             acc[4] &= ~m1.x, acc[5] &= ~m1.y, acc[6] &= ~m1.z, acc[7] &= ~m1.w;
                                     }
                             },
-                            w_begin, wb, min(w_end, wb + round_win), as_bitmap ? qout : qout + produced, as_bitmap, lane, wave, par);
+                            w_begin, wb, min(w_end, wb + round_win), as_bitmap ? qout : qout + produced, as_bitmap, lane, wave, par, nfol);
                 if (uni(U.first) & PSET_UNIT_SCATTER) {
                         __syncthreads();
                         const uint32_t off = scat_at, n = scat_n, doc0 = w_begin * SPAN_BITS;
@@ -313,6 +354,8 @@
                 }
                 if (wave == 0) {
                         counts[tix] = produced;
+                        for (uint32_t m = 0; m < nfol; ++m)
+                                counts[uni(sh.fol_tix[m])] = produced;
                         ((uint32_t *)&sh.unit[p ^ 1u])[lane & 15u] = nwd;
                         sh.tick[p ^ 1u] = nt;
                         __builtin_amdgcn_s_waitcnt(0xc07f);
diff --git a/trinity_amd/csrc/planner.hpp b/trinity_amd/csrc/planner.hpp
--- a/trinity_amd/csrc/planner.hpp
+++ b/trinity_amd/csrc/planner.hpp
@@ -41,6 +41,7 @@
                 uint32_t pset_ranges = 0;
                 uint32_t cand_first = 0, cand_qat[CAND_QUEUES] = {};
                 std::vector<uint32_t> unit_of_task;
+                uint32_t pset_fol_first = 0;
                 ~PlanState() {
                         if (!cache)
                                 return;
@@ -338,6 +339,19 @@
                         P.units[f.b_units + i] = u;
                         S.unit_of_task[u.tix] = (uint32_t)(f.b_units + i);
                 }
+                f.task_folpos.clear();
+                for (const PsetQ &q : f.pset_q) {
+                        if (q.lead_frag == UINT32_MAX) {
+                                for (uint32_t k = 0; k < q.ntasks && q.nfol; ++k)
+                                        P.units[f.b_units + q.unit0 + k].first |= q.nfol << PSET_UNIT_FOL_SHIFT | (q.base + k * q.nfol) << PSET_UNIT_FOL_AT_SHIFT;
+                                continue;
+                        }
+                        const PsetQ &l = S.frags[q.lead_frag].pset_q[q.lead_idx];
+                        if (f.task_folpos.empty())
+                                f.task_folpos.assign(f.tasks.size(), UINT32_MAX);
+                        for (uint32_t k = 0; k < q.ntasks; ++k)
+                                f.task_folpos[f.units[q.unit0 + k].tix] = l.base + k * l.nfol + q.rank;
+                }
                 if (S.n.splane) {
                         std::fill(&P.splane.p[f.b_sterms], &P.splane.p[f.b_sterms] + f.sterms.size(), PL_NONE);
                         for (const QUse &u : f.suses)
@@ -390,6 +404,8 @@
                                         return key_planes_order(S, f, i, tk);
                                 break;
                         case TASK_PSET:
+                                if (!f.task_folpos.empty() && f.task_folpos[i] != UINT32_MAX)
+                                        return PSET_FOL_KEY;
                                 if (S.opt.pset_order)
                                         return key_pset_order(S, f, i);
                                 break;
@@ -427,6 +443,11 @@
                         if (r == SCHED_RANK[TASK_PSET] && S.opt.pset_order)
                                 for (uint32_t bk = PSET_KEY0; bk < PSET_KEY0 + std::min(S.pset_ranges, PSET_RANGE_BKS) * PSET_SUBS; ++bk)
                                         place(bk);
+                        if (r == SCHED_RANK[TASK_PSET]) {
+                                S.pset_fol_first = at;
+                                place(PSET_FOL_KEY);
+                                P.n_pset_lead = S.pset_fol_first - before;
+                        }
                         if (r == SCHED_RANK[TASK_CAND])
                                 for (uint32_t bk = CAND_KEY0; bk < PSET_KEY0; ++bk) {
                                         if ((bk - CAND_KEY0) % CAND_SUBS == 0)
@@ -441,12 +462,55 @@
                 S.run([&](unsigned k) {
                         Frag &f = S.frags[k];
                         for (size_t i = 0; i < f.tasks.size(); ++i) {
-                                const uint32_t pos = f.hist[f.keys[i]]++, ti = (uint32_t)(f.b_tasks + i);
+                                const uint32_t pos = f.keys[i] == PSET_FOL_KEY ? S.pset_fol_first + f.task_folpos[i] : f.hist[f.keys[i]]++, ti = (uint32_t)(f.b_tasks + i);
                                 P.sched[pos] = ti;
                                 if (pos >= units_first && pos - units_first < n_units_run)
                                         P.pset_sched[pos - units_first] = S.unit_of_task[ti];
                         }
                 });
+        }
+
+        inline void group_pset_queries(PlanState &S) {
+                if (!S.opt.share_tasks)
+                        return;
+                size_t nq = 0;
+                for (const Frag &f : S.frags)
+                        nq += f.pset_q.size();
+                if (nq < 2)
+                        return;
+                uint32_t mask = 15;
+                while (mask + 1 < 2 * nq)
+                        mask = 2 * mask + 1;
+                std::vector<std::pair<uint32_t, uint32_t>> tab((size_t)mask + 1, {UINT32_MAX, 0u});
+                uint64_t fol_units = 0;
+                for (uint32_t fi = 0; fi < S.frags.size(); ++fi) {
+                        Frag &f = S.frags[fi];
+                        for (uint32_t e = 0; e < f.pset_q.size(); ++e) {
+                                PsetQ &q = f.pset_q[e];
+                                uint32_t at = (uint32_t)(q.hash >> 20) & mask;
+                                for (; tab[at].first != UINT32_MAX && S.frags[tab[at].first].pset_q[tab[at].second].hash != q.hash; at = (at + 1) & mask)
+                                        ;
+                                if (tab[at].first != UINT32_MAX) {
+                                        Frag &lf = S.frags[tab[at].first];
+                                        PsetQ &l = lf.pset_q[tab[at].second];
+                                        const DevPsetUnit &u = f.units[q.unit0], &v = lf.units[l.unit0];
+                                        if (l.nfol + 1 < PSET_GROUP_MAX && fol_units + q.ntasks <= PSET_FOL_AT_END && q.ntasks == l.ntasks && pset_unit_same(u, v) &&
+                                            f.units[q.unit0 + q.ntasks - 1].w_end == lf.units[l.unit0 + l.ntasks - 1].w_end) {
+                                                q.lead_frag = tab[at].first, q.lead_idx = tab[at].second, q.rank = l.nfol++;
+                                                fol_units += q.ntasks;
+                                                continue;
+                                        }
+                                }
+                                tab[at] = {fi, e};
+                        }
+                }
+                uint32_t base = 0;
+                for (Frag &f : S.frags)
+                        for (PsetQ &q : f.pset_q)
+                                if (q.lead_frag == UINT32_MAX && q.nfol) {
+                                        q.base = base;
+                                        base += q.nfol * q.ntasks;
+                                }
         }
 
         inline void split_tree_section(BatchPlan &P) {
@@ -593,6 +657,7 @@
                 return rc;
         choose_planes(S);
         assign_cand_rows(S);
+        group_pset_queries(S);
         if (const int rc = layout_block(S, alloc_block))
                 return rc;
         if (const int rc = S.run_pass("FILL", "filling the plan", [&](Frag &f) {
diff --git a/trinity_amd/csrc/planner_tasks.hpp b/trinity_amd/csrc/planner_tasks.hpp
--- a/trinity_amd/csrc/planner_tasks.hpp
+++ b/trinity_amd/csrc/planner_tasks.hpp
@@ -206,6 +206,7 @@
                 uint64_t heaviest = 0xffffffffull;
                 for (uint32_t k = 0; pset && k < t.q.nterms; ++k)
                         heaviest = std::min<uint64_t>(heaviest, ix.df_rank[qt[k] & QT_TERM]);
+                const size_t unit0 = f.units.size();
                 for (uint32_t wb = 0; wb < nwin; wb += win_per_task, ++ord) {
                         const uint32_t we = std::min(nwin, wb + win_per_task);
                         uint64_t b1 = 0;
@@ -218,6 +219,8 @@
                                                             (bitmap ? PSET_UNIT_BITMAP : 0u) | (pscatter ? PSET_UNIT_SCATTER : 0u) | round_win << PSET_UNIT_ROUND_SHIFT));
                         f.tasks.push_back({slot, wb, we, pset ? TASK_PSET : TASK_DENSE, task_off});
                 }
+                if (pset && !pscatter && opt.share_tasks && t.q.nterms <= PSET_INLINE_TERMS)
+                        f.pset_q.push_back({pset_query_hash(f.units[unit0], ord, nwin), (uint32_t)unit0, ord});
                 t.q.out_cap = bitmap ? nwin * SPAN_WORDS : (uint32_t)std::min<uint64_t>(0xffffffffull, lead_blocks * 32 + 32ull * (ord + 1) * nlead);
                 f.bitmap_queries += bitmap;
                 f.pscatter_queries += pscatter;
diff --git a/trinity_amd/csrc/planner_types.hpp b/trinity_amd/csrc/planner_types.hpp
--- a/trinity_amd/csrc/planner_types.hpp
+++ b/trinity_amd/csrc/planner_types.hpp
@@ -30,6 +30,7 @@
         uint64_t planes_order = 1;
         uint64_t scatter_bitmap_slack = 4;
         uint64_t pset_order = 1;
+        uint64_t share_tasks = 1;
         uint64_t cand_xcd = 1;
         uint64_t plan_threads = 0;
         uint64_t plan_hot_us = 300;
@@ -142,6 +143,7 @@
         std::vector<uint32_t> slot_of_query;
         std::vector<int32_t> qstatus;
         uint32_t n_dense = 0, n_pset = 0, n_probe = 0, n_cand = 0, n_fused = 0, n_fused16 = 0, n_fusedgen = 0, n_planes = 0, n_planes8 = 0;
+        uint32_t n_pset_lead = 0;
         uint32_t plw = 0;
         uint32_t plane_rows = 0;
         uint64_t out_capacity = 0;
@@ -199,7 +201,7 @@
         constexpr uint32_t SCHED_NB = 64 * 4;
         constexpr uint32_t CAND_SUBS = 128, CAND_COST_SUBS = 16;
         constexpr uint32_t PSET_RANGE_BKS = 64, PSET_SUBS = 64;
-        constexpr uint32_t CAND_KEY0 = TASK_KINDS * SCHED_NB, PSET_KEY0 = CAND_KEY0 + CAND_QUEUES * CAND_SUBS, SCHED_KEYS = PSET_KEY0 + PSET_RANGE_BKS * PSET_SUBS;
+        constexpr uint32_t CAND_KEY0 = TASK_KINDS * SCHED_NB, PSET_KEY0 = CAND_KEY0 + CAND_QUEUES * CAND_SUBS, PSET_FOL_KEY = PSET_KEY0 + PSET_RANGE_BKS * PSET_SUBS, SCHED_KEYS = PSET_FOL_KEY + 1;
         inline uint32_t pset_sub(const uint32_t rank) { return rank < PSET_SUBS / 2 ? rank : std::min(PSET_SUBS / 2 + (rank - PSET_SUBS / 2) / 8, PSET_SUBS - 1); }
         constexpr uint64_t CAND_ROWS_MIN_LEAD = 1024;
         constexpr uint32_t SCHED_RANK[TASK_KINDS] = {3, 0, 4, 5, 6, 7, 8, 1, 2, 9};
@@ -263,6 +265,11 @@
                 bool dense, fuse;
         };
 
+        struct PsetQ {
+                uint64_t hash;
+                uint32_t unit0, ntasks;
+                uint32_t nfol = 0, base = 0, lead_frag = UINT32_MAX, lead_idx = 0, rank = 0;
+        };
         struct QUse {
                 uint32_t qpos, term;
         };
@@ -290,6 +297,8 @@
                 std::vector<uint64_t> benefit;
                 std::vector<uint64_t> cand_row;
                 std::vector<uint32_t> keys, hist;
+                std::vector<PsetQ> pset_q;
+                std::vector<uint32_t> task_folpos;
                 std::vector<uint32_t> treepool;
                 std::vector<uint32_t> tree_terms;
                 uint32_t n_hidden = 0;
@@ -312,7 +321,7 @@
                         keep(fresh.tmp, tmp), keep(fresh.qterms, qterms), keep(fresh.pterms, pterms), keep(fresh.sterms, sterms), keep(fresh.sweights, sweights);
                         keep(fresh.phrases, phrases), keep(fresh.fz, fz), keep(fresh.left_out, left_out), keep(fresh.tasks, tasks), keep(fresh.tcost, tcost);
                         keep(fresh.fused, fused), keep(fresh.ptasks, ptasks), keep(fresh.units, units), keep(fresh.quses, quses), keep(fresh.suses, suses);
-                        keep(fresh.fuses, fuses), keep(fresh.benefit, benefit), keep(fresh.cand_row, cand_row), keep(fresh.keys, keys), keep(fresh.hist, hist), keep(fresh.treepool, treepool);
+                        keep(fresh.fuses, fuses), keep(fresh.benefit, benefit), keep(fresh.cand_row, cand_row), keep(fresh.keys, keys), keep(fresh.hist, hist), keep(fresh.treepool, treepool), keep(fresh.pset_q, pset_q), keep(fresh.task_folpos, task_folpos);
                         keep(fresh.tree_terms, tree_terms);
                         *this = std::move(fresh);
                 }
@@ -372,6 +381,16 @@
                         u.tt[k] = qt[k];
                 return u;
         }
+        inline bool pset_unit_same(const DevPsetUnit &a, const DevPsetUnit &b) {
+                return a.nterms == b.nterms && !memcmp(a.tt, b.tt, sizeof a.tt) && !memcmp(a.row, b.row, sizeof a.row) && a.w_begin == b.w_begin && a.w_end == b.w_end &&
+                       ((a.first ^ b.first) & 0xffu & ~PSET_UNIT_FIRST) == 0;
+        }
+                inline uint64_t pset_query_hash(const DevPsetUnit &u, const uint32_t ntasks, const uint32_t nwin) {
+                uint64_t h = u.nterms | (uint64_t)(u.first & 0xfeu) << 32;
+                auto mix = [&](const uint64_t v) { h = (h ^ v) * 0x9e3779b97f4a7c15ull, h ^= h >> 29; };
+                mix(u.tt[0] | (uint64_t)u.tt[1] << 32), mix(u.tt[2] | (uint64_t)u.tt[3] << 32), mix(ntasks | (uint64_t)nwin << 32);
+                return h;
+        }
         template <class Fn>
         inline void for_each_term_token(const HostIndex &ix, const PlanInput &in, const size_t q, Fn &&fn) {
                 const tri_query &t = in.queries[q];
diff --git a/trinity_amd/csrc/trinity_hip.hip b/trinity_amd/csrc/trinity_hip.hip
--- a/trinity_amd/csrc/trinity_hip.hip
+++ b/trinity_amd/csrc/trinity_hip.hip
@@ -454,7 +454,7 @@
                              {"planes_rebuild", &tri_options::planes_rebuild},
                              {"cand_xcd", &tri_options::cand_xcd},
                              {"plan_threads", &tri_options::plan_threads},
-                             {"probe_max_blocks", &tri_options::probe_max_blocks}, {"phrase_task_div", &tri_options::phrase_task_div}, {"plan_hot_us", &tri_options::plan_hot_us}, {"plan_pin", &tri_options::plan_pin}, {"planes_order", &tri_options::planes_order}, {"pset_order", &tri_options::pset_order}, {"scatter_bitmap_slack", &tri_options::scatter_bitmap_slack}, {"tree_max_bytes", &tri_options::tree_max_bytes}, {"tree_max_nodes", &tri_options::tree_max_nodes}, {"tree_wide_min_nodes", &tri_options::tree_wide_min_nodes}, {"rich_max_terms", &tri_options::rich_max_terms}, {"result_bitmaps", &tri_options::result_bitmaps}, {"cand_task_cost", &tri_options::cand_task_cost}, {"dense_window_cost", &tri_options::dense_window_cost},
+                             {"probe_max_blocks", &tri_options::probe_max_blocks}, {"phrase_task_div", &tri_options::phrase_task_div}, {"plan_hot_us", &tri_options::plan_hot_us}, {"plan_pin", &tri_options::plan_pin}, {"planes_order", &tri_options::planes_order}, {"pset_order", &tri_options::pset_order}, {"share_tasks", &tri_options::share_tasks}, {"scatter_bitmap_slack", &tri_options::scatter_bitmap_slack}, {"tree_max_bytes", &tri_options::tree_max_bytes}, {"tree_max_nodes", &tri_options::tree_max_nodes}, {"tree_wide_min_nodes", &tri_options::tree_wide_min_nodes}, {"rich_max_terms", &tri_options::rich_max_terms}, {"result_bitmaps", &tri_options::result_bitmaps}, {"cand_task_cost", &tri_options::cand_task_cost}, {"dense_window_cost", &tri_options::dense_window_cost},
                              {"isect_max_bytes", &tri_options::isect_max_bytes}, {"isect_max_masks", &tri_options::isect_max_masks}, {"isect_max_runs", &tri_options::isect_max_runs},
                              {"perc_max_bytes", &tri_options::perc_max_bytes}, {"perc_prune", &tri_options::perc_prune}};
                 for (const auto &e : table)
@@ -1306,8 +1306,9 @@
                 HIP_TRY(hipStreamWaitEvent(dev->stream, dev->ev_join, 0));
         if (b->n_pset) {
                 const uint32_t pset_wgs = TRI_PSET_WAVES * 256 / PSET_WG;
-                tri_launch_matching(b, FK_PSETS, 0, [](auto c) { return k_psets<c.value>; }, dim3(std::min<uint32_t>(b->n_pset, (uint32_t)dev->cus * (overlap && dev->opt.overlap_dense_wgs ? std::min<uint32_t>(dense_wgs, pset_wgs) : pset_wgs))),
-                           dim3(PSET_WG), dev->stream, units, pset_sched, b->n_pset, b->d_ticket + TICKET_PSET_WORD, (const uint32_t *)b->dev_at(b->qterms), (const uint32_t *)b->dev_opt(b->qplane), b->d_out,
+                const uint32_t pset_run = fsel.rows ? b->n_pset : b->n_pset_lead;
+                tri_launch_matching(b, FK_PSETS, 0, [](auto c) { return k_psets<c.value>; }, dim3(std::min<uint32_t>(pset_run, (uint32_t)dev->cus * (overlap && dev->opt.overlap_dense_wgs ? std::min<uint32_t>(dense_wgs, pset_wgs) : pset_wgs))),
+                           dim3(PSET_WG), dev->stream, units, pset_sched, pset_run, pset_sched + b->n_pset_lead, b->d_ticket + TICKET_PSET_WORD, (const uint32_t *)b->dev_at(b->qterms), (const uint32_t *)b->dev_opt(b->qplane), b->d_out,
                            b->d_counts, ix->d_masked, (const uint32_t *)ix->d_pcache, b->plw, (const uint32_t *)b->d_scat_off, (const uint32_t *)b->d_scat_cnt,
                            (const uint32_t *)b->d_scat_docs);
                 HIP_TRY(hipGetLastError());
diff --git a/trinity_amd/hostplan.py b/trinity_amd/hostplan.py
--- a/trinity_amd/hostplan.py
+++ b/trinity_amd/hostplan.py
@@ -23,6 +23,8 @@
 TREE_KIND_NARROW, TREE_KIND_WIDE = 0, 1
 DEV_RICH_WIDE = np.dtype([("cells", "<u8"), ("slots", "<u8"), ("stride", "<u4"), ("pad", "<u4")])
 _RICH_WIDE = ["n_rich_wide_tab", "off_rich_wide", "off_rich_sched", "n_rich_wide", "rich_wide_cells", "rich_wide_slots", "sizeof_rich_wide"]
+_SHARE = ["n_pset_lead", "pset_followers", "cand_followers"]
+PSET_UNIT_FOL_SHIFT, PSET_UNIT_FOL_MASK, PSET_UNIT_FOL_AT_SHIFT, PSET_GROUP_MAX = 8, 15, 12, 16
 TREE_NO_PARENT = 0xFFFF
 DEV_UNIT = np.dtype([("out_off", "<u8"), ("begin", "<u4"), ("end", "<u4"), ("tix", "<u4"), ("nterms", "<u4"), ("term_base", "<u4"), ("first", "<u4"), ("tt", "<u4", 4), ("row", "<u4", 4)])
 SCHED_ORDER = [TASK_DENSE, TASK_PSET, TASK_PROBE, TASK_CAND, TASK_FUSED, TASK_FUSED16, TASK_FUSED_GEN, TASK_PLANES, TASK_PLANES8, TASK_TREE]
@@ -46,6 +48,8 @@
         L.tri_host_plan_last_unsupported.restype = None
         L.tri_host_plan_rich_wide.argtypes = [vp, vp]
         L.tri_host_plan_rich_wide.restype = None
+        L.tri_host_plan_share.argtypes = [vp, vp]
+        L.tri_host_plan_share.restype = None
         L.tri_host_pfor128_group.argtypes = [vp, vp, C.POINTER(C.c_uint32), vp, C.POINTER(C.c_uint32)]
         L.tri_host_pfor128_group.restype = None
         for f in (L.tri_host_lucene_encode, L.tri_host_lucene_encode_units):
@@ -110,6 +114,9 @@
         _lib().tri_host_plan_rich_wide(self.h, wide.ctypes.data)
         self.s.update({k: int(v) for k, v in zip(_RICH_WIDE, wide)})
         assert self.s["sizeof_rich_wide"] == DEV_RICH_WIDE.itemsize
+        share = np.zeros(len(_SHARE), dtype=np.uint64)
+        _lib().tri_host_plan_share(self.h, share.ctypes.data)
+        self.s.update({k: int(v) for k, v in zip(_SHARE, share)})
         assert self.s["sizeof_query"] == DEV_QUERY.itemsize and self.s["sizeof_task"] == DEV_TASK.itemsize
         p = _lib().tri_host_plan_block(self.h)
         self.block = np.ctypeslib.as_array(p, shape=(max(1, self.s["block_bytes"]),)).copy()
```

New measurement: 13.32 million. 0.91x the previous value.
